# DaehwanKimLab/centrifuge

Hardware: AMD Instinct MI355X
Metric: classified reads/sec (whole node) on 100bp synthetic reads vs p_compressed; HBM GB/s achieved (higher is better)
Workload: dtype u64

## Files before the change

centrifuge_amd/csrc/cf_device.hip:

```cpp
#include <hip/hip_runtime.h>
#include <sched.h>
#include <dlfcn.h>

#include <algorithm>
#include <cmath>
#include <chrono>
#include <cstdio>
#include <cstdlib>
#include <cstring>
#include <memory>
#include <mutex>
#include <stdexcept>
#include <string>
#include <vector>

#include "../../include/centrifuge_amd.h"
#include "cf_index.hpp"
#include "cf_kernels.hpp"
#include "cf_scan.hpp"
#include "cf_textio.hpp"
#include "cf_inflate.hpp"
#include "cf_restore.hpp"
#include "cf_plan.hpp"
#include "cf_knobs.hpp"
// ... 47 lines not shown
__global__ void __launch_bounds__(256) k_search(DIndex ix, DParams pr, DBatch b) { search_body<G>(ix, pr, b); }

__global__ void __launch_bounds__(256) k_rlen(const uint64_t *off, uint32_t *rlen, uint32_t nReads) { rlen_body(off, rlen, nReads, cf_global_thread()); }
__global__ void __launch_bounds__(256) k_convert(DConvert c) { convert_body(c, cf_global_thread()); }
__global__ void __launch_bounds__(256) k_dense_unpack(DUnpack u) { dense_unpack_body(u, (uint64_t)blockIdx.x * blockDim.x + threadIdx.x); }
__global__ void __launch_bounds__(256) k_pack(DBatch b, uint8_t *recs, uint32_t W) { pack_body(b, recs, W, cf_global_thread()); }

template <int G, int W, bool COUNT>
__global__ void __launch_bounds__(256) __attribute__((amdgpu_waves_per_eu(COUNT ? 1 : W == 4 ? 6 : W == 6 ? 5 : 4, 8))) k_search2(DIndex ix, DParams pr, DBatch b) {
    __shared__ __attribute__((aligned(16))) uint8_t lds[(256 / G) * rec_lds_stride(W) + 256 * 4 * RankTab<G>::WORDS + (256 / G) * 16 * kLazyHits];
    search2_body<G, W, COUNT>(ix, pr, b, lds);
}

template <int W, bool COUNT, int LZ = 0, bool MULTI = false>
__global__ void __launch_bounds__(256) __attribute__((amdgpu_waves_per_eu((W == 4 && LZ == 1) ? 7 : (W == 4 && MULTI) ? 6 : (W == 6 && MULTI) ? 5 : 1, 8))) k_search2_l1(DIndex ix, DParams pr, DBatch b) {
    __shared__ __attribute__((aligned(16))) uint8_t lds[256 * rec_lds_stride(W) + 256 * 16 * (LZ ? LZ : (int)lazy_hits(1, W))];
    search2_body<1, W, COUNT, true, LZ, MULTI>(ix, pr, b, lds);
}
__global__ void __launch_bounds__(256) k_pair_planes(DIndex ix, uint8_t *planes2, uint64_t nGroups) {
    pair_planes_body(ix, planes2, (uint64_t)blockIdx.x * blockDim.x + threadIdx.x, nGroups);
}
__global__ void __launch_bounds__(256) k_occ_planes(DIndex ix, uint8_t *planes, uint64_t nSides) {
    occ_planes_body(ix, planes, (uint64_t)blockIdx.x * blockDim.x + threadIdx.x, nSides);
}
__global__ void __launch_bounds__(256) k_repeat_probe(DIndex ix, uint32_t nSamples, uint32_t depth, uint32_t *hits) {
    const uint32_t i = cf_global_thread();
    bool yes = false;
    if (i < nSamples && ix.len > 2) {
        uint64_t x = 0x9e3779b97f4a7c15ull * (i + 1);
        x ^= x >> 29; x *= 0xbf58476d1ce4e5b9ull; x ^= x >> 32;
        yes = repeat_probe_body(ix, x % (ix.len - 1), depth);
    }
    const uint64_t m = cf_ballot(yes);
    if (m && cf_lane() == (uint32_t)cf_ctz64(m)) (void)cf_atomic_add(hits, (uint32_t)cf_popc64(m));
}

__global__ void __launch_bounds__(256) k_post_fast(DIndex ix, DParams pr, DBatch b) {
    const uint32_t q = cf_global_thread();
    const bool d = q < b.nQueries ? post_fast_body(ix, pr, b, q) : false;
    if (q < b.nQueries && b.postDeferred) b.postDeferred[q] = d ? 1 : 0;
    defer_push(b.slowPost, &b.st->nSlowPost, d, q);
}
template <bool EARLY>
__global__ void __launch_bounds__(256) k_score_fast(DIndex ix, DParams pr, DBatch b) {
    const uint32_t q = cf_global_thread();
    const bool d = q < b.nQueries ? score_fast_body<EARLY>(ix, pr, b, q) : false;
    defer_push(b.slowScore, &b.st->nSlowScore, d, q);
}
__global__ void __launch_bounds__(256) k_list_all(uint32_t *list, uint32_t *counter, uint32_t n) {
    const uint32_t q = cf_global_thread();
    if (q < n) list[q] = q;
    if (q == 0) *counter = n;
}
__global__ void __launch_bounds__(64) __attribute__((amdgpu_waves_per_eu(3, 8))) k_post(DIndex ix, DParams pr, DBatch b, uint32_t capHits) {
    extern __shared__ __attribute__((aligned(16))) uint8_t ldsPost[];
    HitP *scratch = capHits ? reinterpret_cast<HitP *>(ldsPost) + (size_t)cf_local_thread() * capHits : nullptr;
    const uint32_t n = b.st->nSlowPost;
    for (uint32_t i = cf_global_thread(); i < n; i += cf_global_threads()) post_body(ix, pr, b, b.slowPost[i], scratch, capHits);
}
__global__ void __launch_bounds__(64) k_postfix_only(DIndex ix, DParams pr, DBatch b) {
    const uint32_t i = cf_global_thread();
    if (i < b.st->nItems / 2) post_fix(ix, pr, b, b.items[i]);
}
__global__ void k_window(DBatch b, uint32_t qLo, bool keepSlow) { if (cf_global_thread() == 0) row_window_body(b, qLo, keepSlow); }
__global__ void __launch_bounds__(256) k_emit(DParams pr, DBatch b) {
    const uint32_t q = cf_global_thread();
    if (q < b.nQueries) emit_body(pr, b, q);
}
template <int G, bool COUNT>
__global__ void __launch_bounds__(256) k_walk2(DIndex ix, DBatch b) { walk2_body<G, COUNT>(ix, b); }
template <int MODE>
__global__ void __launch_bounds__(256) k_walk_table(DIndex ix, DBatch b) { walk2_body<2, false, MODE>(ix, b); }
template <typename T>
__global__ void __launch_bounds__(256) k_stop_samples(DIndex ix, T *stopVal, uint64_t *stopBits, uint64_t nSamples) {
    for (uint64_t i = (uint64_t)blockIdx.x * blockDim.x + threadIdx.x; i < nSamples; i += (uint64_t)gridDim.x * blockDim.x) {
        const uint64_t pos = trio_at(ix.saPos, i << ix.offRate);
        stopVal[pos] = static_cast<const T *>(ix.offs)[i];
        cf_atomic_or64(&stopBits[pos >> 6], 1ull << (pos & 63));
    }
}
template <typename T>
__global__ void __launch_bounds__(256) k_stop_bounds(DIndex ix, T *stopVal, uint64_t *stopBits) {
    for (uint64_t j = (uint64_t)blockIdx.x * blockDim.x + threadIdx.x; j < ix.nBound; j += (uint64_t)gridDim.x * blockDim.x) {
        const uint64_t pos = trio_at(ix.saPos, ix.boundRow[j]);
        stopVal[pos] = (T)ix.boundRef[j];
        cf_atomic_or64(&stopBits[pos >> 6], 1ull << (pos & 63));
    }
}
template <typename T>
__global__ void k_stop_end(DIndex ix, T *stopVal, uint64_t *stopBits) {
    const uint64_t pos = trio_at(ix.saPos, ix.zOff);
    stopVal[pos] = 0;
    cf_atomic_or64(&stopBits[pos >> 6], 1ull << (pos & 63));
}
template <typename T>
__global__ void __launch_bounds__(256) k_table_by_position(DIndex ix, const T *stopVal, const uint64_t *stopBits, T *table, uint64_t nRows, uint32_t *walkMax) {
    uint32_t gap = 0;
    for (uint64_t row = (uint64_t)blockIdx.x * blockDim.x + threadIdx.x; row < nRows; row += (uint64_t)gridDim.x * blockDim.x) {
        const uint64_t pos = trio_at(ix.saPos, row);
        uint64_t w = pos >> 6;
        uint64_t m = stopBits[w] & (~0ull >> (63 - (pos & 63)));
        while (m == 0 && w > 0) m = stopBits[--w];
        const uint64_t pred = m ? (w << 6) + 63 - (uint64_t)__builtin_clzll(m) : 0;
        table[row] = stopVal[pred];
        const uint32_t g = (uint32_t)(pos - pred);
        gap = g > gap ? g : gap;
    }
    for (int d = 32; d > 0; d >>= 1) { const uint32_t o = __shfl_xor(gap, d, 64); gap = o > gap ? o : gap; }
    if ((threadIdx.x & 63) == 0 && gap) atomicMax(walkMax, gap);
}
template <typename T>
__global__ void __launch_bounds__(256) k_table_spot_check(DIndex ix, const T *table, uint64_t nRows, uint32_t nCheck, uint32_t *bad) {
    const uint32_t i = blockIdx.x * blockDim.x + threadIdx.x;
    if (i >= nCheck) return;
    const uint64_t row = i < 64 ? (i < 32 ? (uint64_t)i : nRows - 1 - (i - 32)) % nRows : (0x9e3779b97f4a7c15ull * (i + 1)) % nRows;
    uint32_t steps = 0;
    const uint32_t want = resolve_plain_row(ix, row, steps);
    if ((uint32_t)table[row] != (sizeof(T) == 2 ? (want & 0xffffu) : want)) atomicAdd(bad, 1u);
}

template <bool COUNT>
__global__ void __launch_bounds__(256) k_walk3(DIndex ix, DBatch b) {
    for (uint64_t i = (uint64_t)blockIdx.x * blockDim.x + threadIdx.x; i < b.st->rowHi - b.st->rowLo; i += (uint64_t)gridDim.x * blockDim.x)
        walk3_body<COUNT>(ix, b, i);
}
template <bool PLANES>
__global__ void __launch_bounds__(256) k_wide_ftab(DIndex ix, uint32_t wideChars, uint64_t *table) {
    __builtin_assume(PLANES ? ix.planes != nullptr : ix.planes == nullptr);
    for (uint64_t t = (uint64_t)blockIdx.x * blockDim.x + threadIdx.x; t < (1ull << (2 * wideChars)); t += (uint64_t)gridDim.x * blockDim.x)
        wide_ftab_body(ix, wideChars, table, t);
}

__global__ void __launch_bounds__(64) k_resolve_slow(DIndex ix, DParams pr, DBatch b) {
    const uint32_t n = b.st->nSlowScore;
    for (uint32_t i = cf_global_thread(); i < n; i += cf_global_threads()) resolve_query_body(ix, pr, b, b.slowScore[i]);
}
__global__ void __launch_bounds__(64) k_score(DIndex ix, DParams pr, DBatch b, uint32_t capRows, uint32_t sparse, uint32_t rowsMin, uint32_t rowsMax) {
    extern __shared__ __attribute__((aligned(16))) uint8_t ldsScore[];
    const uint32_t n = b.st->nSlowScore;
    if (cf_local_thread() % sparse) return;
    const uint32_t me = cf_global_thread() / sparse, all = cf_global_threads() / sparse;
    uint8_t *scratch = capRows ? ldsScore + (size_t)(cf_local_thread() / sparse) * score_scratch_bytes(capRows) : nullptr;
    for (uint32_t i = me; i < n; i += all) score_body(ix, pr, b, b.slowScore[i], scratch, capRows, rowsMin, rowsMax);
}

__global__ void __launch_bounds__(256) k_scatter_nmask(const uint64_t *idx, const uint32_t *mask, uint64_t n, uint64_t nWords, uint32_t *nmask) {
    const uint64_t i = (uint64_t)blockIdx.x * blockDim.x + threadIdx.x;
    if (i < n && idx[i] < nWords) nmask[idx[i]] = mask ? mask[i] : 0u;
}
__global__ void __launch_bounds__(1024) k_count(DBatch b, uint32_t slotBits, bool direct) {
    __shared__ uint32_t slots[3 * kCountSlots];
    count_body(b, slots, blockIdx.x, slotBits, direct);
}
__global__ void __launch_bounds__(256) k_plan(DPlan p) { plan_body(p, cf_global_thread()); }
__global__ void __launch_bounds__(256) k_plan_fill(DPlan p) { plan_fill_body(p, cf_global_thread()); }
__global__ void __launch_bounds__(256) k_rev_words(DPlan p, uint32_t wordsPerRead) { rev_words_body(p, wordsPerRead, (uint64_t)blockIdx.x * blockDim.x + threadIdx.x); }
__global__ void __launch_bounds__(256) k_plan_maxscore(const uint32_t *rlen, const uint8_t *pass, uint32_t nQueries, int paired, uint32_t *maxScore) {
    plan_maxscore_body(rlen, pass, nQueries, paired, maxScore, cf_global_thread());
}
__global__ void __launch_bounds__(256) k_compact(DCompact c) {
    compact_body(c, cf_global_thread());
}
__global__ void __launch_bounds__(256) k_text_count(DTextMark m) { text_count_body(m, (uint64_t)blockIdx.x * blockDim.x + threadIdx.x); }
__global__ void __launch_bounds__(256) k_text_mark(DTextMark m) { text_mark_body(m, (uint64_t)blockIdx.x * blockDim.x + threadIdx.x); }
__global__ void __launch_bounds__(256) k_text_records(DTextRec d) { text_record_body(d, cf_global_thread()); }
__global__ void __launch_bounds__(256) k_inflate(DInflate d) {
    __shared__ InfTables tables[256 / CF_WAVE];
    inflate_body<CF_WAVE>(d, cf_global_thread() / CF_WAVE, cf_lane(), &tables[threadIdx.x / CF_WAVE]);
}
__global__ void __launch_bounds__(64) k_inflate_lane(DInflate d) {
    InfTables tables;
    inflate_body<1>(d, cf_global_thread(), 0, &tables);
}
__global__ void k_text_cut(DTextCut c) { if (cf_global_thread() == 0) text_cut_body(c); }
__global__ void k_text_cut_pair(DTextCutPair c) { if (cf_global_thread() == 0) text_cut_pair_body(c); }
static_assert(kCutBadStart == kTxBadStart, "the pair cut's flag is the record pass's");
__global__ void __launch_bounds__(256) k_text_pack(DTextPack d) { text_pack_body(d, cf_global_thread()); }
__global__ void __launch_bounds__(256) k_fmt_size(DTextFmt f) { fmt_size_body(f, cf_global_thread()); }
__global__ void __launch_bounds__(256) k_fmt_write(DTextFmt f) { fmt_write_body(f, cf_global_thread()); }
__global__ void __launch_bounds__(256) k_fmt_cols_size(DTextFmt f, TextCols pc) { fmt_cols_size_body(f, pc, cf_global_thread()); }
__global__ void __launch_bounds__(256) k_fmt_cols_write(DTextFmt f, TextCols pc) { fmt_cols_write_body(f, pc, cf_global_thread()); }
template <int G, bool WRITE>
__global__ void __launch_bounds__(256) k_restore(DIndex ix, DRestore r) { restore_body<G, WRITE>(ix, r); }
__global__ void __launch_bounds__(256) k_restore_rank(const uint64_t *sumIn, const uint32_t *nextIn, uint64_t *sumOut, uint32_t *nextOut, uint32_t nElem) {
    restore_rank_body(sumIn, nextIn, sumOut, nextOut, nElem, cf_global_thread());
}
__global__ void __launch_bounds__(256) k_restore_link(uint64_t *sum, uint32_t *next, uint32_t nSeg, uint32_t *maxLen) {
    const uint32_t s = cf_global_thread();
    if (s < nSeg) {
        if (next[s] == kRestoreTerm) next[s] = nSeg;
        const uint64_t len = sum[s];
        uint32_t l32 = len > 0xffffffffull ? 0xffffffffu : (uint32_t)len;
        for (int m = 32; m > 0; m >>= 1) { const uint32_t o = cf_shfl_xor(l32, m); if (o > l32) l32 = o; }
        if (cf_lane() == 0 && l32) cf_atomic_max(maxLen, l32);
    }
    else if (s == nSeg) { sum[s] = 0; next[s] = nSeg; }
}

template <int G>
__global__ void k_debug_rank(DIndex ix, const uint8_t *chars, const uint64_t *rows, uint64_t n, uint64_t *out) {
    const uint64_t i = (uint64_t)cf_global_thread() / G;
    const uint64_t ii = i < n ? i : n - 1;
    uint64_t t, bb; bool two;
    if (ix.sides) rank_pair<G>(ix, chars[ii] & 3, rows[ii], rows[ii], t, bb, two);
    else rank_any<G>(ix, chars[ii] & 3, rows[ii], rows[ii], t, bb, two);
    if (i < n && Grp<G>::sub() == 0) out[i] = t;
}

__global__ void __launch_bounds__(256) k_random_sides(const uint8_t *sides, uint64_t numSides, uint32_t steps,
                                                        uint64_t seed, unsigned long long *sink) {
    const uint32_t grp = cf_global_thread() >> 3, sub = cf_lane() & 7;
    uint64_t x = seed + 0x9e3779b97f4a7c15ull * (grp + 1);
    unsigned long long acc = 0;
    for (uint32_t s = 0; s < steps; s++) {
        x ^= x >> 12; x ^= x << 25; x ^= x >> 27;
        const uint64_t side = (x * 0x2545f4914f6cdd1dull) % numSides;
        const u64x2 v = cf_load16(sides + side * 128 + 16 * sub);
        uint32_t f = (uint32_t)(v.x ^ v.y);
        f += __shfl_xor(f, 1, 64); f += __shfl_xor(f, 2, 64); f += __shfl_xor(f, 4, 64);
        x += f & 1u;
        acc += f;
    }
    if (acc == 0x1234567u) sink[0] = acc;
}

}

struct TablePlanRecord { int K = 0, textRate = -1, planes = 0, resolveRate = -1, pair = 0, dropSides = 0; bool valid = false; };
struct cf_index {
    HostIndex h;
    int device = -1;
    DIndex d{};
    DevBuf<uint8_t> planes;
    float planesMs = 0;
    DevBuf<uint8_t> planes2;
    float planes2Ms = 0;
    DevBuf<uint64_t> wide;
    float wideMs = 0;
    DevBuf<uint32_t> text;
    DevBuf<uint64_t> saPos, isa;
    float textMs = 0;
    DevBuf<uint8_t> sides, offs, dense;
    int denseRate = -1;
    uint32_t walkMaxSeen = 0;
    bool denseByPos = false;
    uint32_t restoreShift = 0, restoreMaxSeg = 0;
    DevBuf<uint32_t> posBucket;
    DevBuf<u64x2> posFrag, posSeq;
    float denseMs = 0;
    DevBuf<uint64_t> ftab, eftab, boundRow, paths;
    DevBuf<RefInfo> refInfo;
    DevBuf<uint32_t> boundRef, boundBits, pathTidx;
    uint64_t deviceBytes = 0, fileBytes = 0, budgetSeen = 0;
    cf_index_options opt{};
    bool planned = false;
    bool planDropSides = false, sidesDropped = false;
    uint64_t droppedBytes = 0;
    bool wantTextRate0 = false;
    double repeatFrac = -1.0;
    uint32_t multiRowsPlan = 0;
    TablePlanRecord plan{};
    int plannedTextRate = -2;
    int numCUs = 256;
    int occSides[3] = {0, 0, 0}, occPlanes[3] = {0, 0, 0};
    int occMulti[3] = {0, 0, 0};
    int occLazy[3] = {0, 0, 0};
};

struct cf_classifier {
    cf_index *ix = nullptr;
    cf_params p{};
    std::vector<uint64_t> hostList, exclList;
    DParams d{};
    DevBuf<uint8_t> refExcluded;
    DevBuf<uint64_t> hostSet;
    DevBuf<unsigned long long> counts;
    DevBuf<uint8_t> fmtStrs, fmtLeaf;
    DevBuf<uint32_t> fmtUidOff, fmtRankOff, fmtTaxOff;
    uint32_t fmtIdxZero = 0;
    bool fmtMade = false;
    DevBuf<uint8_t> fmtTaxStrs;
    DevBuf<uint32_t> fmtTrankOff, fmtTnameOff;
    bool fmtTaxMade = false;
    std::mutex fmtMu;
};

template <typename T>
struct PinBuf {
    T *p = nullptr;
    size_t n = 0;
    PinBuf() = default;
    PinBuf(const PinBuf &) = delete;
    PinBuf &operator=(const PinBuf &) = delete;
    ~PinBuf() { if (p) (void)hipHostFree(p); }
    void ensure(size_t count) {
        if (count <= n) return;
        if (p) (void)hipHostFree(p);
        p = nullptr; n = 0;
        count += count / 8;
        if (g_dryBytes) { n = count; return; }
        HIP_OK(hipHostMalloc(reinterpret_cast<void **>(&p), count * sizeof(T), hipHostMallocDefault));
        n = count;
    }
};

struct cf_batch {
    cf_classifier *cl = nullptr;
    uint64_t nReads = 0, nQueries = 0, nWords = 0;
    int paired = 0;
    uint32_t maxLenHost = 0;
    uint32_t recWords = 0;
    bool selfRecords = false;
    bool revMade = false;
    uint32_t revDelta = 0;
    bool loaded = false, planned = false, running = false, finished = false, downloaded = false;
    bool fromBytes = false;
    DevBuf<uint8_t> seq, pass, recs;
    DevBuf<uint64_t> bases, woff, off8, hitBase, qBase, rowVal, rowFirst, tileA;
    DevBuf<uint32_t> nmask, rlen, seeds, items, slotOf, hitCap, nhml, rowRef, nOut, score2, maxScore, qRows, tileC, slowPost, slowScore, qflag, itemMeta;
    DevBuf<HitP> hits;
    DevBuf<PlanHit> qplan;
    DevBuf<QHead> qhead;
    DevBuf<uint64_t> o1tax, o1a, o1b;
    DevBuf<uint8_t> dense;
    uint32_t densePending = 0;
    DevBuf<uint8_t> qinfo;
    DevBuf<uint8_t> postDeferred;
    hipEvent_t evPostFast = nullptr, evPost = nullptr;
    int resultFormat = CF_RESULTS_ROWS;
    DevBuf<uint8_t> text, textOut;
    DevBuf<uint32_t> txCnt, txPos, txSeqOff, txIdOff, txIdLen, txQualOff, txSize, txTuples, txTileC;
    TextCols textCols{};
    bool textFastq = false;
    DevBuf<uint64_t> txBase, txOutOff, txTileA;
    DevBuf<TextStatus> txSt;
    PinBuf<TextStatus> hTxSt;
    PinBuf<uint64_t> hTxTotal;
    PinBuf<uint8_t> hTextOut;
    PinBuf<uint32_t> hTuples;
    DevBuf<uint8_t> zIn;
    DevBuf<InfMember> zMembers;
    DevBuf<uint32_t> zErr;
    DevBuf<InfStatus> zSt;
    DevBuf<uint64_t> zCut;
    PinBuf<InfMember> hZMembers;
    PinBuf<uint64_t> hZCut;
    PinBuf<uint8_t> hTail;
    PinBuf<uint8_t> hTail2;
    bool fromText = false;
    bool rowsStay = false;
    bool textDone = false;
    uint64_t textBytes = 0, tupleWords = 0;
    DevBuf<uint64_t> nIdx; DevBuf<uint32_t> nMsk;
    const uint32_t *nmaskZeroOf = nullptr;
    uint64_t nSparsePrev = 0, nmaskZeroN = 0;
    DevBuf<HmEntry> hm;
    DevBuf<TcEntry> tc;
    DevBuf<OutRow> out, outCompact;
    DevBuf<OpCounts> ops;
    DevBuf<unsigned long long> cursor;
    DevBuf<BatchStatus> st;
    uint64_t hitsCapLimit = 0, rowsCapLimit = 0;
    DPlan pl{};
    DBatch d{};
    PinBuf<BatchStatus> hSt;
    PinBuf<OpCounts> hOps;
    PinBuf<OutRow> hRows;
    PinBuf<uint32_t> hNOut, hScore2, hMaxScore;
    PinBuf<uint8_t> hQInfo;
    uint64_t rowsSpec = 0;
    uint64_t rowsOut = 0, rowsTotal = 0;
    double rowsPerQuery = 0;
    double plannedPerQuery = 0;
    uint32_t passes = 0;
    float planMs = 0;
    float ms[5] = {0, 0, 0, 0, 0};
    OpCounts lastOps{};
    bool opsValid = false;
    hipStream_t stream = nullptr;
    hipStream_t tail = nullptr;
    hipEvent_t ev[10] = {};
    hipEvent_t evLate = nullptr;
    bool evInit = false;
    ~cf_batch() { if (evInit) { for (auto &e : ev) (void)hipEventDestroy(e); (void)hipEventDestroy(evLate); (void)hipEventDestroy(evPostFast); (void)hipEventDestroy(evPost); } if (tail) (void)hipStreamDestroy(tail); }
};

namespace {

void streamSection(std::FILE *f, uint64_t bytes, uint8_t *dst) {
    constexpr size_t kChunk = 32u << 20;
    uint8_t *stage[2] = {nullptr, nullptr};
    hipStream_t st;
    HIP_OK(hipStreamCreate(&st));
    hipEvent_t done[2];
    for (int i = 0; i < 2; i++) {
        HIP_OK(hipHostMalloc(reinterpret_cast<void **>(&stage[i]), kChunk, hipHostMallocDefault));
        HIP_OK(hipEventCreate(&done[i]));
    }
    uint64_t pos = 0;
    int cur = 0;
    bool used[2] = {false, false};
    try {
        while (pos < bytes) {
            const size_t n = static_cast<size_t>(std::min<uint64_t>(kChunk, bytes - pos));
            if (used[cur]) HIP_OK(hipEventSynchronize(done[cur]));
            if (std::fread(stage[cur], 1, n, f) != n) throw std::runtime_error("short read while streaming an index section");
            HIP_OK(hipMemcpyAsync(dst + pos, stage[cur], n, hipMemcpyHostToDevice, st));
            HIP_OK(hipEventRecord(done[cur], st));
            used[cur] = true;
            pos += n;
            cur ^= 1;
        }
        HIP_OK(hipStreamSynchronize(st));
    } catch (...) {
        for (int i = 0; i < 2; i++) { (void)hipHostFree(stage[i]); (void)hipEventDestroy(done[i]); }
        (void)hipStreamDestroy(st);
        throw;
    }
    for (int i = 0; i < 2; i++) { (void)hipHostFree(stage[i]); (void)hipEventDestroy(done[i]); }
    (void)hipStreamDestroy(st);
}

void uploadIndex(cf_index &ix, const std::string &base) {
    HostIndex &h = ix.h;
    h.load(base, [&](Section s, std::FILE *f, uint64_t bytes) {
        switch (s) {
            case Section::Sides:
                ix.sides.alloc(bytes + 128);
                streamSection(f, bytes, ix.sides.p);
                break;
            case Section::Ftab:
                ix.ftab.alloc(bytes / 8);
                streamSection(f, bytes, reinterpret_cast<uint8_t *>(ix.ftab.p));
                break;
            case Section::Eftab:
                ix.eftab.alloc(bytes / 8);
                streamSection(f, bytes, reinterpret_cast<uint8_t *>(ix.eftab.p));
                break;
            case Section::SaSample:
                ix.offs.alloc(bytes + 8);
                streamSection(f, bytes, ix.offs.p);
                break;
        }
    });
    const IndexTables t = makeIndexTables(h);
    ix.boundRow.upload(h.boundRow);
    ix.boundRef.upload(h.boundRef);
    ix.boundBits.upload(t.boundBits);
    {
        std::vector<RefInfo> ri(h.uidTid.size() + 1, RefInfo{0, 0, kNone32});
        for (size_t i = 0; i < h.uidTid.size(); i++) ri[i] = RefInfo{h.uidTid[i], t.refTidx[i], t.refPath[i]};
        ix.refInfo.upload(ri);
    }
    ix.paths.upload(t.paths);
    ix.pathTidx.upload(t.pathTidx);

    DIndex &d = ix.d;
    fillIndexScalars(h, t, d);
    d.sides = ix.sides.p; d.ftab = ix.ftab.p; d.eftab = ix.eftab.p;
    d.offs = ix.offs.p; d.walkOffs = ix.offs.p;
    d.boundRow = ix.boundRow.p; d.boundRef = ix.boundRef.p; d.boundBits = ix.boundBits.p;
    d.refInfo = ix.refInfo.p;
    d.paths = ix.paths.p; d.pathTidx = ix.pathTidx.p;
    ix.deviceBytes = ix.sides.bytes() + ix.ftab.bytes() + ix.eftab.bytes() + ix.offs.bytes() + ix.boundRow.bytes() +
                     ix.boundRef.bytes() + ix.boundBits.bytes() + ix.refInfo.bytes() + ix.paths.bytes() + ix.pathTidx.bytes();
}

int envInt(const char *name, int dflt);
int persistentBlocks(const cf_index &ix, uint64_t groups, int blocksPerCU, int lanes);

size_t freeFor(const cf_index &ix) {
    size_t freeB = 0, totalB = 0;
    HIP_OK(hipMemGetInfo(&freeB, &totalB));
    if (ix.opt.hbm_budget_bytes) {
        const uint64_t left = ix.opt.hbm_budget_bytes > ix.deviceBytes ? ix.opt.hbm_budget_bytes - ix.deviceBytes : 0;
        freeB = (size_t)std::min<uint64_t>(freeB, left);
    }
// ... 665 lines not shown
    c->pair_planes_bytes = ix->planes2.bytes(); c->pair_planes = ix->d.planes2 ? 1 : 0;
    c->resolve_bytes = ix->dense.bytes(); c->resolve_rate = ix->denseRate >= 0 ? ix->denseRate : ix->h.g.offRate;
    c->sides_dropped = ix->sidesDropped ? 1 : 0;
    c->file_bytes_dropped = ix->droppedBytes;
    c->small_range_rows = ix->device >= 0 ? (int32_t)ix->d.multiRows : 0;
    c->repeat_fraction = ix->repeatFrac;
    c->plan_realised = !ix->plan.valid ? -1 :
        (ix->d.wideChars == ix->plan.K && (ix->device >= 0 ? ix->d.posRate : -1) == ix->plan.textRate && (ix->d.planes != nullptr) == (ix->plan.planes != 0) &&
         (ix->denseRate >= 0 ? ix->denseRate : ix->h.g.offRate) == ix->plan.resolveRate && (ix->d.planes2 != nullptr) == (ix->plan.pair != 0) &&
         ix->sidesDropped == (ix->plan.dropSides != 0)) ? 1 : 0;
    c->total_bytes = ix->deviceBytes;
    c->build_ms = ix->planesMs + ix->planes2Ms + ix->wideMs + ix->textMs + ix->denseMs;
    const double log4n = n > 1 ? std::log((double)n) / std::log(4.0) : 0.0;
    const int K = c->wide_ftab_chars ? c->wide_ftab_chars : ix->h.g.ftabChars;
    const double calls = 6.5, rows = 1.42;
    const double twoRow = calls * (std::max(0.0, log4n - K) + 1.4);
    const double r = c->text_verify_rate;
    const double single = r < 0 ? 67.6 : 1.5 * (1.0 + ((double)(1u << (int)r) - 1.0)) + 4.0, verify = r < 0 ? 0.0 : 5.0;
    const double walk = rows * (double)(1u << c->resolve_rate);
    c->est_requests_per_100bp_read = twoRow + single + verify + calls + 2.0 + walk;
    return CF_OK;
}

uint64_t cf_index_text_len(const cf_index *ix) { return ix->h.g.len; }
uint64_t cf_index_num_refs(const cf_index *ix) { return ix->h.uid.size(); }
uint64_t cf_index_num_taxa(const cf_index *ix) { return ix->h.taxa.size(); }
uint64_t cf_index_device_bytes(const cf_index *ix) { return ix->deviceBytes; }
int cf_index_compressed(const cf_index *ix) { return ix->h.compressed ? 1 : 0; }
int cf_index_sa_width(const cf_index *ix) { return ix->h.offw ? 4 : 2; }
int cf_index_wide_ftab_chars(const cf_index *ix) { return ix->d.wideChars; }
int cf_index_occ_planes(const cf_index *ix) { return ix->d.planes ? 1 : 0; }
double cf_index_occ_planes_build_ms(const cf_index *ix) { return ix->planesMs; }
int cf_index_text_verify_rate(const cf_index *ix) { return ix->device >= 0 ? ix->d.posRate : -1; }
double cf_index_text_verify_build_ms(const cf_index *ix) { return ix->textMs; }
int cf_index_resolve_rate(const cf_index *ix) { return ix->denseRate >= 0 ? ix->denseRate : ix->h.g.offRate; }
double cf_index_resolve_build_ms(const cf_index *ix) { return ix->denseMs; }
uint32_t cf_index_walk_bound(const cf_index *ix) { return ix->d.posFrag ? ix->d.walkMax : 0u; }
int cf_index_resolve_by_position(const cf_index *ix) { return ix->denseByPos ? 1 : 0; }
const char *cf_index_uid(const cf_index *ix, uint64_t r) { return r < ix->h.uid.size() ? ix->h.uid[r].c_str() : ""; }
uint64_t cf_index_ref_taxid(const cf_index *ix, uint64_t r) { return r < ix->h.uidTid.size() ? ix->h.uidTid[r] : 0; }
uint64_t cf_index_taxon_id(const cf_index *ix, uint64_t i) { return i < ix->h.taxa.size() ? ix->h.taxa[i] : 0; }
const char *cf_format_seqid(const cf_index *ix, uint32_t u, uint64_t t) { return ix->h.formatSeqId(u, t); }
int cf_tax_rank(const cf_index *ix, uint64_t t) { const TaxNode *n = ix->h.findNode(t); return n ? n->rank : 0; }
const char *cf_tax_rank_string(int rank) { return rankString(rank); }
const char *cf_tax_name(const cf_index *ix, uint64_t t) { return ix->h.name(t); }
uint64_t cf_tax_size(const cf_index *ix, uint64_t t) { return ix->h.size(t); }

cf_status cf_params_default(cf_params *p) {
    if (!p) return CF_ERR_ARG;
    std::memset(p, 0, sizeof *p);
    p->khits = 5; p->min_hitlen = 22; p->rank_slot = 0; p->tree_traverse = 1;
    return CF_OK;
}

cf_status cf_classifier_create(cf_index *ix, const cf_params *p, cf_classifier **out) {
    if (!ix || !p || !out || p->khits < 1 || p->min_hitlen < 15 || p->rank_slot < 0 || p->rank_slot > 9) return CF_ERR_ARG;
    *out = nullptr;
    if (ix->device < 0) { g_err = "index was opened host-only"; return CF_ERR_NO_DEVICE; }
    auto cl = std::make_unique<cf_classifier>();
    cf_status st = guard([&] {
        HIP_OK(hipSetDevice(ix->device));
        cl->ix = ix; cl->p = *p;
        cl->hostList.assign(p->host_taxids, p->host_taxids + std::max(0, p->n_host));
        cl->exclList.assign(p->exclude_taxids, p->exclude_taxids + std::max(0, p->n_exclude));
        cl->p.host_taxids = cl->hostList.data(); cl->p.exclude_taxids = cl->exclList.data();
        const ClassifierTables t = makeClassifier(ix->h, cl->p, cl->d);
        if (cl->d.ihits >= 0x7fffffffu) throw ArgError("-k too large");
        if (ix->h.g.len >= (1ull << 40)) throw ArgError("index too large: hit records hold 40-bit rows");
        if (!t.refExcluded.empty()) { cl->refExcluded.upload(t.refExcluded); cl->d.refExcluded = cl->refExcluded.p; }
        if (!t.hostSet.empty()) { cl->hostSet.upload(t.hostSet); cl->d.hostSet = cl->hostSet.p; cl->d.nHostSet = (uint32_t)t.hostSet.size(); }
        cl->counts.alloc(3 * ix->h.taxa.size());
        HIP_OK(hipMemset(cl->counts.p, 0, cl->counts.bytes()));
    });
    if (st == CF_OK) *out = cl.release();
    return st;
}
void cf_classifier_destroy(cf_classifier *c) { delete c; }

uint32_t cf_gen_rand_seed(const uint8_t *seq, const uint8_t *qual, uint64_t len, const char *name, uint64_t nlen,
                          uint32_t seed) {
    uint32_t r = (seed + 101u) * 59u * 61u * 67u * 71u * 73u * 79u * 83u;
    for (uint64_t i = 0; i < len; i++) r ^= (uint32_t)seq[i] << ((i & 15) << 1);
    for (uint64_t i = 0; i < len; i++) r ^= (uint32_t)(qual ? qual[i] : (uint8_t)'I') << ((i & 3) << 3);
    for (uint64_t i = 0; i < nlen; i++) {
        const int p = (int)(signed char)name[i];
        if (p == '/') break;
        r ^= (uint32_t)p << ((i & 3) << 3);
    }
    return r;
}


static void sizeBatch(cf_batch *bt, uint64_t nReads, uint64_t nWords, uint64_t nBases, uint32_t maxLen, int paired) {
    cf_classifier *cl = bt->cl;
    if (paired && (nReads & 1)) throw ArgError("a paired batch needs an even number of reads");
    if (nReads >= 0x7fffffffull) throw ArgError("a batch holds fewer than 2^31 reads");
    if (maxLen > kMaxReadLen) throw ArgError("reads of more than 16,777,213 bases are not supported (24-bit offsets in the hit records)");
    const uint32_t ftc = (uint32_t)std::max(1, cl->ix->h.g.ftabChars);
    bt->nReads = nReads; bt->paired = paired ? 1 : 0; bt->nQueries = paired ? nReads / 2 : nReads; bt->nWords = nWords;
    bt->maxLenHost = maxLen;
    const uint64_t nq = bt->nQueries;
    bt->bases.ensure(nWords + 16); bt->nmask.ensure(nWords + 16);
    bt->rlen.ensure(nReads + 16); bt->seeds.ensure(nReads + 1); bt->woff.ensure(nReads + 1);
    bt->pass.ensure(nReads + 1); bt->hitCap.ensure(nReads + 16);
    bt->slotOf.ensure(nReads + 1); bt->hitBase.ensure(nReads + 1); bt->items.ensure(nReads + 1);
    bt->nhml.ensure(2 * nReads + 1);
    bt->maxScore.ensure(nq + 1); bt->qflag.ensure(nq + 1); bt->qhead.ensure(nq + 1); bt->qRows.ensure(nq + 16); bt->qBase.ensure(nq + 1);
    bt->qplan.ensure((nq + 1) * kInlinePlan); bt->o1tax.ensure((nq + 1) * kFieldRows); bt->o1a.ensure((nq + 1) * kFieldRows); bt->o1b.ensure((nq + 1) * kFieldRows);
    bt->slowPost.ensure(nq + 1); bt->slowScore.ensure(nq + 1);
    if (envInt("CF_EARLY_SCORE", 0)) bt->postDeferred.ensure(nq + 16);
    bt->out.ensure(nq * (uint64_t)cl->d.k + 1); bt->nOut.ensure(nq + 16); bt->score2.ensure(nq + 1); bt->rowFirst.ensure(nq + 1);
    bt->cursor.ensure(4); bt->ops.ensure(1); bt->st.ensure(1);
    bt->tileA.ensure(scan_tiles_for(std::max(nReads, nq)) + 1); bt->tileC.ensure(scan_tiles_for(std::max(nReads, nq)) + 1);
    bt->recWords = searchVersion() != 2 ? 0u : maxLen <= 128 ? 4u : maxLen <= 192 ? 6u : maxLen <= 256 ? 8u : 0u;
    if ((uint64_t)(0.15 * maxLen) + maxLen / (uint64_t)ftc + 3 >= 255) bt->recWords = 0;
    bt->selfRecords = bt->recWords && cl->ix->d.planes && nWords < 0xffffffffull && envInt("CF_SELF_RECORDS", 1);
    if (bt->selfRecords) bt->itemMeta.ensure(8 * nReads + 8);
    bt->revDelta = bt->selfRecords && 2 * nWords + 64 < 0xffffffffull && envInt("CF_REV_WORDS", 1) ? (uint32_t)nWords + 16u : 0u;
    if (bt->revDelta) bt->bases.ensure(2 * (nWords + 16));
    else if (bt->recWords) bt->recs.ensure(2 * nReads * (uint64_t)rec_bytes((int)bt->recWords) + 64);
    uint64_t hitsWant = 2 * ((nBases ? nBases : 32 * nWords) / ftc + 2 * nReads);
    hitsWant += hitsWant / 50 + 4096;
    if (bt->hitsCapLimit) hitsWant = std::min(hitsWant, bt->hitsCapLimit);
    if (bt->hits.n < hitsWant) bt->hits.ensure(hitsWant);
    if (bt->recWords && bt->hits.n > 0xffffffffull) throw ArgError("batch too large: its hit lists need 32-bit offsets, split it");
    uint64_t rowsWant = std::max<uint64_t>(4 * nq, 1u << 16);
    if (bt->plannedPerQuery > 0) rowsWant = std::max<uint64_t>(rowsWant, (uint64_t)((double)nq * bt->plannedPerQuery * 1.15));
    if (const int per = envInt("CF_ROWS_PER_QUERY", 0)) rowsWant = std::max<uint64_t>((uint64_t)per * nq, 1024);
    if (bt->rowsCapLimit) rowsWant = bt->rowsCapLimit;
    if (bt->rowVal.n < rowsWant || bt->rowsCapLimit) { bt->rowVal.ensure(rowsWant); bt->rowRef.ensure(rowsWant); bt->hm.ensure(rowsWant); bt->tc.ensure(rowsWant); }
    bt->outCompact.ensure(nq * (uint64_t)cl->d.k + 1);
    bt->hSt.ensure(1); bt->hOps.ensure(1);
    bt->hNOut.ensure(nq + 1); bt->hScore2.ensure(nq + 1); bt->hMaxScore.ensure(nq + 1);
    if (bt->resultFormat == CF_RESULTS_NARROW) { bt->qinfo.ensure(nq + 16); bt->hQInfo.ensure(nq + 16); }
    bt->rowsSpec = bt->rowsPerQuery > 0 ? (uint64_t)((double)nq * bt->rowsPerQuery * 1.04) + 4096 : nq + nq / 4 + 1024;
    bt->rowsSpec = std::min<uint64_t>(bt->rowsSpec, nq * (uint64_t)cl->d.k);
    bt->hRows.ensure(std::max<uint64_t>(bt->rowsSpec, nq + nq / 4 + 1024));
    if (g_dryBytes) return;
    if (!bt->evInit) { for (auto &e : bt->ev) HIP_OK(hipEventCreate(&e)); HIP_OK(hipEventCreate(&bt->evLate)); HIP_OK(hipEventCreate(&bt->evPostFast)); HIP_OK(hipEventCreate(&bt->evPost)); bt->evInit = true; }
    if (!bt->tail && (envInt("CF_TAIL_STREAM", 0) || envInt("CF_EARLY_SCORE", 0))) HIP_OK(hipStreamCreateWithFlags(&bt->tail, hipStreamNonBlocking));
}

static void bindBatch(cf_batch *bt) {
    cf_classifier *cl = bt->cl;
    DPlan &pl = bt->pl;
    pl.nmask = bt->nmask.p; pl.rlen = bt->rlen.p; pl.woff = bt->woff.p; pl.nReads = (uint32_t)bt->nReads; pl.ftabChars = cl->ix->h.g.ftabChars;
    pl.maxLenAllowed = bt->maxLenHost;
    pl.nWords = bt->nWords;
    pl.pass = bt->pass.p; pl.hitCap = bt->hitCap.p; pl.slotOf = bt->slotOf.p;
    pl.hitBase = bt->hitBase.p; pl.items = bt->items.p; pl.st = bt->st.p;
    pl.itemMeta = bt->selfRecords ? bt->itemMeta.p : nullptr;
    pl.bases = bt->bases.p; pl.revDelta = bt->revDelta;
    pl.hitsCap = bt->hitsCapLimit ? std::min<uint64_t>(bt->hitsCapLimit, bt->hits.n) : bt->hits.n;
    DBatch &d = bt->d;
    d.bases = bt->bases.p; d.nmask = bt->nmask.p; d.rlen = bt->rlen.p; d.woff = bt->woff.p; d.seeds = bt->seeds.p;
    d.pass = bt->pass.p; d.items = bt->items.p; d.slotOf = bt->slotOf.p; d.hitBase = bt->hitBase.p; d.hitCap = bt->hitCap.p;
    d.lazyHits = (uint32_t)(envInt("CF_LAZY_HITS", 1) != 0) | (cl->ix->d.posFrag ? 4u : 0u);
    d.directRefs = (uint32_t)(cl->ix->dense.p && cl->ix->d.walkRate == 0 && envInt("CF_SCORE_FAST", 1) != 0 && envInt("CF_DIRECT_REFS", 1) != 0);
    d.hits = bt->hits.p; d.nhml = bt->nhml.p; d.qflag = bt->qflag.p; d.qhead = bt->qhead.p; d.qplan = bt->qplan.p; d.qplanStride = bt->qplan.n / kInlinePlan; d.qRows = bt->qRows.p; d.qBase = bt->qBase.p;
    d.rowVal = bt->rowVal.p; d.rowRef = bt->rowRef.p; d.hm = bt->hm.p; d.tc = bt->tc.p;
    d.out = bt->out.p; d.nOut = bt->nOut.p; d.score2 = bt->score2.p;
    d.counts = cl->counts.p; d.nTaxa = (uint32_t)cl->ix->h.taxa.size();
    d.nReads = (uint32_t)bt->nReads; d.nQueries = (uint32_t)bt->nQueries; d.paired = bt->paired;
    d.cursor = bt->cursor.p; d.st = bt->st.p; d.ops = bt->ops.p;
    d.slowPost = bt->slowPost.p; d.slowScore = bt->slowScore.p; d.postDeferred = envInt("CF_EARLY_SCORE", 0) ? bt->postDeferred.p : nullptr;
    d.o1tax = bt->o1tax.p; d.o1a = bt->o1a.p; d.o1b = bt->o1b.p; d.oStride = bt->o1tax.n / kFieldRows;
    d.hitsCap = pl.hitsCap;
    d.rowsCap = bt->rowsCapLimit ? std::min<uint64_t>(bt->rowsCapLimit, bt->rowVal.n) : bt->rowVal.n;
    d.recs = bt->recWords && !bt->selfRecords ? bt->recs.p : nullptr; d.recWords = bt->recWords;
    d.itemMeta = bt->selfRecords ? bt->itemMeta.p : nullptr;
}

static void enqueuePlan(cf_batch *bt, hipStream_t st) {
    const uint64_t nReads = bt->nReads;
    const DPlan &pl = bt->pl;
    HIP_OK(hipStreamWaitEvent(st, bt->ev[8], 0));
    if (bt->densePending) {
        const uint32_t L = bt->densePending - 1;
        const DUnpack u{bt->dense.p, bt->bases.p, bt->rlen.p, (uint32_t)nReads, L, bt->revDelta ? bt->bases.p + bt->revDelta : nullptr};
        bt->revMade = bt->revDelta != 0;
        const uint64_t threads = nReads * std::max<uint64_t>(((uint64_t)L + 31) >> 5, 1);
        hipLaunchKernelGGL(k_dense_unpack, dim3((unsigned)((threads + 255) / 256)), dim3(256), 0, st, u);
        bt->densePending = 0;
    }
    HIP_OK(hipEventRecord(bt->ev[5], st));
    HIP_OK(hipMemsetAsync(bt->st.p, 0, sizeof(BatchStatus), st));
    const dim3 gp((unsigned)((nReads + 1 + 255) / 256)), bl(256);
    if (bt->fromBytes && nReads) hipLaunchKernelGGL(k_rlen, gp, bl, 0, st, bt->off8.p, bt->rlen.p, (uint32_t)nReads);
    scan_enqueue<SCAN_WORDS>(bt->rlen.p, nReads, bt->woff.p, nullptr, bt->tileA.p, bt->tileC.p, st);
    if (bt->fromBytes && nReads) {
        DConvert c{bt->seq.p, bt->off8.p, bt->woff.p, bt->bases.p, bt->nmask.p, (uint32_t)nReads};
        hipLaunchKernelGGL(k_convert, dim3((unsigned)((nReads + 255) / 256)), dim3(256), 0, st, c);
    }
    if (bt->fromText && nReads) {
        const DTextPack c{bt->text.p, bt->txSeqOff.p, bt->rlen.p, bt->woff.p, bt->bases.p, bt->nmask.p, (uint32_t)nReads};
        hipLaunchKernelGGL(k_text_pack, dim3((unsigned)((nReads + 255) / 256)), dim3(256), 0, st, c);
    }
    hipLaunchKernelGGL(k_plan, gp, bl, 0, st, pl);
    scan_enqueue<SCAN_HITS>(bt->hitCap.p, nReads, bt->hitBase.p, bt->slotOf.p, bt->tileA.p, bt->tileC.p, st);
    hipLaunchKernelGGL(k_plan_fill, gp, bl, 0, st, pl);
    if (pl.revDelta && nReads && !bt->revMade) {
        const uint64_t threads = nReads * (uint64_t)bt->recWords;
        hipLaunchKernelGGL(k_rev_words, dim3((unsigned)((threads + 255) / 256)), bl, 0, st, pl, bt->recWords);
    }
    if (bt->nQueries) hipLaunchKernelGGL(k_plan_maxscore, dim3((unsigned)((bt->nQueries + 255) / 256)), bl, 0, st, bt->rlen.p, bt->pass.p,
                                         (uint32_t)bt->nQueries, bt->paired, bt->maxScore.p);
    if (bt->recWords && !bt->selfRecords && nReads) {
        const uint64_t threads = 2 * nReads * (uint64_t)bt->recWords;
        hipLaunchKernelGGL(k_pack, dim3((unsigned)((threads + 255) / 256)), bl, 0, st, bt->d, bt->recs.p, bt->recWords);
    }
    HIP_OK(hipEventRecord(bt->ev[6], st));
    bt->planned = true;
}

static dim3 listGrid(const cf_index &ix, uint64_t nq) { return dim3((unsigned)std::max<uint64_t>(1, std::min<uint64_t>((nq + 63) / 64, (uint64_t)ix.numCUs * 32))); }

static bool earlyScoreMode(const cf_batch *bt) {
    static const bool on = envInt("CF_EARLY_SCORE", 0) != 0 && envInt("CF_POST_FAST", 1) != 0 && envInt("CF_SCORE_FAST", 1) != 0 && envInt("CF_TAIL_STREAM", 0) == 0;
    return on && bt->d.directRefs != 0 && bt->tail != nullptr && bt->nQueries != 0;
}

static void enqueuePost(cf_batch *bt, hipStream_t st) {
    cf_classifier *cl = bt->cl;
    cf_index &ix = *cl->ix;
    const DBatch &d = bt->d;
    const uint32_t nq = (uint32_t)bt->nQueries;
    if (!nq) return;
    static const bool fast = envInt("CF_POST_FAST", 1) != 0;
    if (fast) hipLaunchKernelGGL(k_post_fast, dim3((nq + 255) / 256), dim3(256), 0, st, ix.d, cl->d, d);
    else hipLaunchKernelGGL(k_list_all, dim3((nq + 255) / 256), dim3(256), 0, st, bt->slowPost.p, &bt->st.p->nSlowPost, nq);
    if (earlyScoreMode(bt)) {
        HIP_OK(hipEventRecord(bt->evPostFast, st));
        HIP_OK(hipStreamWaitEvent(bt->tail, bt->evPostFast, 0));
        hipLaunchKernelGGL(k_post, listGrid(ix, nq), dim3(64), 0, bt->tail, ix.d, cl->d, d, 0u);
        HIP_OK(hipEventRecord(bt->evPost, bt->tail));
        hipLaunchKernelGGL(k_score_fast<true>, dim3((nq + 255) / 256), dim3(256), 0, st, ix.d, cl->d, d);
        HIP_OK(hipStreamWaitEvent(st, bt->evPost, 0));
        return;
    }
    static const bool postLds = envInt("CF_POST_LDS", 0) != 0;
    const uint32_t capHits = postLds ? (uint32_t)std::min<uint64_t>(60, 2 * ((uint64_t)bt->maxLenHost / (uint64_t)std::max(1, ix.h.g.ftabChars) + 2)) : 0u;
    hipLaunchKernelGGL(k_post, listGrid(ix, nq), dim3(64), (size_t)64 * capHits * sizeof(HitP), st, ix.d, cl->d, d, capHits);
}

static bool enqueueRowPass(cf_batch *bt, uint32_t qLo, hipStream_t st, bool marks, hipStream_t late = nullptr, bool early = false) {
    cf_classifier *cl = bt->cl;
    cf_index &ix = *cl->ix;
    const DBatch &d = bt->d;
    const uint32_t nq = (uint32_t)bt->nQueries;
    static const bool fast = envInt("CF_SCORE_FAST", 1) != 0;
    HIP_OK(hipMemsetAsync(bt->cursor.p + 1, 0, 8, st));
    hipLaunchKernelGGL(k_window, dim3(1), dim3(64), 0, st, d, qLo, early);
    const bool direct = d.directRefs != 0;
    if (nq && !direct) hipLaunchKernelGGL(k_emit, dim3((nq + 255) / 256), dim3(256), 0, st, cl->d, d);
    if (marks) HIP_OK(hipEventRecord(bt->ev[2], st));
    const bool counted = nq && !direct ? launchWalk(cl, bt, st) : true;
    if (marks) HIP_OK(hipEventRecord(bt->ev[3], st));
    if (nq) {
        if (early) {}
        else if (fast) hipLaunchKernelGGL(k_score_fast<false>, dim3((nq + 255) / 256), dim3(256), 0, st, ix.d, cl->d, d);
        else hipLaunchKernelGGL(k_list_all, dim3((nq + 255) / 256), dim3(256), 0, st, bt->slowScore.p, &bt->st.p->nSlowScore, nq);
        if (late && late != st) {
            HIP_OK(hipEventRecord(bt->evLate, st));
            HIP_OK(hipStreamWaitEvent(late, bt->evLate, 0));
            st = late;
        }
        if (direct) hipLaunchKernelGGL(k_resolve_slow, listGrid(ix, nq), dim3(64), 0, st, ix.d, cl->d, d);
        static const uint32_t capRows = (uint32_t)std::clamp(envInt("CF_SCORE_LDS_ROWS", 0), 0, 64), sparse = (uint32_t)std::clamp(envInt("CF_SCORE_LDS_SPARSE", 2), 1, 64);
        hipLaunchKernelGGL(k_score, listGrid(ix, nq), dim3(64), (size_t)(64 / sparse) * score_scratch_bytes(capRows), st, ix.d, cl->d, d, capRows, capRows ? sparse : 1u, 0u, 0xffffffffu);
        static const uint32_t slotBits = (uint32_t)std::clamp(envInt("CF_COUNT_SLOT_BITS", (int)kCountSlotBits), 1, (int)kCountSlotBits);
        hipLaunchKernelGGL(k_count, dim3((nq + kCountChunk - 1) / kCountChunk), dim3(1024), 0, st, d, slotBits, d.nTaxa <= (1u << slotBits));
    }
    if (marks) HIP_OK(hipEventRecord(bt->ev[4], st));
    return counted;
}

static void enqueueCompact(cf_batch *bt, hipStream_t st) {
    const uint32_t nq = (uint32_t)bt->nQueries;
    const dim3 g((nq + 1 + 255) / 256), bl(256);
    scan_enqueue<SCAN_PLAIN>(bt->nOut.p, nq, bt->rowFirst.p, nullptr, bt->tileA.p, bt->tileC.p, st);
    const bool narrow = bt->resultFormat == CF_RESULTS_NARROW;
    const DCompact c{bt->out.p, bt->o1tax.p, bt->o1a.p, bt->o1b.p, bt->d.oStride, bt->nOut.p, bt->rowFirst.p, (uint32_t)bt->cl->d.k, nq, bt->outCompact.p, bt->st.p,
                     narrow ? reinterpret_cast<NarrowRow *>(bt->outCompact.p) : nullptr, bt->qinfo.p, bt->pass.p, bt->paired};
    hipLaunchKernelGGL(k_compact, g, bl, 0, st, c);
}

static void enqueueClassify(cf_batch *bt, hipStream_t st) {
    cf_classifier *cl = bt->cl;
    HIP_OK(hipMemsetAsync(bt->cursor.p, 0, 32, st));
    HIP_OK(hipMemsetAsync(bt->ops.p, 0, sizeof(OpCounts), st));
    static const bool allFast = envInt("CF_POST_FAST", 1) != 0 && envInt("CF_SCORE_FAST", 1) != 0;
    if (!allFast) {
        HIP_OK(hipMemsetAsync(bt->qRows.p, 0, 4 * (bt->nQueries + 1), st));
        HIP_OK(hipMemsetAsync(bt->nOut.p, 0, 4 * (bt->nQueries + 1), st));
    }
    HIP_OK(hipMemsetAsync(&bt->st.p->nSlowPost, 0, 8, st));
    HIP_OK(hipEventRecord(bt->ev[0], st));
    bool counted = true;
    if (bt->nReads) counted = launchSearch(cl, bt, st) && counted;
    HIP_OK(hipEventRecord(bt->ev[1], st));
    static const int tailMode = envInt("CF_TAIL_STREAM", 0);
    hipStream_t ts = bt->tail && tailMode == 1 ? bt->tail : st;
    hipStream_t late = bt->tail && tailMode == 2 ? bt->tail : ts;
    if (ts != st) HIP_OK(hipStreamWaitEvent(ts, bt->ev[1], 0));
    const bool early = earlyScoreMode(bt);
    enqueuePost(bt, ts);
    scan_enqueue<SCAN_PLAIN>(bt->qRows.p, bt->nQueries, bt->qBase.p, nullptr, bt->tileA.p, bt->tileC.p, ts);
    counted = enqueueRowPass(bt, 0, ts, true, late, early) && counted;
    enqueueCompact(bt, late);
    HIP_OK(hipEventRecord(bt->ev[9], late));
    bt->opsValid = counted;
    bt->passes = 1;
    bt->running = true; bt->finished = false; bt->downloaded = false;
    bt->stream = st;
}

static void enqueueDownload(cf_batch *bt, hipStream_t st) {
    const uint64_t nq = bt->nQueries;
    HIP_OK(hipStreamWaitEvent(st, bt->ev[9], 0));
    HIP_OK(hipMemcpyAsync(bt->hSt.p, bt->st.p, sizeof(BatchStatus), hipMemcpyDeviceToHost, st));
    HIP_OK(hipMemcpyAsync(bt->hOps.p, bt->ops.p, sizeof(OpCounts), hipMemcpyDeviceToHost, st));
    if (nq && !bt->rowsStay) {
        const uint64_t spec = std::min<uint64_t>(bt->rowsSpec, nq * (uint64_t)bt->cl->d.k);
        if (bt->resultFormat == CF_RESULTS_NARROW) {
            HIP_OK(hipMemcpyAsync(bt->hQInfo.p, bt->qinfo.p, nq, hipMemcpyDeviceToHost, st));
            HIP_OK(hipMemcpyAsync(bt->hScore2.p, bt->score2.p, nq * 4, hipMemcpyDeviceToHost, st));
            HIP_OK(hipMemcpyAsync(bt->hRows.p, bt->outCompact.p, spec * sizeof(NarrowRow), hipMemcpyDeviceToHost, st));
        } else {
            HIP_OK(hipMemcpyAsync(bt->hNOut.p, bt->nOut.p, nq * 4, hipMemcpyDeviceToHost, st));
            HIP_OK(hipMemcpyAsync(bt->hScore2.p, bt->score2.p, nq * 4, hipMemcpyDeviceToHost, st));
            HIP_OK(hipMemcpyAsync(bt->hMaxScore.p, bt->maxScore.p, nq * 4, hipMemcpyDeviceToHost, st));
            HIP_OK(hipMemcpyAsync(bt->hRows.p, bt->outCompact.p, spec * sizeof(OutRow), hipMemcpyDeviceToHost, st));
        }
    }
    HIP_OK(hipEventRecord(bt->ev[7], st));
    bt->downloaded = true;
}

static void waitBatch(cf_batch *bt) {
    if (!bt->running) throw ArgError("no batch in flight on this slot");
    if (bt->finished) return;
    hipStream_t st = bt->stream;
    if (!bt->downloaded) enqueueDownload(bt, st);
    HIP_OK(hipEventSynchronize(bt->ev[7]));
    HIP_OK(hipGetLastError());
    bool redo = false;
    auto fetchStatus = [&] {
        HIP_OK(hipEventSynchronize(bt->ev[9]));
        HIP_OK(hipMemcpyAsync(bt->hSt.p, bt->st.p, sizeof(BatchStatus), hipMemcpyDeviceToHost, st));
        HIP_OK(hipStreamSynchronize(st));
        HIP_OK(hipGetLastError());
    };
    HIP_OK(hipEventSynchronize(bt->ev[9]));
    auto lapse = [&](float &ms, int a, int b) { if (hipEventElapsedTime(&ms, bt->ev[a], bt->ev[b]) != hipSuccess) { ms = 0; (void)hipGetLastError(); } };
    lapse(bt->planMs, 5, 6);
    lapse(bt->ms[0], 0, 1); lapse(bt->ms[1], 1, 2); lapse(bt->ms[2], 2, 3); lapse(bt->ms[3], 3, 4); lapse(bt->ms[4], 0, 4);
    if (bt->hSt.p->flags & kStLenOverflow) throw ArgError("a read is longer than the max_len the batch was submitted with");
    if (bt->hSt.p->flags & kStWordsOverflow) throw ArgError("the read lengths need more packed words than n_words says were uploaded");
    if (bt->hSt.p->flags & kStHitsOverflow) {
        const uint64_t need = bt->hSt.p->hitsNeed;
        if (bt->recWords && need > 0xffffffffull) throw ArgError("batch too large: its hit lists need 32-bit offsets, split it");
        bt->hitsCapLimit = 0;
        bt->hits.ensure(need + 1);
        bindBatch(bt);
        enqueuePlan(bt, st);
        enqueueClassify(bt, st);
        fetchStatus();
        if (bt->hSt.p->flags & kStHitsOverflow) throw std::logic_error("hit pool still too small after growing it");
        redo = true;
    }
    while (bt->hSt.p->qHi < bt->nQueries) {
        if (bt->hSt.p->qHi == bt->hSt.p->qLo) {
            const uint64_t need = bt->hSt.p->needRows;
            bt->rowsCapLimit = 0;
            bt->rowVal.ensure(need); bt->rowRef.ensure(need); bt->hm.ensure(need); bt->tc.ensure(need);
            bindBatch(bt);
        }
        enqueueRowPass(bt, bt->hSt.p->qHi, st, false);
        bt->passes++;
        bt->opsValid = false;
        fetchStatus();
        redo = true;
    }
    if (redo) {
        enqueueCompact(bt, st);
        HIP_OK(hipEventRecord(bt->ev[9], st));
        enqueueDownload(bt, st);
        HIP_OK(hipEventSynchronize(bt->ev[7]));
        HIP_OK(hipGetLastError());
    }
    bt->rowsOut = bt->hSt.p->rowsOut;
    bt->rowsTotal = bt->hSt.p->rowsTotal;
    if (bt->nQueries) { bt->rowsPerQuery = (double)bt->rowsOut / (double)bt->nQueries; bt->plannedPerQuery = (double)bt->rowsTotal / (double)bt->nQueries; }
    if (bt->rowsOut > bt->rowsSpec && !bt->rowsStay) {
        const uint64_t have = bt->rowsSpec;
        const size_t rb = bt->resultFormat == CF_RESULTS_NARROW ? sizeof(NarrowRow) : sizeof(OutRow);
        if (bt->rowsOut > bt->hRows.n) {
            PinBuf<OutRow> bigger;
            bigger.ensure(bt->rowsOut + bt->rowsOut / 8);
            std::memcpy(bigger.p, bt->hRows.p, have * rb);
            std::swap(bt->hRows.p, bigger.p); std::swap(bt->hRows.n, bigger.n);
        }
        HIP_OK(hipMemcpy(reinterpret_cast<uint8_t *>(bt->hRows.p) + have * rb, reinterpret_cast<const uint8_t *>(bt->outCompact.p) + have * rb, (bt->rowsOut - have) * rb, hipMemcpyDeviceToHost));
    }
    bt->lastOps = *bt->hOps.p;
    bt->lastOps.nRows = bt->rowsTotal;
    bt->finished = true;
}

static void uploadBytes(cf_batch *bt, const uint8_t *seq, const uint64_t *off, const uint32_t *seeds, uint64_t nReads, int paired, hipStream_t st) {
    uint64_t nWords = 0, maxLen = 0;
    for (uint64_t r = 0; r < nReads; r++) {
        if (off[r + 1] < off[r]) throw ArgError("read offsets must be non-decreasing");
        const uint64_t L = off[r + 1] - off[r];
        nWords += (L + 31) >> 5;
        maxLen = std::max(maxLen, L);
    }
    if (maxLen > 0xffffffffull) throw ArgError("a read is longer than 2^32 bases");
    const uint64_t nbases = off[nReads] - off[0];
    if (nbases && !seq) throw ArgError("null sequence buffer");
    sizeBatch(bt, nReads, nWords, nbases, (uint32_t)maxLen, paired);
    bt->seq.ensure(nbases + 16); bt->off8.ensure(nReads + 1);
    bindBatch(bt);
    HIP_OK(hipMemsetAsync(bt->seq.p + nbases, 0, 16, st));
    if (nbases) HIP_OK(hipMemcpyAsync(bt->seq.p, seq + off[0], nbases, hipMemcpyHostToDevice, st));
    if (off[0] == 0) HIP_OK(hipMemcpyAsync(bt->off8.p, off, (nReads + 1) * 8, hipMemcpyHostToDevice, st));
    else {
        std::vector<uint64_t> rel(nReads + 1);
        for (uint64_t r = 0; r <= nReads; r++) rel[r] = off[r] - off[0];
        HIP_OK(hipMemcpy(bt->off8.p, rel.data(), (nReads + 1) * 8, hipMemcpyHostToDevice));
    }
    if (nReads) HIP_OK(hipMemcpyAsync(bt->seeds.p, seeds, nReads * 4, hipMemcpyHostToDevice, st));
    HIP_OK(hipEventRecord(bt->ev[8], st));
    bt->fromBytes = true; bt->fromText = false; bt->densePending = 0; bt->revMade = false; bt->nmaskZeroOf = nullptr;
    bt->loaded = true; bt->planned = false; bt->running = false; bt->finished = false;
}

static void uploadSparseMask(cf_batch *bt, const uint64_t *idx, const uint32_t *mask, uint64_t nNWords, uint64_t nWords, hipStream_t st) {
    if (bt->nmaskZeroOf != bt->nmask.p || bt->nmaskZeroN != bt->nmask.n) {
        HIP_OK(hipMemsetAsync(bt->nmask.p, 0, bt->nmask.bytes(), st));
        bt->nmaskZeroOf = bt->nmask.p; bt->nmaskZeroN = bt->nmask.n; bt->nSparsePrev = 0;
    } else if (bt->nSparsePrev) {
        hipLaunchKernelGGL(k_scatter_nmask, dim3((unsigned)((bt->nSparsePrev + 255) / 256)), dim3(256), 0, st, bt->nIdx.p, nullptr,
                           bt->nSparsePrev, (uint64_t)bt->nmask.n, bt->nmask.p);
        bt->nSparsePrev = 0;
    }
    if (nNWords) {
        bt->nSparsePrev = nNWords;
        bt->nIdx.ensure(nNWords); bt->nMsk.ensure(nNWords);
        HIP_OK(hipMemcpyAsync(bt->nIdx.p, idx, nNWords * 8, hipMemcpyHostToDevice, st));
        HIP_OK(hipMemcpyAsync(bt->nMsk.p, mask, nNWords * 4, hipMemcpyHostToDevice, st));
        hipLaunchKernelGGL(k_scatter_nmask, dim3((unsigned)((nNWords + 255) / 256)), dim3(256), 0, st, bt->nIdx.p, bt->nMsk.p,
                           nNWords, nWords, bt->nmask.p);
    }
}

static void uploadPacked(cf_batch *bt, const cf_packed_reads *in, hipStream_t st) {
    if (in->n_reads && (!in->len || !in->seeds)) throw ArgError("null length / seed array");
    if (in->n_words && !in->bases) throw ArgError("null packed-base array");
    if (!in->nmask && in->n_nwords && (!in->nword_idx || !in->nword_mask)) throw ArgError("null sparse N-mask arrays");
    sizeBatch(bt, in->n_reads, in->n_words, in->n_bases, in->max_len, in->paired);
    bindBatch(bt);
    if (in->n_words) {
        HIP_OK(hipMemcpyAsync(bt->bases.p, in->bases, in->n_words * 8, hipMemcpyHostToDevice, st));
        if (in->nmask) { HIP_OK(hipMemcpyAsync(bt->nmask.p, in->nmask, in->n_words * 4, hipMemcpyHostToDevice, st)); bt->nmaskZeroOf = nullptr; }
        else uploadSparseMask(bt, in->nword_idx, in->nword_mask, in->n_nwords, in->n_words, st);
    }
    if (in->n_reads) {
        HIP_OK(hipMemcpyAsync(bt->rlen.p, in->len, in->n_reads * 4, hipMemcpyHostToDevice, st));
        HIP_OK(hipMemcpyAsync(bt->seeds.p, in->seeds, in->n_reads * 4, hipMemcpyHostToDevice, st));
    }
    HIP_OK(hipEventRecord(bt->ev[8], st));
    bt->fromBytes = false; bt->fromText = false; bt->densePending = 0; bt->revMade = false;
    bt->loaded = true; bt->planned = false; bt->running = false; bt->finished = false;
}

static void uploadDense(cf_batch *bt, const cf_dense_reads *in, hipStream_t st) {
    if (in->n_reads && (!in->bases4 || !in->seeds)) throw ArgError("null dense-base / seed array");
    if (in->n_nwords && (!in->nword_idx || !in->nword_mask)) throw ArgError("null sparse N-mask arrays");
    if (in->read_len > kMaxReadLen) throw ArgError("reads of more than 16,777,213 bases are not supported (24-bit offsets in the hit records)");
    const uint64_t W = ((uint64_t)in->read_len + 31) >> 5, bpr = ((uint64_t)in->read_len + 3) >> 2;
    const uint64_t nWords = in->n_reads * W, nBytes = in->n_reads * bpr;
    sizeBatch(bt, in->n_reads, nWords, in->n_reads * (uint64_t)in->read_len, in->read_len, in->paired);
    bt->dense.ensure(nBytes + 32);
    bindBatch(bt);
    if (in->n_reads) {
        HIP_OK(hipMemcpyAsync(bt->dense.p, in->bases4, nBytes, hipMemcpyHostToDevice, st));
        HIP_OK(hipMemsetAsync(bt->dense.p + nBytes, 0, 32, st));
        HIP_OK(hipMemcpyAsync(bt->seeds.p, in->seeds, in->n_reads * 4, hipMemcpyHostToDevice, st));
        if (nWords) uploadSparseMask(bt, in->nword_idx, in->nword_mask, in->n_nwords, nWords, st);
    }
    bt->densePending = in->n_reads ? in->read_len + 1 : 0; bt->revMade = false;
    HIP_OK(hipEventRecord(bt->ev[8], st));
    bt->fromBytes = false; bt->fromText = false;
    bt->loaded = true; bt->planned = false; bt->running = false; bt->finished = false;
}


static void uploadText(cf_batch *bt, const cf_text_reads *in, hipStream_t st, cf_text_info *info) {
    if (in->format != CF_TEXT_FASTA && in->format != CF_TEXT_FASTQ) throw ArgError("cf_text_reads::format is CF_TEXT_FASTA or CF_TEXT_FASTQ");
    const int nBlocks = in->text2 ? 2 : 1;
    const char *src[2] = {in->text, in->text2};
    const uint64_t nBs[2] = {in->n_bytes, in->text2 ? in->n_bytes2 : 0};
    if ((nBs[0] && !src[0]) || (nBs[1] && !src[1])) throw ArgError("null text block");
    if (nBs[0] + nBs[1] >= 0xffff0000ull) throw ArgError("the text blocks of a batch hold fewer than 2^32 bytes (32-bit places in them)");
    const bool fasta = in->format == CF_TEXT_FASTA;
    uint64_t at[2], pieces[2], pieceAt[2], recCap[2], posCap[2], posAt[2], textBytes = 0, nPieces = 0, posTotal = 0, recMax = 0;
    for (int k = 0; k < nBlocks; k++) {
        at[k] = textBytes; pieces[k] = (nBs[k] + kTextPiece - 1) / kTextPiece; pieceAt[k] = nPieces;
        recCap[k] = nBs[k] / 32 + 1024; posCap[k] = fasta ? recCap[k] : 4 * recCap[k]; posAt[k] = posTotal;
        textBytes += pieces[k] * kTextPiece + kTextPad; nPieces += pieces[k] + 16; posTotal += posCap[k] + 16;
        recMax = std::max(recMax, recCap[k]);
    }
    const uint64_t readCap = recMax * (uint64_t)nBlocks;
    bt->text.ensure(textBytes);
    bt->txCnt.ensure(nPieces + 16); bt->txBase.ensure(nPieces + 16); bt->txPos.ensure(posTotal + 16);
    bt->txTileA.ensure(scan_tiles_for(std::max(pieces[0], pieces[nBlocks - 1])) + 1); bt->txTileC.ensure(scan_tiles_for(std::max(pieces[0], pieces[nBlocks - 1])) + 1);
    bt->rlen.ensure(readCap + 16); bt->seeds.ensure(readCap + 16);
    bt->txSeqOff.ensure(readCap + 16); bt->txIdOff.ensure(readCap + 16); bt->txIdLen.ensure(readCap + 16);
    if (!fasta) bt->txQualOff.ensure(readCap + 16);
    bt->txSt.ensure(1); bt->hTxSt.ensure(1); bt->hTxTotal.ensure(2);
    *info = cf_text_info{};
    bt->loaded = false; bt->planned = false; bt->running = false; bt->finished = false;
    HIP_OK(hipMemsetAsync(bt->txSt.p, 0, sizeof(TextStatus), st));
    const uint32_t seed0 = (in->global_seed + 101u) * 59u * 61u * 67u * 71u * 73u * 79u * 83u;
    const dim3 bl(256);
    for (int k = 0; k < nBlocks; k++) {
        uint8_t *text = bt->text.p + at[k];
        HIP_OK(hipMemsetAsync(text + nBs[k], 0, pieces[k] * kTextPiece + kTextPad - nBs[k], st));
        if (nBs[k]) HIP_OK(hipMemcpyAsync(text, src[k], nBs[k], hipMemcpyHostToDevice, st));
        uint32_t *cnt = bt->txCnt.p + pieceAt[k], *pos = bt->txPos.p + posAt[k];
        uint64_t *base = bt->txBase.p + pieceAt[k];
        const DTextMark m{text, nBs[k], fasta ? (uint32_t)'>' : (uint32_t)'\n', cnt, base, pos, posCap[k]};
        const dim3 gp((unsigned)std::max<uint64_t>(1, (pieces[k] + 255) / 256));
        if (pieces[k]) hipLaunchKernelGGL(k_text_count, gp, bl, 0, st, m);
        scan_enqueue<SCAN_PLAIN>(cnt, pieces[k], base, nullptr, bt->txTileA.p, bt->txTileC.p, st);
        if (pieces[k]) hipLaunchKernelGGL(k_text_mark, gp, bl, 0, st, m);
        DTextRec d{text, nBs[k], pos, base + pieces[k], posCap[k], (uint32_t)recCap[k], (uint32_t)in->format, seed0,
                   bt->rlen.p, bt->seeds.p, bt->txSeqOff.p, bt->txIdOff.p, bt->txIdLen.p, bt->txSt.p, (uint32_t)at[k], (uint32_t)nBlocks, (uint32_t)k,
                   fasta ? nullptr : bt->txQualOff.p};
        hipLaunchKernelGGL(k_text_records, dim3((unsigned)((recCap[k] + 255) / 256)), bl, 0, st, d);
        HIP_OK(hipMemcpyAsync(bt->hTxTotal.p + k, base + pieces[k], 8, hipMemcpyDeviceToHost, st));
    }
    HIP_OK(hipMemcpyAsync(bt->hTxSt.p, bt->txSt.p, sizeof(TextStatus), hipMemcpyDeviceToHost, st));
    HIP_OK(hipStreamSynchronize(st));
    HIP_OK(hipGetLastError());
    const TextStatus ts = *bt->hTxSt.p;
    uint64_t nRec[2] = {0, 0};
    for (int k = 0; k < nBlocks; k++) nRec[k] = fasta ? bt->hTxTotal.p[k] : bt->hTxTotal.p[k] >> 2;
    if (ts.flags) { info->irregular = ts.flags; return; }
    if (nBlocks == 2 && nRec[0] != nRec[1]) { info->irregular = kTxMateCount; return; }
    uint64_t nq = nRec[0];
    if (in->max_reads && nq > in->max_reads) nq = in->max_reads;
    const uint64_t nReads = nq * (uint64_t)nBlocks;
    sizeBatch(bt, nReads, ts.words(), ts.bases(), ts.maxLen, nBlocks == 2);
    bindBatch(bt);
    HIP_OK(hipEventRecord(bt->ev[8], st));
    bt->fromText = true; bt->fromBytes = false; bt->densePending = 0; bt->revMade = false; bt->nmaskZeroOf = nullptr;
    bt->textFastq = !fasta;
    bt->loaded = true;
    info->n_reads = nReads; info->n_bases = ts.bases(); info->max_len = ts.maxLen;
}

constexpr uint64_t kBgzfTailRoom = 1u << 20;
static void uploadBgzf(cf_batch *bt, const cf_bgzf_reads *in, hipStream_t st, cf_text_info *info, cf_bgzf_info *zi) {
    if (in->format != CF_TEXT_FASTA && in->format != CF_TEXT_FASTQ) throw ArgError("cf_bgzf_reads::format is CF_TEXT_FASTA or CF_TEXT_FASTQ");
    if ((in->n_bytes && !in->members) || (in->head_bytes && !in->head)) throw ArgError("null member / head bytes");
    if (in->n_bytes >= 0xffff0000ull || in->head_bytes >= 0xffff0000ull) throw ArgError("the text of a batch holds fewer than 2^32 - 65536 bytes (32-bit places in it)");
    *info = cf_text_info{}; *zi = cf_bgzf_info{};
    bt->loaded = false; bt->planned = false; bt->running = false; bt->finished = false;
    const uint8_t *z = static_cast<const uint8_t *>(in->members);
    uint64_t nMembers = 0;
    for (uint64_t at = 0; at < in->n_bytes; nMembers++) {
        if (in->n_bytes - at < 18) break;
        at += (uint64_t)(z[at + 16] | (z[at + 17] << 8)) + 1;
    }
    bt->hZMembers.ensure(nMembers + 1);
    uint64_t total = in->head_bytes, at = 0;
    uint32_t m = 0;
    for (; at < in->n_bytes; m++) {
        const uint8_t *h = z + at;
        bool ok = in->n_bytes - at >= 18 && h[0] == 0x1f && h[1] == 0x8b && h[2] == 8 && (h[3] & 4);
        const uint64_t xlen = ok ? (uint64_t)(h[10] | (h[11] << 8)) : 0, bsize = ok ? (uint64_t)(h[16] | (h[17] << 8)) + 1 : 0;
        ok = ok && xlen >= 6 && h[12] == 'B' && h[13] == 'C' && h[14] == 2 && h[15] == 0 && bsize >= 12 + xlen + 8 && bsize <= in->n_bytes - at;
        uint32_t crc = 0, isize = 0;
        if (ok) { std::memcpy(&crc, h + bsize - 8, 4); std::memcpy(&isize, h + bsize - 4, 4); ok = isize <= kInfMaxOut; }
        if (!ok) { zi->corrupt = kInfHeader; zi->bad_member = m; return; }
        bt->hZMembers.p[m] = InfMember{(uint32_t)(at + 12 + xlen), (uint32_t)(bsize - 12 - xlen - 8), (uint32_t)total, isize, crc};
        total += isize; at += bsize;
        if (total >= 0xffff0000ull) throw ArgError("the text of a batch holds fewer than 2^32 - 65536 bytes (32-bit places in it)");
    }
    nMembers = m;
    zi->inflated_bytes = total - in->head_bytes;
    const bool fasta = in->format == CF_TEXT_FASTA;
    const uint64_t pieces = (total + kTextPiece - 1) / kTextPiece, recCap = total / 32 + 1024, posCap = fasta ? recCap : 4 * recCap;
    bt->text.ensure(pieces * kTextPiece + kTextPad);
    bt->zIn.ensure(in->n_bytes + kInfPad + 8); bt->zMembers.ensure(nMembers + 1); bt->zErr.ensure(nMembers + 1); bt->zSt.ensure(1); bt->zCut.ensure(2);
    bt->hZCut.ensure(4); bt->hTail.ensure(kBgzfTailRoom + 16);
    bt->txCnt.ensure(pieces + 32); bt->txBase.ensure(pieces + 32); bt->txPos.ensure(posCap + 32);
    bt->txTileA.ensure(scan_tiles_for(pieces) + 1); bt->txTileC.ensure(scan_tiles_for(pieces) + 1);
    bt->rlen.ensure(recCap + 16); bt->seeds.ensure(recCap + 16);
    bt->txSeqOff.ensure(recCap + 16); bt->txIdOff.ensure(recCap + 16); bt->txIdLen.ensure(recCap + 16);
    if (!fasta) bt->txQualOff.ensure(recCap + 16);
    bt->txSt.ensure(1); bt->hTxSt.ensure(1); bt->hTxTotal.ensure(2);
    HIP_OK(hipMemsetAsync(bt->txSt.p, 0, sizeof(TextStatus), st));
    HIP_OK(hipMemsetAsync(bt->zSt.p, 0, sizeof(InfStatus), st));
    uint8_t *text = bt->text.p;
    HIP_OK(hipMemsetAsync(text + total, 0, pieces * kTextPiece + kTextPad - total, st));
    if (in->head_bytes) HIP_OK(hipMemcpyAsync(text, in->head, in->head_bytes, hipMemcpyHostToDevice, st));
    if (nMembers) {
        HIP_OK(hipMemcpyAsync(bt->zIn.p, in->members, in->n_bytes, hipMemcpyHostToDevice, st));
        HIP_OK(hipMemcpyAsync(bt->zMembers.p, bt->hZMembers.p, nMembers * sizeof(InfMember), hipMemcpyHostToDevice, st));
        const DInflate d{bt->zIn.p, bt->zMembers.p, (uint32_t)nMembers, text, bt->zErr.p, bt->zSt.p, nullptr};
        static const bool byLane = cfamd::cf_knob("CF_INFLATE_LANES") && std::atoi(cfamd::cf_knob("CF_INFLATE_LANES")) == 1;
        if (byLane) hipLaunchKernelGGL(k_inflate_lane, dim3((unsigned)((nMembers + 63) / 64)), dim3(64), 0, st, d);
        else hipLaunchKernelGGL(k_inflate, dim3((unsigned)((nMembers + 256 / CF_WAVE - 1) / (256 / CF_WAVE))), dim3(256), 0, st, d);
    }
    const dim3 bl(256);
    const DTextMark mk{text, total, fasta ? (uint32_t)'>' : (uint32_t)'\n', bt->txCnt.p, bt->txBase.p, bt->txPos.p, posCap};
    const dim3 gp((unsigned)std::max<uint64_t>(1, (pieces + 255) / 256));
    if (pieces) hipLaunchKernelGGL(k_text_count, gp, bl, 0, st, mk);
    scan_enqueue<SCAN_PLAIN>(bt->txCnt.p, pieces, bt->txBase.p, nullptr, bt->txTileA.p, bt->txTileC.p, st);
    if (pieces) hipLaunchKernelGGL(k_text_mark, gp, bl, 0, st, mk);
    const DTextCut ct{text, total, bt->txPos.p, bt->txBase.p + pieces, posCap, fasta ? 0u : 1u, in->last ? 1u : 0u, bt->zCut.p};
    hipLaunchKernelGGL(k_text_cut, dim3(1), dim3(64), 0, st, ct);
    HIP_OK(hipMemcpyAsync(bt->hZCut.p, bt->zCut.p, 16, hipMemcpyDeviceToHost, st));
    HIP_OK(hipMemcpyAsync(bt->hZCut.p + 2, bt->zSt.p, sizeof(InfStatus), hipMemcpyDeviceToHost, st));
    HIP_OK(hipStreamSynchronize(st));
    HIP_OK(hipGetLastError());
    InfStatus zs; std::memcpy(&zs, bt->hZCut.p + 2, sizeof zs);
    if (zs.bad) {
        zi->bad_member = 0xffffffffu - zs.bad;
        HIP_OK(hipMemcpy(&zi->corrupt, bt->zErr.p + zi->bad_member, 4, hipMemcpyDeviceToHost));
        if (!zi->corrupt) zi->corrupt = kInfBadCode;
        return;
    }
    const uint64_t cut = bt->hZCut.p[0];
    if (cut > total) throw std::runtime_error("cf_batch_upload_bgzf: the cut lies behind the text");
    if (total - cut > kBgzfTailRoom) { info->irregular = kTxTailRoom; return; }
    if (total > cut) HIP_OK(hipMemcpyAsync(bt->hTail.p, text + cut, total - cut, hipMemcpyDeviceToHost, st));
    const uint32_t seed0 = (in->global_seed + 101u) * 59u * 61u * 67u * 71u * 73u * 79u * 83u;
    const DTextRec d{text, cut, bt->txPos.p, bt->zCut.p + 1, posCap, (uint32_t)recCap, (uint32_t)in->format, seed0,
                     bt->rlen.p, bt->seeds.p, bt->txSeqOff.p, bt->txIdOff.p, bt->txIdLen.p, bt->txSt.p, 0u, 1u, 0u, fasta ? nullptr : bt->txQualOff.p};
    hipLaunchKernelGGL(k_text_records, dim3((unsigned)((recCap + 255) / 256)), bl, 0, st, d);
    HIP_OK(hipMemcpyAsync(bt->hTxSt.p, bt->txSt.p, sizeof(TextStatus), hipMemcpyDeviceToHost, st));
    HIP_OK(hipStreamSynchronize(st));
    HIP_OK(hipGetLastError());
    const TextStatus ts = *bt->hTxSt.p;
    if (ts.flags) { info->irregular = ts.flags; return; }
    uint64_t nq = fasta ? bt->hZCut.p[1] : bt->hZCut.p[1] >> 2;
    if (in->max_reads && nq > in->max_reads) nq = in->max_reads;
    sizeBatch(bt, nq, ts.words(), ts.bases(), ts.maxLen, false);
    bindBatch(bt);
    HIP_OK(hipEventRecord(bt->ev[8], st));
    bt->fromText = true; bt->fromBytes = false; bt->densePending = 0; bt->revMade = false; bt->nmaskZeroOf = nullptr;
    bt->textFastq = !fasta;
    bt->loaded = true;
    info->n_reads = nq; info->n_bases = ts.bases(); info->max_len = ts.maxLen;
    zi->tail = reinterpret_cast<const char *>(bt->hTail.p); zi->tail_bytes = total - cut;
}

static bool bgzfMemberTable(const cf_bgzf_reads *in, uint64_t inAt, uint64_t textAt, InfMember *out, uint64_t &nMembers, uint64_t &total, cf_bgzf_info *zi) {
    const uint8_t *z = static_cast<const uint8_t *>(in->members);
    uint64_t at = 0;
    uint32_t m = 0;
    total = in->head_bytes;
    for (; at < in->n_bytes; m++) {
        const uint8_t *h = z + at;
        bool ok = in->n_bytes - at >= 18 && h[0] == 0x1f && h[1] == 0x8b && h[2] == 8 && (h[3] & 4);
        const uint64_t xlen = ok ? (uint64_t)(h[10] | (h[11] << 8)) : 0, bsize = ok ? (uint64_t)(h[16] | (h[17] << 8)) + 1 : 0;
        ok = ok && xlen >= 6 && h[12] == 'B' && h[13] == 'C' && h[14] == 2 && h[15] == 0 && bsize >= 12 + xlen + 8 && bsize <= in->n_bytes - at;
        uint32_t crc = 0, isize = 0;
        if (ok) { std::memcpy(&crc, h + bsize - 8, 4); std::memcpy(&isize, h + bsize - 4, 4); ok = isize <= kInfMaxOut; }
        if (!ok) { zi->corrupt = kInfHeader; zi->bad_member = m; return false; }
        if (out) out[m] = InfMember{(uint32_t)(inAt + at + 12 + xlen), (uint32_t)(bsize - 12 - xlen - 8), (uint32_t)(textAt + total), isize, crc};
        total += isize; at += bsize;
        if (total >= 0xffff0000ull) throw ArgError("the texts of a batch hold fewer than 2^32 - 65536 bytes (32-bit places in them)");
    }
    nMembers = m;
    return true;
}
static void uploadBgzfPair(cf_batch *bt, const cf_bgzf_reads *in1, const cf_bgzf_reads *in2, hipStream_t st, cf_text_info *info, cf_bgzf_info *z1, cf_bgzf_info *z2) {
    const cf_bgzf_reads *in[2] = {in1, in2};
    cf_bgzf_info *zi[2] = {z1, z2};
    if (in1->format != CF_TEXT_FASTA && in1->format != CF_TEXT_FASTQ) throw ArgError("cf_bgzf_reads::format is CF_TEXT_FASTA or CF_TEXT_FASTQ");
    if (in2->format != in1->format || in2->global_seed != in1->global_seed || in2->max_reads != in1->max_reads)
        throw ArgError("cf_batch_upload_bgzf_pair: format, global_seed and max_reads are the first mate's; the second mate's differ");
    for (int k = 0; k < 2; k++) {
        if ((in[k]->n_bytes && !in[k]->members) || (in[k]->head_bytes && !in[k]->head)) throw ArgError("null member / head bytes");
        if (in[k]->n_bytes >= 0xffff0000ull || in[k]->head_bytes >= 0xffff0000ull) throw ArgError("the texts of a batch hold fewer than 2^32 - 65536 bytes (32-bit places in them)");
    }
    const uint64_t inAt[2] = {0, (in1->n_bytes + 7) & ~7ull}, inBytes = inAt[1] + in2->n_bytes;
    if (inBytes >= 0xffff0000ull) throw ArgError("the members of a batch hold fewer than 2^32 - 65536 bytes (32-bit places in them)");
    *info = cf_text_info{}; *z1 = cf_bgzf_info{}; *z2 = cf_bgzf_info{};
    bt->loaded = false; bt->planned = false; bt->running = false; bt->finished = false;
    uint64_t nM[2] = {0, 0}, total[2] = {0, 0};
    for (int k = 0; k < 2; k++) if (!bgzfMemberTable(in[k], 0, 0, nullptr, nM[k], total[k], zi[k])) return;
    if (total[0] + total[1] >= 0xffff0000ull) throw ArgError("the texts of a batch hold fewer than 2^32 - 65536 bytes (32-bit places in them)");
    const bool fasta = in1->format == CF_TEXT_FASTA;
    uint64_t at[2], pieces[2], pieceAt[2], recCap[2], posCap[2], posAt[2], textBytes = 0, nPieces = 0, posTotal = 0, recMax = 0;
    for (int k = 0; k < 2; k++) {
        at[k] = textBytes; pieces[k] = (total[k] + kTextPiece - 1) / kTextPiece; pieceAt[k] = nPieces;
        recCap[k] = total[k] / 32 + 1024; posCap[k] = fasta ? recCap[k] : 4 * recCap[k]; posAt[k] = posTotal;
        textBytes += pieces[k] * kTextPiece + kTextPad; nPieces += pieces[k] + 16; posTotal += posCap[k] + 16;
        recMax = std::max(recMax, recCap[k]);
    }
    if (textBytes >= 0xffffffffull) throw ArgError("the texts of a batch hold fewer than 2^32 - 65536 bytes (32-bit places in them)");
    const uint64_t nMembers = nM[0] + nM[1];
    bt->hZMembers.ensure(nMembers + 1);
    for (int k = 0; k < 2; k++) (void)bgzfMemberTable(in[k], inAt[k], at[k], bt->hZMembers.p + (k ? nM[0] : 0), nM[k], total[k], zi[k]);
    for (int k = 0; k < 2; k++) zi[k]->inflated_bytes = total[k] - in[k]->head_bytes;
    const uint64_t readCap = 2 * recMax;
    bt->text.ensure(textBytes);
    bt->zIn.ensure(inBytes + kInfPad + 8); bt->zMembers.ensure(nMembers + 1); bt->zErr.ensure(nMembers + 1); bt->zSt.ensure(1); bt->zCut.ensure(4);
    bt->hZCut.ensure(6); bt->hTail.ensure(kBgzfTailRoom + 16); bt->hTail2.ensure(kBgzfTailRoom + 16);
    bt->txCnt.ensure(nPieces + 16); bt->txBase.ensure(nPieces + 16); bt->txPos.ensure(posTotal + 16);
    bt->txTileA.ensure(scan_tiles_for(std::max(pieces[0], pieces[1])) + 1); bt->txTileC.ensure(scan_tiles_for(std::max(pieces[0], pieces[1])) + 1);
    bt->rlen.ensure(readCap + 16); bt->seeds.ensure(readCap + 16);
    bt->txSeqOff.ensure(readCap + 16); bt->txIdOff.ensure(readCap + 16); bt->txIdLen.ensure(readCap + 16);
    if (!fasta) bt->txQualOff.ensure(readCap + 16);
    bt->txSt.ensure(1); bt->hTxSt.ensure(1); bt->hTxTotal.ensure(2);
    HIP_OK(hipMemsetAsync(bt->txSt.p, 0, sizeof(TextStatus), st));
    HIP_OK(hipMemsetAsync(bt->zSt.p, 0, sizeof(InfStatus), st));
    for (int k = 0; k < 2; k++) {
        uint8_t *text = bt->text.p + at[k];
        HIP_OK(hipMemsetAsync(text + total[k], 0, pieces[k] * kTextPiece + kTextPad - total[k], st));
        if (in[k]->head_bytes) HIP_OK(hipMemcpyAsync(text, in[k]->head, in[k]->head_bytes, hipMemcpyHostToDevice, st));
        if (nM[k]) HIP_OK(hipMemcpyAsync(bt->zIn.p + inAt[k], in[k]->members, in[k]->n_bytes, hipMemcpyHostToDevice, st));
    }
    if (nMembers) {
        HIP_OK(hipMemcpyAsync(bt->zMembers.p, bt->hZMembers.p, nMembers * sizeof(InfMember), hipMemcpyHostToDevice, st));
        const DInflate d{bt->zIn.p, bt->zMembers.p, (uint32_t)nMembers, bt->text.p, bt->zErr.p, bt->zSt.p, nullptr};
        hipLaunchKernelGGL(k_inflate, dim3((unsigned)((nMembers + 256 / CF_WAVE - 1) / (256 / CF_WAVE))), dim3(256), 0, st, d);
    }
    const dim3 bl(256);
    DTextCutPair cp{};
    for (int k = 0; k < 2; k++) {
        uint8_t *text = bt->text.p + at[k];
        uint32_t *cnt = bt->txCnt.p + pieceAt[k], *pos = bt->txPos.p + posAt[k];
        uint64_t *base = bt->txBase.p + pieceAt[k];
        const DTextMark mk{text, total[k], fasta ? (uint32_t)'>' : (uint32_t)'\n', cnt, base, pos, posCap[k]};
        const dim3 gp((unsigned)std::max<uint64_t>(1, (pieces[k] + 255) / 256));
        if (pieces[k]) hipLaunchKernelGGL(k_text_count, gp, bl, 0, st, mk);
        scan_enqueue<SCAN_PLAIN>(cnt, pieces[k], base, nullptr, bt->txTileA.p, bt->txTileC.p, st);
        if (pieces[k]) hipLaunchKernelGGL(k_text_mark, gp, bl, 0, st, mk);
        cp.blk[k] = DTextCut{text, total[k], pos, base + pieces[k], posCap[k], fasta ? 0u : 1u, in[k]->last ? 1u : 0u, bt->zCut.p + 2 * k};
    }
    cp.flags = &bt->txSt.p->flags;
    hipLaunchKernelGGL(k_text_cut_pair, dim3(1), dim3(64), 0, st, cp);
    HIP_OK(hipMemcpyAsync(bt->hZCut.p, bt->zCut.p, 32, hipMemcpyDeviceToHost, st));
    HIP_OK(hipMemcpyAsync(bt->hZCut.p + 4, bt->zSt.p, sizeof(InfStatus), hipMemcpyDeviceToHost, st));
    HIP_OK(hipStreamSynchronize(st));
    HIP_OK(hipGetLastError());
    InfStatus zs; std::memcpy(&zs, bt->hZCut.p + 4, sizeof zs);
    if (zs.bad) {
        const uint64_t g = 0xffffffffu - zs.bad;
        cf_bgzf_info *z = g < nM[0] ? z1 : z2;
        z->bad_member = (uint32_t)(g < nM[0] ? g : g - nM[0]);
        HIP_OK(hipMemcpy(&z->corrupt, bt->zErr.p + g, 4, hipMemcpyDeviceToHost));
        if (!z->corrupt) z->corrupt = kInfBadCode;
        return;
    }
    const uint64_t cut[2] = {bt->hZCut.p[0], bt->hZCut.p[2]}, nMark[2] = {bt->hZCut.p[1], bt->hZCut.p[3]};
    if (cut[0] > total[0] || cut[1] > total[1]) throw std::runtime_error("cf_batch_upload_bgzf_pair: a cut lies behind its text");
    if (in1->last && in2->last && (cut[0] < total[0] || cut[1] < total[1])) { info->irregular = kTxMateCount; return; }
    if (total[0] - cut[0] > kBgzfTailRoom || total[1] - cut[1] > kBgzfTailRoom) { info->irregular = kTxTailRoom; return; }
    uint8_t *hTail[2] = {bt->hTail.p, bt->hTail2.p};
    for (int k = 0; k < 2; k++) if (total[k] > cut[k]) HIP_OK(hipMemcpyAsync(hTail[k], bt->text.p + at[k] + cut[k], total[k] - cut[k], hipMemcpyDeviceToHost, st));
    const uint32_t seed0 = (in1->global_seed + 101u) * 59u * 61u * 67u * 71u * 73u * 79u * 83u;
    for (int k = 0; k < 2; k++) {
        const DTextRec d{bt->text.p + at[k], cut[k], bt->txPos.p + posAt[k], bt->zCut.p + 2 * k + 1, posCap[k], (uint32_t)recCap[k], (uint32_t)in1->format, seed0,
                         bt->rlen.p, bt->seeds.p, bt->txSeqOff.p, bt->txIdOff.p, bt->txIdLen.p, bt->txSt.p, (uint32_t)at[k], 2u, (uint32_t)k,
                         fasta ? nullptr : bt->txQualOff.p};
        hipLaunchKernelGGL(k_text_records, dim3((unsigned)((recCap[k] + 255) / 256)), bl, 0, st, d);
    }
    HIP_OK(hipMemcpyAsync(bt->hTxSt.p, bt->txSt.p, sizeof(TextStatus), hipMemcpyDeviceToHost, st));
    HIP_OK(hipStreamSynchronize(st));
    HIP_OK(hipGetLastError());
    const TextStatus ts = *bt->hTxSt.p;
    if (ts.flags) { info->irregular = ts.flags; return; }
    uint64_t nq = fasta ? nMark[0] : nMark[0] >> 2;
    if (nq != (fasta ? nMark[1] : nMark[1] >> 2)) throw std::runtime_error("cf_batch_upload_bgzf_pair: the two cuts hold different numbers of records");
    if (in1->max_reads && nq > in1->max_reads) nq = in1->max_reads;
    sizeBatch(bt, 2 * nq, ts.words(), ts.bases(), ts.maxLen, true);
    bindBatch(bt);
    HIP_OK(hipEventRecord(bt->ev[8], st));
    bt->fromText = true; bt->fromBytes = false; bt->densePending = 0; bt->revMade = false; bt->nmaskZeroOf = nullptr;
    bt->textFastq = !fasta;
    bt->loaded = true;
    info->n_reads = 2 * nq; info->n_bases = ts.bases(); info->max_len = ts.maxLen;
    for (int k = 0; k < 2; k++) { zi[k]->tail = reinterpret_cast<const char *>(hTail[k]); zi[k]->tail_bytes = total[k] - cut[k]; }
}

cf_status cf_host_alloc(void **p, size_t bytes) {
    if (!p) return CF_ERR_ARG;
    *p = nullptr;
    if (!haveDevice()) { g_err = "no HIP device visible"; return CF_ERR_NO_DEVICE; }
    return guard([&] { HIP_OK(hipHostMalloc(p, bytes ? bytes : 1, hipHostMallocDefault)); });
}
void cf_host_free(void *p) { if (p) (void)hipHostFree(p); }

cf_status cf_batch_alloc(cf_classifier *cl, uint64_t maxReads, uint64_t maxWords, cf_batch **out) {
    if (!cl || !out) return CF_ERR_ARG;
    *out = nullptr;
    auto bt = std::make_unique<cf_batch>();
    cf_status st = guard([&] {
        HIP_OK(hipSetDevice(cl->ix->device));
        bt->cl = cl;
        const uint64_t per = maxReads ? (32 * maxWords + maxReads - 1) / maxReads : 0;
        sizeBatch(bt.get(), maxReads & ~1ull, maxWords, 0, (uint32_t)std::min<uint64_t>(per, 128), 0);
        bt->nReads = bt->nQueries = bt->nWords = 0;
    });
    if (st == CF_OK) *out = bt.release();
    return st;
}

cf_status cf_slot_estimate_bytes(uint64_t maxReads, uint64_t maxWords, int khits, int ftabChars, int occPlanes, uint64_t *bytes) {
    if (!bytes || khits < 1 || ftabChars < 1) return CF_ERR_ARG;
    *bytes = 0;
    return guard([&] {
        cf_index ix;
        ix.h.g.ftabChars = ftabChars;
        if (occPlanes) ix.d.planes = reinterpret_cast<const uint8_t *>(&ix);
        cf_classifier cl;
        cl.ix = &ix; cl.d.k = (uint32_t)khits;
        uint64_t total = 0;
        g_dryBytes = &total;
        try {
            cf_batch bt;
            bt.cl = &cl;
            const uint64_t per = maxReads ? (32 * maxWords + maxReads - 1) / maxReads : 0;
            sizeBatch(&bt, maxReads & ~1ull, maxWords, 0, (uint32_t)std::min<uint64_t>(per, 128), 0);
            bt.evInit = false;
        } catch (...) { g_dryBytes = nullptr; throw; }
        g_dryBytes = nullptr;
        *bytes = total;
    });
}

cf_status cf_batch_upload_packed_async(cf_batch *bt, const cf_packed_reads *in, void *streamv) {
    if (!bt || !in) return CF_ERR_ARG;
    return guard([&] {
        HIP_OK(hipSetDevice(bt->cl->ix->device));
        if (bt->running && !bt->finished) throw ArgError("the slot still has a batch in flight: cf_batch_wait first");
        uploadPacked(bt, in, static_cast<hipStream_t>(streamv));
    });
}

cf_status cf_batch_upload_dense_async(cf_batch *bt, const cf_dense_reads *in, void *streamv) {
    if (!bt || !in) return CF_ERR_ARG;
    return guard([&] {
        HIP_OK(hipSetDevice(bt->cl->ix->device));
        if (bt->running && !bt->finished) throw ArgError("the slot still has a batch in flight: cf_batch_wait first");
        uploadDense(bt, in, static_cast<hipStream_t>(streamv));
    });
}

cf_status cf_batch_set_result_format(cf_batch *bt, int format) {
    if (!bt || (format != CF_RESULTS_ROWS && format != CF_RESULTS_NARROW)) return CF_ERR_ARG;
    if (format == CF_RESULTS_NARROW && bt->cl->d.k > 63) { g_err = "the narrow result format holds a query's row count in six bits: -k <= 63"; return CF_ERR_ARG; }
    if (bt->running && !bt->finished) { g_err = "the slot still has a batch in flight: cf_batch_wait first"; return CF_ERR_ARG; }
    return guard([&] {
        HIP_OK(hipSetDevice(bt->cl->ix->device));
        if (format != bt->resultFormat) { bt->finished = false; bt->running = false; bt->downloaded = false; }
        bt->resultFormat = format;
        if (format == CF_RESULTS_NARROW) { bt->qinfo.ensure(bt->nOut.n + 16); bt->hQInfo.ensure(bt->nOut.n + 16); }
    });
}

cf_status cf_classify_async(cf_classifier *cl, cf_batch *bt, void *streamv) {
    if (!cl || !bt || bt->cl != cl) return CF_ERR_ARG;
    return guard([&] {
        HIP_OK(hipSetDevice(cl->ix->device));
        if (!bt->loaded) throw ArgError("no reads were uploaded into this slot");
        hipStream_t st = static_cast<hipStream_t>(streamv);
        bt->rowsStay = false; bt->textDone = false;
        if (!bt->planned) enqueuePlan(bt, st);
        enqueueClassify(bt, st);
    });
}

cf_status cf_batch_reclassify_async(cf_classifier *cl, cf_batch *bt, void *streamv) {
    if (!cl || !bt || bt->cl != cl) return CF_ERR_ARG;
    return guard([&] {
        HIP_OK(hipSetDevice(cl->ix->device));
        if (!bt->loaded) throw ArgError("no reads were uploaded into this slot");
        if (bt->running && !bt->finished) throw ArgError("the slot still has a batch in flight: cf_batch_wait first");
        hipStream_t st = static_cast<hipStream_t>(streamv);
        bt->rowsStay = false; bt->textDone = false;
        enqueuePlan(bt, st);
        enqueueClassify(bt, st);
    });
}

cf_status cf_batch_download_async(cf_batch *bt, void *streamv) {
    if (!bt) return CF_ERR_ARG;
    return guard([&] {
        HIP_OK(hipSetDevice(bt->cl->ix->device));
        if (!bt->running) throw ArgError("cf_classify_async first");
        enqueueDownload(bt, static_cast<hipStream_t>(streamv));
    });
}

cf_status cf_batch_submit(cf_batch *bt, const cf_packed_reads *in, void *streamv) {
    cf_status s = cf_batch_upload_packed_async(bt, in, streamv);
    if (s == CF_OK) s = cf_classify_async(bt->cl, bt, streamv);
    if (s == CF_OK) s = cf_batch_download_async(bt, streamv);
    return s;
}

cf_status cf_batch_wait_narrow(cf_batch *bt, cf_results_narrow *res) {
    if (!bt) return CF_ERR_ARG;
    if (bt->resultFormat != CF_RESULTS_NARROW) { g_err = "cf_batch_wait_narrow on a slot whose result format is not CF_RESULTS_NARROW"; return CF_ERR_ARG; }
    const cf_status rc = guard([&] {
        HIP_OK(hipSetDevice(bt->cl->ix->device));
        if (bt->rowsStay && bt->finished) throw ArgError("the batch was finished by cf_batch_wait_text: its rows were not downloaded");
        waitBatch(bt);
        if (res) {
            static_assert(sizeof(cf_row16) == sizeof(NarrowRow), "cf_row16 layout");
            res->rows = reinterpret_cast<const cf_row16 *>(bt->hRows.p);
            res->qinfo = bt->hQInfo.p; res->score2 = bt->hScore2.p;
            res->n_queries = bt->nQueries; res->total_rows = bt->rowsOut;
            res->planned_sa_rows = bt->rowsTotal; res->row_passes = bt->passes;
            res->slow_post = bt->hSt.p->nSlowPost; res->slow_score = bt->hSt.p->nSlowScore;
        }
    });
    if (rc != CF_OK) {
        (void)hipStreamSynchronize(bt->stream);
        bt->running = false; bt->finished = false;
    }
    return rc;
}

uint32_t cf_narrow_max_score(uint8_t qinfo, uint32_t len1, uint32_t len2, int paired) {
    const uint64_t s0 = len1 > 15 ? (uint64_t)(len1 - 15) * (len1 - 15) : 0u, s1 = len2 > 15 ? (uint64_t)(len2 - 15) * (len2 - 15) : 0u;
    const bool p0 = (qinfo & 0x40u) != 0, p1 = paired && (qinfo & 0x80u) != 0;
    const uint64_t v = (p0 && p1) ? s0 + s1 : p0 ? s0 : p1 ? s1 : 0u;
    return v >= 0xffffffffull ? kMaxScoreNever : (uint32_t)v;
}

// ... 658 lines not shown
```

centrifuge_amd/csrc/cf_kernels.hpp:

```cpp
#pragma once
#include "cf_platform.hpp"

namespace cfamd {

constexpr uint32_t kNone32 = 0xffffffffu;
constexpr uint64_t kNone64 = ~0ull;
constexpr uint32_t kSideChars = 384;
constexpr int kSearchChunk = CF_WAVE;

struct RefInfo { uint64_t tax; uint32_t tidx, pid; };
static_assert(sizeof(RefInfo) == 16, "RefInfo layout");
struct DIndex {
    const uint8_t *sides;
    const uint64_t *ftab, *eftab;
    uint64_t fchr0, fchr1, fchr2, fchr3;
    uint64_t len, zOff, zSide;
    uint32_t zIn;
    int32_t ftabChars, offRate, offw;
    const void *offs;
    const uint8_t *planes;
    const uint8_t *planes2;
    const uint64_t *wide;
    int32_t wideChars;
    const uint64_t *text;
    const uint64_t *saPos;
    const uint64_t *isa;
    int32_t posRate;
    int32_t isaRate;
    uint32_t multiRows, multiMinRun;
    uint32_t verifyMinRun;
    const void *walkOffs;
    int32_t walkRate;
    const uint64_t *boundRow;
    const uint32_t *boundRef;
    const uint32_t *boundBits;
    uint64_t lastBoundary;
    uint32_t nBound;
    int32_t boundShift;
    const uint32_t *posBucket;
    const u64x2 *posFrag, *posSeq;
    uint32_t posShift, nPosFrag, walkMax;
    const RefInfo *refInfo;
    const uint64_t *paths;
    const uint32_t *pathTidx;
    uint32_t nRef, tidxOne;
    int32_t small;
};

struct DParams {
    uint32_t k, m, inc, ihits, rankSlot;
    int32_t traverse;
    const uint8_t *refExcluded;
    const uint64_t *hostSet;
    uint32_t nHostSet;
};

struct Hit {
    uint64_t top, bot;
    uint32_t bwoff, len;
    uint32_t nelt;
};

struct HitP { uint64_t w0, w1; };
constexpr uint64_t kHitPosForm = 1ull << 39, kRowIsPos = 1ull << 63;
CF_DEV uint32_t nhml_make(uint32_t nHits, bool hasLong) { return (nHits & 0x7fffffffu) | (hasLong ? 0x80000000u : 0u); }
CF_DEV uint32_t nhml_n(uint32_t v) { return v & 0x7fffffffu; }
CF_DEV bool nhml_long(uint32_t v) { return (v >> 31) != 0; }
static_assert(sizeof(HitP) == 16, "HitP layout");
constexpr uint64_t kHit40 = (1ull << 40) - 1;
constexpr uint32_t kHit24 = (1u << 24) - 1;
constexpr uint32_t kMaxReadLen = kHit24 - 2;

CF_DEV HitP hit_pack(const Hit &h) {
    const bool dummy = h.top == kNone64;
    const bool pos = !dummy && (h.top & kRowIsPos) != 0;
    const uint64_t size = dummy ? 0 : pos ? (1ull | kHitPosForm) : h.bot - h.top;
    const uint64_t bw = h.bwoff == kNone32 ? (uint64_t)kHit24 : (uint64_t)(h.bwoff & kHit24);
    HitP p;
    p.w0 = (dummy ? kHit40 : (h.top & kHit40)) | ((uint64_t)(h.len & kHit24) << 40);
    p.w1 = (size & kHit40) | (bw << 40);
    return p;
}
CF_DEV uint32_t hp_len(const HitP &p) { return (uint32_t)(p.w0 >> 40); }
CF_DEV uint64_t hp_size(const HitP &p) { return p.w1 & (kHit40 & ~kHitPosForm); }
CF_DEV bool hp_posform(const HitP &p) { return (p.w1 & kHitPosForm) != 0; }
CF_DEV uint32_t hp_bwoff(const HitP &p) { const uint32_t b = (uint32_t)(p.w1 >> 40); return b == kHit24 ? kNone32 : b; }
CF_DEV uint64_t hp_top(const HitP &p) { return p.w0 & kHit40; }
CF_DEV uint64_t hp_row(const HitP &p) { return (p.w0 & kHit40) | (hp_posform(p) ? kRowIsPos : 0ull); }
CF_DEV bool hp_dummy(const HitP &p) { return (p.w0 & kHit40) == kHit40 && (p.w1 & kHit40) == 0; }
CF_DEV void hp_set_len(HitP &p, uint32_t len) { p.w0 = (p.w0 & kHit40) | ((uint64_t)(len & kHit24) << 40); }
CF_DEV void hp_set_bwoff(HitP &p, uint32_t bw) { p.w1 = (p.w1 & kHit40) | ((uint64_t)(bw == kNone32 ? kHit24 : (bw & kHit24)) << 40); }
CF_DEV Hit hit_unpack(const HitP &p) {
    Hit h;
    const bool dummy = hp_dummy(p);
    h.top = dummy ? kNone64 : hp_row(p);
    h.bot = dummy ? kNone64 : hp_row(p) + hp_size(p);
    h.len = hp_len(p); h.bwoff = hp_bwoff(p); h.nelt = 0;
    return h;
}
CF_DEV uint32_t plan_nelt(uint64_t len, uint64_t size, uint64_t maxG, uint64_t m, uint64_t ihits) {
    if (len <= m || size == 0) return 0;
    const uint64_t nelt = size < maxG ? size : maxG;
    return nelt > ihits ? 0u : (uint32_t)nelt;
}

struct PlanHit {
    uint64_t top;
    uint32_t nelt;
    uint32_t meta;
};
CF_DEV uint32_t plan_meta(uint32_t len, int rdi, int f, uint32_t ts) { return (len & 0xffffu) | ((uint32_t)rdi << 16) | ((uint32_t)f << 17) | (ts << 18); }
CF_DEV uint32_t pm_len(uint32_t m) { return m & 0xffffu; }
CF_DEV int pm_rdi(uint32_t m) { return (int)((m >> 16) & 1u); }
CF_DEV int pm_f(uint32_t m) { return (int)((m >> 17) & 1u); }
CF_DEV uint32_t pm_ts(uint32_t m) { return m >> 18; }
constexpr uint32_t kPlanTsMax = (1u << 14) - 1;
constexpr uint32_t kInlinePlan = 4;
constexpr uint32_t kPlanNotInline = 7;

CF_DEV uint32_t qf_make(uint32_t nPlan, uint32_t paired, uint32_t firstMate, uint32_t nMates) { return nPlan | (paired << 3) | (firstMate << 4) | (nMates << 5); }
CF_DEV uint32_t qf_nplan(uint32_t f) { return f & 7u; }
CF_DEV bool qf_paired(uint32_t f) { return (f >> 3) & 1u; }
CF_DEV uint32_t qf_first(uint32_t f) { return (f >> 4) & 1u; }
CF_DEV int qf_nmates(uint32_t f) { return (int)((f >> 5) & 3u); }

struct QHead {
    uint32_t nProc[2][2];
    uint8_t lo[2], hi[2];
    uint8_t brk[2];
    uint8_t pad2[2];
    uint32_t maxG[2][2];
};
static_assert(sizeof(QHead) == 40, "QHead layout");

struct HmEntry {
    uint64_t taxID;
    uint32_t uniqueID, pid;
    uint32_t sc[2][2];
    uint32_t hl[2][2];
    uint32_t ts, score, hitLen, tidx;
    uint8_t rank, pad[7];
};

struct TcEntry { uint64_t tid; uint32_t cnt, tidx; };

struct OutRow { uint64_t taxID; uint32_t uniqueID, score, hitLen, tidx; };
struct NarrowRow { uint32_t uniqueID, tidx, score, hitLen; };
static_assert(sizeof(NarrowRow) == 16, "NarrowRow layout");
constexpr uint32_t kFieldRows = 4;

struct OpCounts { unsigned long long nFtab, nPair, nPair2, nSingle, nWalk, nRows, nFtabWide, nVerify, nTextLoads, nPosHits; };

struct BatchStatus {
    uint32_t nItems;
// ... 184 lines not shown

CF_DEV uint32_t popc_below(uint64_t v, uint32_t o) {
    const uint32_t lo = (uint32_t)v, hi = (uint32_t)(v >> 32);
    const uint32_t klo = o >= 32 ? 0xffffffffu : ((1u << o) - 1u);
    const uint32_t khi = o >= 64 ? 0xffffffffu : (o > 32 ? ((1u << (o - 32)) - 1u) : 0u);
    return (uint32_t)cf_popc32(lo & klo) + (uint32_t)cf_popc32(hi & khi);
}

CF_DEV uint64_t trio_get(const u64x2 &v, uint32_t k) {
    const uint64_t m = (1ull << 40) - 1;
    return k == 0 ? (v.x & m) : k == 1 ? (((v.x >> 40) | (v.y << 24)) & m) : ((v.y >> 16) & m);
}
CF_DEV uint64_t trio_at(const uint64_t *tab, uint64_t i) {
    const uint64_t pc = i / 3;
    return trio_get(cf_load16(reinterpret_cast<const uint8_t *>(tab + 2 * pc)), (uint32_t)(i - 3 * pc));
}
CF_DEV void trio_put(uint64_t *tab, uint64_t i, uint64_t val) {
    const uint64_t pc = i / 3;
    const uint32_t k = (uint32_t)(i - 3 * pc);
    val &= (1ull << 40) - 1;
    uint64_t *w = tab + 2 * pc;
    if (k == 0) { if (val) cf_atomic_or64(w, val); }
    else if (k == 1) { if (val << 40) cf_atomic_or64(w, val << 40); if (val >> 24) cf_atomic_or64(w + 1, val >> 24); }
    else if (val) cf_atomic_or64(w + 1, val << 16);
}
constexpr uint64_t trio_words(uint64_t count) { return 2 * ((count + 2) / 3) + 2; }

template <int G>
CF_DEV void rank_any(const DIndex &ix, int c, uint64_t top, uint64_t bot, uint64_t &t, uint64_t &b, bool &twoSides) {
    if (ix.planes) {
        const u64x2 et = cf_load16(ix.planes + (top >> 6) * 64 + 16 * c);
        t = et.y + popc_below(et.x, (uint32_t)top & 63u);
        twoSides = (bot >> 6) != (top >> 6);
        if (!twoSides) b = et.y + popc_below(et.x, (uint32_t)bot & 63u);
        else { const u64x2 eb = cf_load16(ix.planes + (bot >> 6) * 64 + 16 * c); b = eb.y + popc_below(eb.x, (uint32_t)bot & 63u); }
    } else rank_pair<G>(ix, c, top, bot, t, b, twoSides);
}

CF_DEV bool lf_own_any(const DIndex &ix, uint64_t &row, int &c) {
    if (row == ix.zOff) return false;
    if (ix.planes) {
        const uint8_t *p = ix.planes + (row >> 6) * 64;
        const uint32_t o = (uint32_t)row & 63u;
        const u64x2 e0 = cf_load16(p), e1 = cf_load16(p + 16), e2 = cf_load16(p + 32), e3 = cf_load16(p + 48);
        c = ((e0.x >> o) & 1) ? 0 : ((e1.x >> o) & 1) ? 1 : ((e2.x >> o) & 1) ? 2 : 3;
        const u64x2 e = c == 0 ? e0 : c == 1 ? e1 : c == 2 ? e2 : e3;
        row = e.y + popc_below(e.x, o);
    } else {
        const uint64_t s = row / kSideChars;
        const uint32_t o = (uint32_t)(row - s * kSideChars);
        c = (ix.sides[s * 128 + (o >> 2)] >> (2 * (o & 3))) & 3;
        row = lf_own<1>(ix, row);
    }
    return true;
}

CF_DEV uint64_t ftab_hi(const DIndex &ix, uint64_t i) {
    const uint64_t v = ix.ftab[i];
    return v <= ix.len ? v : ix.eftab[(v ^ kNone64) * 2 + 1];
}
CF_DEV uint64_t ftab_lo(const DIndex &ix, uint64_t i) {
    const uint64_t v = ix.ftab[i];
    return v <= ix.len ? v : ix.eftab[(v ^ kNone64) * 2];
}

struct ReadWin {
    uint64_t w, idx;
    uint32_t m;
};

CF_DEV int strand_char(const DBatch &b, uint64_t wbase, uint32_t L, bool fw, uint32_t j, ReadWin &win) {
    const uint32_t pos = fw ? j : L - 1 - j;
    const uint64_t wi = wbase + (pos >> 5);
    if (wi != win.idx) { win.w = b.bases[wi]; win.m = b.nmask[wi]; win.idx = wi; }
    const uint32_t sh = pos & 31;
    if ((win.m >> sh) & 1u) return 4;
    const int c = (int)((win.w >> (2 * sh)) & 3);
    return fw ? c : (c ^ 3);
}

CF_DEV uint64_t load8_any(const uint8_t *base, uint64_t off) {
    const uint64_t a = off & ~7ull;
    const uint32_t sh = (uint32_t)(off & 7) * 8;
    const uint64_t lo = cf_load8(base + a);
    if (sh == 0) return lo;
    const uint64_t hi = cf_load8(base + a + 8);
    return (lo >> sh) | (hi << (64 - sh));
}
CF_DEV uint64_t nonzero_bytes(uint64_t t) { t |= t >> 4; t |= t >> 2; t |= t >> 1; return t & 0x0101010101010101ull; }
CF_DEV uint64_t bswap64(uint64_t v) {
    v = ((v & 0x00ff00ff00ff00ffull) << 8) | ((v >> 8) & 0x00ff00ff00ff00ffull);
    v = ((v & 0x0000ffff0000ffffull) << 16) | ((v >> 16) & 0x0000ffff0000ffffull);
    return (v << 32) | (v >> 32);
}

CF_DEV void squeeze8(uint64_t x, uint32_t &c16, uint32_t &n8) {
    const uint64_t isN = nonzero_bytes(x & 0xfcfcfcfcfcfcfcfcull);
    uint64_t c = x & 0x0303030303030303ull & ~(isN * 3);
    c = (c | (c >> 6)) & 0x000f000f000f000full;
    c = (c | (c >> 12)) & 0x000000ff000000ffull;
    c = (c | (c >> 24)) & 0xffffull;
    c16 = (uint32_t)c;
    n8 = (uint32_t)((isN * 0x0102040810204080ull) >> 56);
}
CF_DEV uint64_t spread_pairs(uint32_t m) {
    uint64_t x = m;
    x = (x | (x << 16)) & 0x0000ffff0000ffffull;
    x = (x | (x << 8)) & 0x00ff00ff00ff00ffull;
    x = (x | (x << 4)) & 0x0f0f0f0f0f0f0f0full;
    x = (x | (x << 2)) & 0x3333333333333333ull;
    x = (x | (x << 1)) & 0x5555555555555555ull;
    return x * 3;
}
CF_DEV uint64_t pair_reverse(uint64_t x) {
    x = cf_brev64(x);
    return ((x >> 1) & 0x5555555555555555ull) | ((x & 0x5555555555555555ull) << 1);
}

struct DConvert {
    const uint8_t *seq;
    const uint64_t *off;
    const uint64_t *woff;
    uint64_t *bases;
    uint32_t *nmask;
    uint32_t nReads;
};
CF_DEV void convert_body(const DConvert &c, uint32_t r) {
    if (r >= c.nReads) return;
    const uint64_t o = c.off[r], L = c.off[r + 1] - o, wo = c.woff[r];
    for (uint64_t k = 0; 32 * k < L; k++) {
        uint64_t w = 0;
        uint32_t m = 0;
#pragma unroll
        for (uint32_t g = 0; g < 4; g++) {
            const uint64_t j0 = 32 * k + 8 * g;
            if (j0 >= L) break;
            uint64_t x = load8_any(c.seq, o + j0);
            if (L - j0 < 8) x &= (1ull << (8 * (L - j0))) - 1;
            uint32_t c16, n8;
            squeeze8(x, c16, n8);
            w |= (uint64_t)c16 << (16 * g);
            m |= n8 << (8 * g);
        }
        c.bases[wo + k] = w;
        c.nmask[wo + k] = m;
    }
}
struct DUnpack {
    const uint8_t *dense;
    uint64_t *bases;
    uint32_t *rlen;
    uint32_t nReads, readLen;
    uint64_t *rev;
};
CF_DEV void dense_unpack_body(const DUnpack &u, uint64_t t) {
    const uint32_t W = (u.readLen + 31) >> 5, bpr = (u.readLen + 3) >> 2;
    if (W == 0) { if (t < u.nReads) u.rlen[t] = 0; return; }
    const uint64_t r = t / W;
    const uint32_t k = (uint32_t)(t - r * W);
    if (r >= u.nReads) return;
    uint64_t w = load8_any(u.dense, r * bpr + 8ull * k);
    const uint32_t have = u.readLen - 32 * k;
    if (have < 32) w &= (1ull << (2 * have)) - 1;
    u.bases[r * W + k] = w;
    if (k == 0) u.rlen[r] = u.readLen;
    if (u.rev) {
        const uint32_t L = u.readLen;
        const int32_t s0 = (int32_t)(L - 1 - 32u * k) - 31;
        uint64_t x;
        if (s0 >= 0) {
            const uint64_t at = r * bpr + ((uint32_t)s0 >> 2);
            const uint32_t sh = 2u * ((uint32_t)s0 & 3u);
            x = load8_any(u.dense, at) >> sh;
            if (sh) x |= (load8_any(u.dense, at + 8) & 0xffull) << (64 - sh);
        } else x = load8_any(u.dense, r * bpr) << (2 * (uint32_t)(-s0));
        uint64_t rv = pair_reverse(x);
        if (have < 32) rv &= (1ull << (2 * have)) - 1;
        u.rev[r * W + k] = rv;
    }
}

CF_DEV void rlen_body(const uint64_t *off, uint32_t *rlen, uint32_t nReads, uint32_t r) {
    if (r >= nReads) return;
    const uint64_t l = off[r + 1] - off[r];
    rlen[r] = l > 0xffffffffull ? 0xffffffffu : (uint32_t)l;
}

struct DPlan {
    const uint32_t *nmask;
    const uint32_t *rlen;
    const uint64_t *woff;
    uint32_t nReads;
    int32_t ftabChars;
    uint32_t maxLenAllowed;
    uint64_t nWords;
    uint8_t *pass;
    uint32_t *hitCap;
    uint32_t *slotOf;
    uint64_t *hitBase;
    uint32_t *items;
    uint32_t *itemMeta;
    uint64_t *bases;
    uint32_t revDelta;
    BatchStatus *st;
    uint64_t hitsCap;
};

CF_DEV void plan_body(const DPlan &p, uint32_t r) {
    if (r < p.nReads) {
        const uint64_t L = p.rlen[r], wo = p.woff[r];
        uint32_t nN = 0;
        const bool inside = wo + ((L + 31) >> 5) <= p.nWords;
        if (!inside) cf_atomic_or(&p.st->flags, kStWordsOverflow);
        for (uint64_t k = 0; inside && 32 * k < L; k++) {
            uint32_t m = p.nmask[wo + k];
            if (L - 32 * k < 32) m &= (1u << (L - 32 * k)) - 1u;
            nN += (uint32_t)cf_popc32(m);
        }
        const uint64_t maxns = (uint64_t)(0.0 + (double)0.15f * (double)L);
        bool ok = inside && L >= 2 && nN <= maxns;
        if (ok && L > p.maxLenAllowed) { cf_atomic_or(&p.st->flags, kStLenOverflow); ok = false; }
        const uint32_t cap = ok ? (uint32_t)(nN + (L - nN) / (uint64_t)p.ftabChars + 2) : 0u;
        p.pass[r] = ok ? 1 : 0;
        p.hitCap[r] = cap;
    }
}

CF_DEV uint64_t rev_word(const uint64_t *rw, uint32_t L, uint32_t k) {
    const uint32_t have = L - 32u * k;
    const int32_t s0 = (int32_t)(L - 1 - 32u * k) - 31;
    uint64_t x;
    if (s0 >= 0) {
        const uint32_t wi = (uint32_t)s0 >> 5, sh = (uint32_t)s0 & 31;
        x = rw[wi] >> (2 * sh);
        if (sh) x |= rw[wi + 1] << (64 - 2 * sh);
    } else x = rw[0] << (2 * (uint32_t)(-s0));
    uint64_t w = pair_reverse(x);
    if (have < 32) w &= (1ull << (2 * have)) - 1;
    return w;
}

constexpr uint32_t kItemHasN = 0x80000000u;
constexpr uint32_t kItemPre = 0x40000000u;
CF_DEV void plan_fill_body(const DPlan &p, uint32_t r) {
    if (r > p.nReads) return;
    if (r == p.nReads) {
        const uint64_t need = p.hitBase[r];
        p.st->hitsNeed = need;
        if (need > p.hitsCap) { cf_atomic_or(&p.st->flags, kStHitsOverflow); p.st->nItems = 0; }
        else p.st->nItems = 2u * p.slotOf[r];
        return;
    }
    const uint32_t slot = p.slotOf[r];
    if (p.pass[r]) {
        p.items[slot] = r;
        if (p.itemMeta) {
            const uint32_t wo = (uint32_t)p.woff[r], L = p.rlen[r], hb = (uint32_t)p.hitBase[r];
            uint32_t any = 0;
            for (uint32_t k = 0; 32 * k < L; k++) {
                uint32_t mk = p.nmask[p.woff[r] + k];
                if (L - 32 * k < 32) mk &= (1u << (L - 32 * k)) - 1u;
                any |= mk;
            }
            const bool pre = p.revDelta && !any;
            const uint32_t Lf = L | (any ? kItemHasN : 0u) | (pre ? kItemPre : 0u);
            uint32_t *m = p.itemMeta + 8 * (size_t)slot;
            m[0] = pre ? wo + p.revDelta : wo; m[1] = Lf; m[2] = hb; m[3] = r;
            m[4] = wo; m[5] = Lf; m[6] = hb + p.hitCap[r]; m[7] = r;
        }
    } else p.slotOf[r] = kNone32;
}

CF_DEV void rev_words_body(const DPlan &p, uint32_t wordsPerRead, uint64_t t) {
    const uint64_t r = t / wordsPerRead;
    const uint32_t k = (uint32_t)(t - r * wordsPerRead);
    if (r >= p.nReads || !p.revDelta || !p.pass[r]) return;
    const uint32_t L = p.rlen[r];
    if (32u * k >= L) return;
    const uint64_t wo = p.woff[r];
    p.bases[wo + p.revDelta + k] = rev_word(p.bases + wo, L, k);
}

constexpr uint32_t kMaxScoreNever = 0xffffffffu;
CF_DEV void plan_maxscore_body(const uint32_t *rlen, const uint8_t *pass, uint32_t nQueries, int paired, uint32_t *maxScore, uint32_t q) {
    if (q >= nQueries) return;
    const uint32_t r0 = paired ? 2 * q : q;
    const uint64_t L0 = rlen[r0];
    const uint64_t s0 = L0 > 15 ? (L0 - 15) * (L0 - 15) : 0u;
    const bool p0 = pass[r0] != 0;
    uint64_t v = p0 ? s0 : 0u;
    if (paired) {
        const uint64_t L1 = rlen[r0 + 1];
        const uint64_t s1 = L1 > 15 ? (L1 - 15) * (L1 - 15) : 0u;
        const bool p1 = pass[r0 + 1] != 0;
        v = (p0 && p1) ? s0 + s1 : p0 ? s0 : p1 ? s1 : 0u;
    }
    maxScore[q] = v >= 0xffffffffull ? kMaxScoreNever : (uint32_t)v;
}

struct DCompact {
    const OutRow *out;
    const uint64_t *o1tax, *o1a, *o1b;
    uint64_t oStride;
    const uint32_t *nOut;
    const uint64_t *rowFirst;
    uint32_t k, nQueries;
    OutRow *dst;
    BatchStatus *st;
    NarrowRow *dstNarrow;
    uint8_t *qinfo;
    const uint8_t *pass;
    int32_t paired;
};
CF_DEV OutRow row_of_one(uint64_t tax, uint64_t a, uint64_t bb) {
    OutRow o; o.taxID = tax; o.uniqueID = (uint32_t)a; o.score = (uint32_t)(a >> 32); o.hitLen = (uint32_t)bb; o.tidx = (uint32_t)(bb >> 32);
    return o;
}
CF_DEV void compact_body(const DCompact &c, uint32_t q) {
    if (q == c.nQueries && c.st) c.st->rowsOut = c.rowFirst[q];
    if (q >= c.nQueries) return;
    const uint32_t n = c.nOut[q] < c.k ? c.nOut[q] : c.k;
    const uint64_t f = c.rowFirst[q];
    if (c.dstNarrow) {
        if (n <= kFieldRows) {
#pragma unroll
            for (uint32_t i = 0; i < kFieldRows; i++) if (i < n) {
                const uint64_t a = c.o1a[i * c.oStride + q], bb = c.o1b[i * c.oStride + q];
                c.dstNarrow[f + i] = NarrowRow{(uint32_t)a, (uint32_t)(bb >> 32), (uint32_t)(a >> 32), (uint32_t)bb};
            }
        } else for (uint32_t i = 0; i < n; i++) { const OutRow o = c.out[(uint64_t)q * c.k + i]; c.dstNarrow[f + i] = NarrowRow{o.uniqueID, o.tidx, o.score, o.hitLen}; }
        const uint32_t r0 = c.paired ? 2 * q : q;
        c.qinfo[q] = (uint8_t)(n | (c.pass[r0] ? 0x40u : 0u) | ((c.paired && c.pass[r0 + 1]) ? 0x80u : 0u));
        return;
    }
    if (n <= kFieldRows) {
#pragma unroll
        for (uint32_t i = 0; i < kFieldRows; i++) if (i < n) c.dst[f + i] = row_of_one(c.o1tax[i * c.oStride + q], c.o1a[i * c.oStride + q], c.o1b[i * c.oStride + q]);
    } else for (uint32_t i = 0; i < n; i++) c.dst[f + i] = c.out[(uint64_t)q * c.k + i];
}

CF_DEV int ps_begin(const DIndex &ix, const DBatch &b, uint64_t wbase, uint32_t L, bool fw, uint32_t cur,
                    ReadWin &win, uint64_t &top, uint64_t &bot, uint32_t &dep, uint32_t &len, uint32_t &newCur,
                    bool &usedFtab) {
    const uint32_t ftc = (uint32_t)ix.ftabChars;
    const uint32_t left = L - cur;
    usedFtab = false;
    if (left < ftc) { len = L - cur; newCur = L; return 0; }
    uint64_t fi = 0;
    for (uint32_t i = 0; i < ftc; i++) {
        const int c = strand_char(b, wbase, L, fw, L - cur - 1 - i, win);
        if (c > 3) { len = i + 1; newCur = cur + i + 1; return 0; }
        fi |= (uint64_t)c << (2 * i);
    }
    usedFtab = true;
    top = ftab_hi(ix, fi);
    bot = ftab_lo(ix, fi + 1);
    dep = cur + ftc;
    if (bot <= top) { len = ftc; newCur = dep; return 0; }
    return 1;
}

enum : int { MODE_IDLE = 0, MODE_CALL = 1, MODE_EXT = 2 };

template <int G>
CF_DEV void search_body(const DIndex &ix, const DParams &pr, const DBatch &b) {
    const int sub = Grp<G>::sub();
    const uint32_t lane = cf_lane();
    const uint32_t leaderLane = lane & ~(uint32_t)(G - 1);
    int mode = MODE_IDLE;
    uint32_t item = 0, L = 0, cur = 0, offset = 0, dep = 0, nh = 0, mxl = 0;
    uint64_t wbase = 0, top = 0, bot = 0;
    bool fw = true;
    HitP *hl = nullptr;
    ReadWin win{0, kNone64, 0};
    const uint32_t nItems = b.st->nItems;
    uint32_t wnext = 0, wend = 0;
    bool exhausted = false;
    unsigned long long cFtab = 0, cPair = 0, cPair2 = 0, cSingle = 0;

    for (;;) {
        const uint64_t idleMask = cf_ballot(mode == MODE_IDLE && sub == 0);
        if (idleMask) {
            if (wnext >= wend && !exhausted) {
                uint32_t base = 0;
                if (lane == 0) base = (uint32_t)cf_atomic_add(&b.cursor[0], (unsigned long long)kSearchChunk);
                base = cf_first_lane_u32(base);
                if (base >= nItems) { exhausted = true; wnext = wend = 0; }
                else { wnext = base; wend = base + kSearchChunk < nItems ? base + kSearchChunk : nItems; }
            }
            const uint32_t avail = wend - wnext;
            const uint32_t nIdle = (uint32_t)cf_popc64(idleMask);
            if (mode == MODE_IDLE) {
                const uint32_t rnk = (uint32_t)cf_popc64(idleMask & ((1ull << leaderLane) - 1));
                if (rnk < avail) {
                    item = wnext + rnk;
                    const uint32_t rd = b.items[item >> 1];
                    fw = (item & 1) == 0;
                    wbase = b.woff[rd];
                    L = b.rlen[rd];
                    hl = b.hits + b.hitBase[rd] + (fw ? 0u : b.hitCap[rd]);
                    cur = 0; nh = 0; mxl = 0; win.idx = kNone64;
                    mode = MODE_CALL;
                }
            }
            wnext += nIdle < avail ? nIdle : avail;
        }
        if (cf_ballot(mode != MODE_IDLE) == 0) {
            if (exhausted) break;
            continue;
        }
        bool push = false;
        uint64_t pTop = kNone64, pBot = kNone64;
        uint32_t pLen = 0;
        if (mode == MODE_CALL) {
            offset = cur;
            uint32_t len = 0, newCur = 0;
            bool usedFtab;
            const int r = ps_begin(ix, b, wbase, L, fw, cur, win, top, bot, dep, len, newCur, usedFtab);
            if (usedFtab) cFtab++;
            if (r == 0) { push = true; pLen = len; cur = newCur; }
            else mode = MODE_EXT;
        }
        if (mode == MODE_EXT) {
            bool stop = dep >= L;
            if (!stop) {
                const int c = strand_char(b, wbase, L, fw, L - dep - 1, win);
                if (c > 3) stop = true;
                else {
                    uint64_t t, bb; bool two;
                    if (bot - top > 1) { cPair++; } else { cSingle++; }
                    rank_any<G>(ix, c, top, bot, t, bb, two);
                    if (two) cPair2++;
                    if (bb <= t) stop = true;
                    else { top = t; bot = bb; dep++; stop = dep >= L; }
                }
            }
            if (stop) { push = true; pTop = top; pBot = bot; pLen = dep - offset; cur = dep; }
        }
        if (push) {
            if (sub == 0) {
                Hit h; h.top = pTop; h.bot = pBot; h.bwoff = offset; h.len = pLen; h.nelt = 0;
                hl[nh] = hit_pack(h);
            }
            nh++;
            mxl = pLen > mxl ? pLen : mxl;
            bool done = cur >= L;
            if (!done) {
                if (pLen > pr.inc) cur += 1;
                done = cur + pr.m >= L;
            }
            if (done) {
                if (sub == 0) b.nhml[item] = nhml_make(nh, mxl >= pr.m);
                mode = MODE_IDLE;
            } else mode = MODE_CALL;
        }
    }
    if (b.ops && sub == 0 && (cFtab | cPair | cSingle)) {
        cf_atomic_add(&b.ops->nFtab, cFtab); cf_atomic_add(&b.ops->nPair, cPair);
        cf_atomic_add(&b.ops->nPair2, cPair2); cf_atomic_add(&b.ops->nSingle, cSingle);
    }
}


constexpr int rec_bytes(int W) { return ((12 * W + 16 + 31) / 32) * 32; }
constexpr int rec_lds_stride(int W) { return rec_bytes(W) + 8; }

CF_DEV bool pack_word(const DBatch &b, uint32_t item, uint32_t k, uint64_t &w, uint32_t &m, uint32_t *meta) {
    if (item >= b.st->nItems) return false;
    const uint32_t rd = b.items[item >> 1];
    const bool fw = (item & 1) == 0;
    const uint64_t wo = b.woff[rd];
    const uint32_t L = b.rlen[rd];
    w = 0; m = 0;
    if (32 * k < L) {
        const uint32_t have = L - 32 * k;
        if (fw) {
            const int32_t s0 = (int32_t)(L - 1 - 32 * k) - 31;
            uint64_t x;
            uint32_t mm;
            if (s0 >= 0) {
                const uint32_t wi = (uint32_t)s0 >> 5, sh = (uint32_t)s0 & 31;
                x = b.bases[wo + wi] >> (2 * sh);
                mm = b.nmask[wo + wi] >> sh;
                if (sh) { x |= b.bases[wo + wi + 1] << (64 - 2 * sh); mm |= b.nmask[wo + wi + 1] << (32 - sh); }
            } else {
                const uint32_t neg = (uint32_t)(-s0);
                x = b.bases[wo] << (2 * neg);
                mm = b.nmask[wo] << neg;
            }
            w = pair_reverse(x);
            m = cf_brev32(mm);
// ... 903 lines not shown
    }
    a[first + hole] = val;
}
CF_DEV void ss_adjust_heap(HitP *a, int first, int hole, int len, const HitP &val) {
    const int top = hole;
    int child = hole;
    while (child < (len - 1) / 2) {
        child = 2 * (child + 1);
        if (hit_less(a[first + child], a[first + (child - 1)])) child--;
        a[first + hole] = a[first + child]; hole = child;
    }
    if ((len & 1) == 0 && child == (len - 2) / 2) {
        child = 2 * (child + 1);
        a[first + hole] = a[first + (child - 1)]; hole = child - 1;
    }
    ss_push_heap(a, first, hole, top, val);
}
CF_DEV void ss_heapsort(HitP *a, int first, int last) {
    const int len = last - first;
    if (len >= 2) {
        int parent = (len - 2) / 2;
        for (;;) { const HitP v = a[first + parent]; ss_adjust_heap(a, first, parent, len, v); if (parent == 0) break; parent--; }
    }
    while (last - first > 1) {
        --last;
        const HitP v = a[last]; a[last] = a[first];
        ss_adjust_heap(a, first, 0, last - first, v);
    }
}
CF_DEV void std_sort_hits(HitP *a, int n) {
    if (n <= 1) return;
    int lg = 0;
    for (int t = n; t > 1; t >>= 1) lg++;
    int stF[48], stL[48], stD[48], sp = 0;
    int first = 0, last = n, depth = 2 * lg;
    for (;;) {
        while (last - first > 16) {
            if (depth == 0) { ss_heapsort(a, first, last); break; }
            --depth;
            const int mid = first + (last - first) / 2;
            {
                const int x = first + 1, y = mid, z = last - 1;
                if (hit_less(a[x], a[y])) {
                    if (hit_less(a[y], a[z])) hit_swap(a[first], a[y]);
                    else if (hit_less(a[x], a[z])) hit_swap(a[first], a[z]);
                    else hit_swap(a[first], a[x]);
                } else if (hit_less(a[x], a[z])) hit_swap(a[first], a[x]);
                else if (hit_less(a[y], a[z])) hit_swap(a[first], a[z]);
                else hit_swap(a[first], a[y]);
            }
            int lo = first + 1, hi = last;
            for (;;) {
                while (hit_less(a[lo], a[first])) ++lo;
                --hi;
                while (hit_less(a[first], a[hi])) --hi;
                if (!(lo < hi)) break;
                hit_swap(a[lo], a[hi]);
                ++lo;
            }
            if (sp < 48) { stF[sp] = lo; stL[sp] = last; stD[sp] = depth; sp++; }
            last = lo;
        }
        if (sp == 0) break;
        --sp; first = stF[sp]; last = stL[sp]; depth = stD[sp];
    }
    if (n > 16) {
        ss_insertion(a, 0, 16);
        for (int i = 16; i != n; ++i) ss_linear_insert(a, i);
    } else ss_insertion(a, 0, n);
}

CF_DEV void hit_reset(HitP &h) { Hit z; z.top = z.bot = 0; z.bwoff = kNone32; z.len = 0; z.nelt = 0; h = hit_pack(z); }

CF_DEV void post_trim(HitP *h, uint32_t n) {
    if (n < 2) return;
    for (uint32_t i = 0; i + 1 < n; i++) {
        for (uint32_t j = i + 1; j < n; j++) {
            const uint32_t bi = hp_bwoff(h[i]), bj = hp_bwoff(h[j]), li = hp_len(h[i]), lj = hp_len(h[j]);
            if (bi >= bj) { hp_set_len(h[i], 0); break; }
            if ((uint64_t)bi + li <= bj) break;
            if (li >= lj) {
                const uint32_t e = bj + lj;
                hp_set_bwoff(h[j], bi + li); hp_set_len(h[j], e - (bi + li));
            } else hp_set_len(h[i], bj - bi);
        }
    }
}

CF_DEV void post_fix(const DIndex &ix, const DParams &pr, const DBatch &b, uint32_t rd, HitP *const hs[2], const uint32_t n[2]) {
    const uint64_t wbase = b.woff[rd], m = pr.m;
    const uint32_t L = b.rlen[rd];
    uint64_t sum[2] = {0, 0};
    for (int f = 0; f < 2; f++) for (uint32_t i = 0; i < n[f]; i++) if (hp_len(hs[f][i]) >= m) sum[f] += hp_len(hs[f][i]);
    if (sum[0] >= m && sum[1] >= m) {
        for (uint32_t i = 0; i < n[0]; i++) {
            HitP &hit = hs[0][i];
            const uint64_t len = hp_len(hit), l = hp_bwoff(hit), r = l + len;
            for (uint32_t j = 0; j < n[1]; j++) {
                HitP &rc = hs[1][j];
                const uint64_t rclen = hp_len(rc);
                if (len < m && rclen < m) continue;
                const uint64_t rc_l = (uint64_t)L - hp_bwoff(rc) - rclen, rc_r = rc_l + rclen;
                if (r <= rc_l) continue;
                if (rc_r <= l) continue;
                if (l == rc_l && r == rc_r) continue;
                if (l < rc_l && r > rc_r) continue;
                if (l > rc_l && r < rc_r) continue;
                if (l > rc_l) {
                    Hit t; ps_whole<1>(ix, b, wbase, L, true, (uint32_t)rc_l, t);
                    if (t.len == len + l - rc_l) hit = hit_pack(t);
                }
                if (r > rc_r) {
                    Hit t; ps_whole<1>(ix, b, wbase, L, false, (uint32_t)(L - r), t);
                    if (t.len == rclen + r - rc_r) rc = hit_pack(t);
                }
            }
        }
        for (uint32_t i = 0; i < n[0]; i++) {
            HitP &hit = hs[0][i];
            const uint64_t len = hp_len(hit), l = hp_bwoff(hit), r = l + len;
            for (uint32_t j = 0; j < n[1]; j++) {
                HitP &rc = hs[1][j];
                const uint64_t rclen = hp_len(rc), rc_l = (uint64_t)L - hp_bwoff(rc) - rclen, rc_r = rc_l + rclen;
                if (rc_l < l) break;
                if (len != rclen) continue;
                if (l == rc_l && r == rc_r && hp_size(hit) + hp_size(rc) > pr.ihits) {
                    hit_reset(hit); hit_reset(rc); break;
                }
            }
        }
    }
    post_trim(hs[0], n[0]);
    post_trim(hs[1], n[1]);
}
CF_DEV void post_fix(const DIndex &ix, const DParams &pr, const DBatch &b, uint32_t rd) {
    const uint32_t slot = b.slotOf[rd];
    HitP *hs[2] = {b.hits + b.hitBase[rd], b.hits + b.hitBase[rd] + b.hitCap[rd]};
    const uint32_t n[2] = {nhml_n(b.nhml[2 * slot]), nhml_n(b.nhml[2 * slot + 1])};
    post_fix(ix, pr, b, rd, hs, n);
}

CF_DEV void hits_copy(HitP *dst, const HitP *src, uint32_t n) {
    uint32_t i = 0;
    for (; i + 4 <= n; i += 4) { const HitP a = src[i], b2 = src[i + 1], c = src[i + 2], d = src[i + 3]; dst[i] = a; dst[i + 1] = b2; dst[i + 2] = c; dst[i + 3] = d; }
    for (; i < n; i++) dst[i] = src[i];
}

CF_DEV void post_body(const DIndex &ix, const DParams &pr, const DBatch &b, uint32_t q, HitP *scratch = nullptr, uint32_t scratchCap = 0) {
    if (b.st->flags & kStHitsOverflow) { b.qRows[q] = 0; return; }
    QHead qi;
    for (int a = 0; a < 2; a++) { qi.lo[a] = qi.hi[a] = 0; qi.nProc[a][0] = qi.nProc[a][1] = 0; qi.brk[a] = 0; qi.pad2[a] = 0; qi.maxG[a][0] = qi.maxG[a][1] = 0; }
    uint32_t nPlanned = 0;
    const uint32_t r0 = b.paired ? 2 * q : q;
    const bool p0 = b.pass[r0] != 0, p1 = b.paired ? b.pass[r0 + 1] != 0 : false;
    uint32_t rds[2] = {r0, r0 + 1};
    int nm;
    uint32_t isPaired = 0, firstMate = 0;
    if (b.paired && p0 && p1) { nm = 2; isPaired = 1; }
    else if (p0) nm = 1;
    else if (p1) { nm = 1; rds[0] = r0 + 1; firstMate = 1; }
    else nm = 0;
    const uint64_t k = pr.k, m = pr.m;
    uint64_t maxG = k;
    uint32_t rowsTotal = 0;
    uint32_t tsBase = 0;
    bool tsWide = false;
    for (int rdi = 0; rdi < nm; rdi++) {
        const uint32_t rd = rds[rdi], slot = b.slotOf[rd];
        HitP *const pool[2] = {b.hits + b.hitBase[rd], b.hits + b.hitBase[rd] + b.hitCap[rd]};
        HitP *hs[2] = {pool[0], pool[1]};
        const uint32_t hm0 = b.nhml[2 * slot], hm1 = b.nhml[2 * slot + 1];
        const uint32_t n[2] = {nhml_n(hm0), nhml_n(hm1)};
        const bool long0 = nhml_long(hm0), long1 = nhml_long(hm1);
        if (!long0 && !long1) continue;
        const uint32_t need = (long0 ? n[0] : 0u) + (long1 ? n[1] : 0u);
        const bool staged = scratch != nullptr && need <= scratchCap;
        if (staged) {
            hs[0] = scratch; hs[1] = scratch + (long0 ? n[0] : 0u);
            if (long0) hits_copy(hs[0], pool[0], n[0]);
            if (long1) hits_copy(hs[1], pool[1], n[1]);
        }
        if (long0 && long1) post_fix(ix, pr, b, rd, hs, n);
        else post_trim(hs[long0 ? 0 : 1], n[long0 ? 0 : 1]);
        uint64_t tot[2] = {0, 0}, mx[2] = {0, 0};
        for (int f = 0; f < 2; f++) if (f == 0 ? long0 : long1) for (uint32_t i = 0; i < n[f]; i++) {
            const uint64_t len = hp_len(hs[f][i]);
            if (len < m) continue;
            tot[f] += (len - 15) * (len - 15);
            if (len > mx[f]) mx[f] = len;
        }
        int lo, hi;
        if (tot[0] != tot[1]) { lo = tot[0] > tot[1] ? 0 : 1; hi = lo + 1; }
        else if (mx[0] != mx[1]) { lo = mx[0] > mx[1] ? 0 : 1; hi = lo + 1; }
        else { lo = 0; hi = 2; }
        qi.lo[rdi] = (uint8_t)lo; qi.hi[rdi] = (uint8_t)hi;
        for (int f = lo; f < hi; f++) {
            HitP *h = hs[f];
            for (uint32_t i = 0; i < n[f]; i++)
                if (hp_len(h[i]) >= m && hp_size(h[i]) > maxG) maxG = hp_size(h[i]);
            if (maxG > k) maxG += k;
            qi.maxG[rdi][f] = maxG > 0xffffffffull ? 0xffffffffu : (uint32_t)maxG;
            std_sort_hits(h, (int)n[f]);
            uint64_t cnt = 0;
            uint32_t i = 0;
            for (; i < n[f]; i++) {
                const uint64_t len = hp_len(h[i]), size = hp_size(h[i]);
                const uint64_t nelt = plan_nelt(len, size, maxG, m, pr.ihits);
                if (nelt == 0) continue;
                if (nPlanned < kInlinePlan) {
                    PlanHit ph;
                    ph.top = hp_row(h[i]); ph.nelt = (uint32_t)nelt; ph.meta = plan_meta((uint32_t)len, rdi, f, tsBase + i);
                    if (tsBase + i > kPlanTsMax || len > 0xffffu) tsWide = true;
                    b.qplan[(uint64_t)nPlanned * b.qplanStride + q] = ph;
                }
                nPlanned++;
                rowsTotal += (uint32_t)nelt;
                cnt += nelt;
                if (cnt >= maxG) { i++; qi.brk[rdi] |= (uint8_t)(1u << f); break; }
            }
            qi.nProc[rdi][f] = i;
            tsBase += i - ((qi.brk[rdi] >> f) & 1u);
            if (staged) hits_copy(pool[f], h, n[f]);
        }
    }
    const uint32_t nPlan = (nPlanned <= kInlinePlan && !tsWide) ? nPlanned : kPlanNotInline;
    b.qflag[q] = qf_make(nPlan, isPaired, firstMate, (uint32_t)nm);
    if (nPlan == kPlanNotInline) b.qhead[q] = qi;
    b.qRows[q] = rowsTotal;
}

CF_DEV void defer_push(uint32_t *list, uint32_t *counter, bool defer, uint32_t q) {
    const uint64_t mask = cf_ballot(defer);
    if (!mask) return;
    const uint32_t lane = cf_lane();
    const int leader = cf_ctz64(mask);
    uint32_t base = 0;
    if ((int)lane == leader) base = cf_atomic_add(counter, (uint32_t)cf_popc64(mask));
    base = cf_shfl(base, leader);
    if (defer) list[base + (uint32_t)cf_popc64(mask & ((1ull << lane) - 1))] = q;
}

constexpr int kPostFastHits = 8;
CF_DEV bool post_fast_body(const DIndex &ix, const DParams &pr, const DBatch &b, uint32_t q) {
    (void)ix;
    if (b.st->flags & kStHitsOverflow) { b.qRows[q] = 0; return false; }
    uint32_t fOf0 = 2, fOf1 = 2, np0 = 0, np1 = 0, brk0 = 0, brk1 = 0;
    uint8_t isPaired = 0, firstMate = 0;
    const uint32_t r0 = b.paired ? 2 * q : q;
    const bool p0 = b.pass[r0] != 0, p1 = b.paired ? b.pass[r0 + 1] != 0 : false;
    uint32_t rd0 = r0;
    int nm;
    if (b.paired && p0 && p1) { nm = 2; isPaired = 1; }
    else if (p0) nm = 1;
    else if (p1) { nm = 1; rd0 = r0 + 1; firstMate = 1; }
    else nm = 0;
    const uint64_t k = pr.k, m = pr.m;
    uint64_t maxG = k;
    uint32_t rowsTotal = 0, tsBase = 0, nPlanned = 0;
    PlanHit pl0{0, 0, 0}, pl1{0, 0, 0}, pl2{0, 0, 0}, pl3{0, 0, 0};
    static_assert(kInlinePlan == 4, "four plan slots below");
    bool defer = false;
    for (int rdi = 0; rdi < nm && !defer; rdi++) {
        const uint32_t rd = rd0 + (uint32_t)rdi, slot = b.slotOf[rd];
        const uint32_t hm0 = b.nhml[2 * slot], hm1 = b.nhml[2 * slot + 1];
        const bool long0 = nhml_long(hm0), long1 = nhml_long(hm1);
        if (!long0 && !long1) continue;
        if (long0 && long1) { defer = true; break; }
        const int f = long0 ? 0 : 1;
        const uint32_t n = nhml_n(f ? hm1 : hm0);
        if (n > (uint32_t)kPostFastHits) { defer = true; break; }
        const uint8_t *hp = reinterpret_cast<const uint8_t *>(b.hits + b.hitBase[rd] + (f ? b.hitCap[rd] : 0u));
        uint64_t w0[kPostFastHits], w1[kPostFastHits];
#pragma unroll
        for (int i = 0; i < kPostFastHits; i++) {
            u64x2 v{0, 0};
            if ((uint32_t)i < n) v = cf_load16(hp + 16 * i);
            w0[i] = v.x; w1[i] = v.y;
        }
        bool apart = true;
        uint64_t mg = maxG;
#pragma unroll
        for (int i = 0; i < kPostFastHits; i++) {
            if ((uint32_t)i >= n) continue;
            const HitP hi{w0[i], w1[i]};
            const uint64_t len = hp_len(hi), size = hp_size(hi);
            if (len >= m && size > mg) mg = size;
            if (i + 1 < kPostFastHits && (uint32_t)(i + 1) < n) {
                const HitP hj{w0[i + 1], w1[i + 1]};
                const uint64_t bi = hp_bwoff(hi), bj = hp_bwoff(hj);
                if (bi >= bj || bi + len > bj) apart = false;
            }
        }
        if (!apart) { defer = true; break; }
        maxG = mg;
        if (maxG > k) maxG += k;
        uint32_t rank[kPostFastHits];
#pragma unroll
        for (int i = 0; i < kPostFastHits; i++) rank[i] = 0;
#pragma unroll
        for (int i = 0; i < kPostFastHits; i++) {
#pragma unroll
            for (int j = i + 1; j < kPostFastHits; j++) {
                if ((uint32_t)j < n) {
                    const bool jFirst = hit_less(HitP{w0[j], w1[j]}, HitP{w0[i], w1[i]});
                    rank[i] += jFirst ? 1u : 0u;
                    rank[j] += jFirst ? 0u : 1u;
                }
            }
        }
        uint64_t cnt = 0;
        uint32_t visited = n;
        bool stopped = false, brk = false;
#pragma unroll
        for (int r = 0; r < kPostFastHits; r++) {
            if ((uint32_t)r >= n || stopped) continue;
            uint64_t c0 = 0, c1 = 0;
#pragma unroll
            for (int i = 0; i < kPostFastHits; i++) if ((uint32_t)i < n && rank[i] == (uint32_t)r) { c0 = w0[i]; c1 = w1[i]; }
            const HitP c{c0, c1};
            const uint64_t len = hp_len(c), size = hp_size(c);
            uint64_t nelt = 0;
            if (!(len <= m || size == 0)) {
                nelt = size < maxG ? size : maxG;
                if (nelt > pr.ihits) nelt = 0;
            }
            if (nelt == 0) continue;
            const PlanHit ph{hp_row(c), (uint32_t)nelt, plan_meta((uint32_t)len, rdi, f, tsBase + (uint32_t)r)};
            if (tsBase + (uint32_t)r > kPlanTsMax || len > 0xffffu) defer = true;
            if (nPlanned == 0) pl0 = ph; else if (nPlanned == 1) pl1 = ph; else if (nPlanned == 2) pl2 = ph; else if (nPlanned == 3) pl3 = ph;
            nPlanned++;
            rowsTotal += (uint32_t)nelt;
            cnt += nelt;
            if (cnt >= maxG) { visited = (uint32_t)r + 1; brk = true; stopped = true; }
        }
        if (rdi == 0) { fOf0 = (uint32_t)f; np0 = visited; brk0 = brk ? 1u : 0u; }
        else { fOf1 = (uint32_t)f; np1 = visited; brk1 = brk ? 1u : 0u; }
        tsBase += visited - (brk ? 1u : 0u);
    }
    if (defer || nPlanned > kInlinePlan) return true;
    (void)np0; (void)np1; (void)brk0; (void)brk1; (void)fOf0; (void)fOf1;
    b.qflag[q] = qf_make(nPlanned, isPaired, firstMate, (uint32_t)nm);
    if (nPlanned > 0) b.qplan[q] = pl0;
    if (nPlanned > 1) b.qplan[b.qplanStride + q] = pl1;
    if (nPlanned > 2) b.qplan[2 * b.qplanStride + q] = pl2;
    if (nPlanned > 3) b.qplan[3 * b.qplanStride + q] = pl3;
    b.qRows[q] = rowsTotal;
    return false;
}

CF_DEV void row_window_body(const DBatch &b, uint32_t qLo, bool keepSlow = false) {
    BatchStatus &st = *b.st;
    const uint32_t nq = b.nQueries;
    st.rowsTotal = b.qBase[nq];
    st.needRows = 0;
    if (!keepSlow) st.nSlowScore = 0;
    if (st.flags & kStHitsOverflow) { st.qLo = st.qHi = 0; st.rowLo = st.rowHi = 0; return; }
    if (qLo > nq) qLo = nq;
    const uint64_t rowLo = b.qBase[qLo];
    uint32_t lo = qLo, hi = nq;
    while (lo < hi) {
        const uint32_t md = lo + (hi - lo + 1) / 2;
        if (b.qBase[md] - rowLo <= b.rowsCap) lo = md; else hi = md - 1;
    }
    if (lo == qLo && qLo < nq) st.needRows = b.qBase[qLo + 1] - rowLo;
    st.qLo = qLo; st.qHi = lo;
    st.rowLo = rowLo; st.rowHi = b.qBase[lo];
}

template <typename Put>
CF_DEV void for_each_planned_row(const DParams &pr, const DBatch &b, uint32_t q, Put put) {
    if (q < b.st->qLo || q >= b.st->qHi) return;
    const uint32_t nRows = b.qRows[q];
    if (nRows == 0) return;
    const uint32_t qf = b.qflag[q], nPlan = qf_nplan(qf);
    const uint64_t base = b.qBase[q] - b.st->rowLo;
    uint32_t rowoff = 0;
    if (nPlan != kPlanNotInline) {
#pragma unroll
        for (uint32_t j = 0; j < kInlinePlan; j++) {
            if (j >= nPlan) continue;
            const PlanHit ph = b.qplan[(uint64_t)j * b.qplanStride + q];
            for (uint32_t e = 0; e < ph.nelt; e++) put(base + rowoff + e, ph.top + e);
            rowoff += ph.nelt;
        }
        return;
    }
    const QHead *qp = &b.qhead[q];
    const uint32_t r0 = (b.paired ? 2 * q : q) + qf_first(qf);
    const int nMates = qf_nmates(qf);
    for (int rdi = 0; rdi < nMates; rdi++) {
        const uint32_t rd = r0 + rdi;
        const int lo = qp->lo[rdi], hi = qp->hi[rdi];
        for (int f = lo; f < hi; f++) {
            const HitP *h = b.hits + b.hitBase[rd] + (f ? b.hitCap[rd] : 0u);
            const uint32_t np = qp->nProc[rdi][f];
            const uint64_t mg = qp->maxG[rdi][f];
            for (uint32_t i = 0; i < np; i++) {
                const HitP hp = h[i];
                const uint32_t ne = plan_nelt(hp_len(hp), hp_size(hp), mg, pr.m, pr.ihits);
                for (uint32_t e = 0; e < ne; e++) put(base + rowoff + e, hp_row(hp) + e);
                rowoff += ne;
            }
// ... 759 lines not shown
```

centrifuge_amd/csrc/cf_scan.hpp:

```cpp
#pragma once
#include <hip/hip_runtime.h>

#include <cstdint>

namespace cfamd {

enum : int { SCAN_WORDS = 0, SCAN_PLAIN = 1, SCAN_HITS = 2 };
constexpr int kScanBlock = 256, kScanPer = 16, kScanTile = kScanBlock * kScanPer;

template <int MODE>
__device__ __forceinline__ uint64_t scan_value(uint32_t x) {
    return MODE == SCAN_WORDS ? (((uint64_t)x + 31) >> 5) : MODE == SCAN_HITS ? 2ull * x : (uint64_t)x;
}

__device__ __forceinline__ void scan_load(const uint32_t *in, uint64_t n, uint64_t first, uint32_t (&x)[kScanPer]) {
    if (first + kScanPer <= n) {
        const uint4 *p = reinterpret_cast<const uint4 *>(in + first);
#pragma unroll
        for (int i = 0; i < kScanPer / 4; i++) { const uint4 v = p[i]; x[4 * i] = v.x; x[4 * i + 1] = v.y; x[4 * i + 2] = v.z; x[4 * i + 3] = v.w; }
    } else {
#pragma unroll
        for (int i = 0; i < kScanPer; i++) x[i] = first + i < n ? in[first + i] : 0u;
    }
}

__device__ __forceinline__ void scan_block_reduce(uint64_t &a, uint32_t &c, uint64_t *ldsA, uint32_t *ldsC) {
#pragma unroll
    for (int m = 32; m > 0; m >>= 1) { a += __shfl_xor(a, m, 64); c += __shfl_xor(c, m, 64); }
    const int w = threadIdx.x >> 6;
    if ((threadIdx.x & 63) == 0) { ldsA[w] = a; ldsC[w] = c; }
    __syncthreads();
    a = 0; c = 0;
#pragma unroll
    for (int i = 0; i < kScanBlock / 64; i++) { a += ldsA[i]; c += ldsC[i]; }
}

template <int MODE>
__global__ void __launch_bounds__(kScanBlock) k_scan_sums(const uint32_t *in, uint64_t n, uint64_t *tileA, uint32_t *tileC) {
    __shared__ uint64_t ldsA[kScanBlock / 64];
    __shared__ uint32_t ldsC[kScanBlock / 64];
    uint32_t x[kScanPer];
    scan_load(in, n, (uint64_t)blockIdx.x * kScanTile + (uint64_t)threadIdx.x * kScanPer, x);
    uint64_t a = 0;
    uint32_t c = 0;
#pragma unroll
    for (int i = 0; i < kScanPer; i++) { a += scan_value<MODE>(x[i]); if (MODE == SCAN_HITS) c += x[i] != 0; }
    scan_block_reduce(a, c, ldsA, ldsC);
    if (threadIdx.x == 0) { tileA[blockIdx.x] = a; if (MODE == SCAN_HITS) tileC[blockIdx.x] = c; }
}

__global__ void __launch_bounds__(kScanBlock) k_scan_tiles(uint64_t *tileA, uint32_t *tileC, uint32_t nTiles, bool withC) {
    __shared__ uint64_t sA[kScanBlock];
    __shared__ uint32_t sC[kScanBlock];
    uint64_t carryA = 0;
    uint32_t carryC = 0;
    for (uint32_t base = 0; base < nTiles; base += kScanBlock) {
        const uint32_t i = base + threadIdx.x;
        const uint64_t a = i < nTiles ? tileA[i] : 0;
        const uint32_t c = (withC && i < nTiles) ? tileC[i] : 0;
        sA[threadIdx.x] = a; sC[threadIdx.x] = c;
        __syncthreads();
        for (int d = 1; d < kScanBlock; d <<= 1) {
            const uint64_t ta = threadIdx.x >= (unsigned)d ? sA[threadIdx.x - d] : 0;
            const uint32_t tc = threadIdx.x >= (unsigned)d ? sC[threadIdx.x - d] : 0;
            __syncthreads();
            sA[threadIdx.x] += ta; sC[threadIdx.x] += tc;
            __syncthreads();
        }
        if (i < nTiles) { tileA[i] = carryA + sA[threadIdx.x] - a; if (withC) tileC[i] = carryC + sC[threadIdx.x] - c; }
        carryA += sA[kScanBlock - 1]; carryC += sC[kScanBlock - 1];
        __syncthreads();
    }
}

template <int MODE>
__global__ void __launch_bounds__(kScanBlock) k_scan_write(const uint32_t *in, uint64_t n, const uint64_t *tileA, const uint32_t *tileC,
                                                            uint64_t *outA, uint32_t *outC) {
    __shared__ uint64_t ldsA[kScanBlock / 64];
    __shared__ uint32_t ldsC[kScanBlock / 64];
    const uint64_t first = (uint64_t)blockIdx.x * kScanTile + (uint64_t)threadIdx.x * kScanPer;
    uint32_t x[kScanPer];
    scan_load(in, n, first, x);
    uint64_t a = 0;
    uint32_t c = 0;
#pragma unroll
    for (int i = 0; i < kScanPer; i++) { a += scan_value<MODE>(x[i]); if (MODE == SCAN_HITS) c += x[i] != 0; }
    uint64_t ia = a;
    uint32_t ic = c;
    const int lane = threadIdx.x & 63, w = threadIdx.x >> 6;
#pragma unroll
    for (int d = 1; d < 64; d <<= 1) {
        const uint64_t ta = __shfl_up(ia, d, 64);
        const uint32_t tc = __shfl_up(ic, d, 64);
        if (lane >= d) { ia += ta; ic += tc; }
    }
    if (lane == 63) { ldsA[w] = ia; ldsC[w] = ic; }
    __syncthreads();
    uint64_t offA = tileA[blockIdx.x] + ia - a;
    uint32_t offC = (MODE == SCAN_HITS ? tileC[blockIdx.x] : 0u) + ic - c;
    for (int i = 0; i < w; i++) { offA += ldsA[i]; offC += ldsC[i]; }
#pragma unroll
    for (int i = 0; i < kScanPer; i++) {
        const uint64_t idx = first + i;
        if (idx <= n) { outA[idx] = offA; if (MODE == SCAN_HITS) outC[idx] = offC; }
        offA += scan_value<MODE>(x[i]);
        if (MODE == SCAN_HITS) offC += x[i] != 0;
    }
}

inline uint32_t scan_tiles_for(uint64_t n) { return (uint32_t)((n + 1 + kScanTile - 1) / kScanTile); }

template <int MODE>
inline void scan_enqueue(const uint32_t *in, uint64_t n, uint64_t *outA, uint32_t *outC, uint64_t *tileA, uint32_t *tileC, hipStream_t st) {
    const uint32_t tiles = scan_tiles_for(n);
    hipLaunchKernelGGL((k_scan_sums<MODE>), dim3(tiles), dim3(kScanBlock), 0, st, in, n, tileA, tileC);
    hipLaunchKernelGGL(k_scan_tiles, dim3(1), dim3(kScanBlock), 0, st, tileA, tileC, tiles, MODE == SCAN_HITS);
    hipLaunchKernelGGL((k_scan_write<MODE>), dim3(tiles), dim3(kScanBlock), 0, st, in, n, (const uint64_t *)tileA, (const uint32_t *)tileC, outA, outC);
}

}
```

Measured before the change: 1.433 billion.

## Fuse plan and compact passes into tiled scan kernels, skip word-offset scan for uniform reads

The per-read plan, hit-cap scan and plan-fill steps become one two-pass tiled scan: sums, tile scan, then a write pass that redoes the per-read plan and stages offsets in LDS. Compaction is likewise fused into the scan write pass, and the max-score kernel is folded into the plan. For dense uniform-length input, word offsets are written during unpack and the rlen/woff scan kernels are skipped. This removes several kernel launches and global round trips for intermediate arrays, at the cost of recomputing the plan in both scan passes and more complex LDS staging.

```diff
diff --git a/centrifuge_amd/csrc/cf_device.hip b/centrifuge_amd/csrc/cf_device.hip
--- a/centrifuge_amd/csrc/cf_device.hip
+++ b/centrifuge_amd/csrc/cf_device.hip
@@ -223,15 +223,26 @@
     __shared__ uint32_t slots[3 * kCountSlots];
     count_body(b, slots, blockIdx.x, slotBits, direct);
 }
-__global__ void __launch_bounds__(256) k_plan(DPlan p) { plan_body(p, cf_global_thread()); }
-__global__ void __launch_bounds__(256) k_plan_fill(DPlan p) { plan_fill_body(p, cf_global_thread()); }
+struct PlanScan {
+    static constexpr bool kWithC = true;
+    DPlan p;
+    __device__ void sums(uint64_t tile0, uint32_t t, uint64_t &a, uint32_t &c) const { plan_sums_thread(p, tile0, t, a, c); }
+    __device__ void load(uint64_t first, uint32_t (&x)[kScanPer], uint64_t &a, uint32_t &c) const { plan_write_load(p, first, x, a, c); }
+    __device__ void stage(const uint32_t (&x)[kScanPer], uint32_t t, uint64_t offA, uint32_t offC, uint64_t *sA, uint32_t *sC) const { plan_write_stage(x, t, offA, offC, sA, sC); }
+    __device__ void write(uint64_t tile0, uint32_t t, const uint64_t *sA, const uint32_t *sC) const { plan_write_thread(p, tile0, t, sA, sC); }
+};
+__global__ void __launch_bounds__(kScanBlock) k_plan_sums(PlanScan f, uint64_t *tileA, uint32_t *tileC) { scan_sums_tile(f, tileA, tileC); }
+__global__ void __launch_bounds__(kScanBlock) k_plan_write(PlanScan f, const uint64_t *tileA, const uint32_t *tileC) { scan_write_tile(f, tileA, tileC); }
 __global__ void __launch_bounds__(256) k_rev_words(DPlan p, uint32_t wordsPerRead) { rev_words_body(p, wordsPerRead, (uint64_t)blockIdx.x * blockDim.x + threadIdx.x); }
-__global__ void __launch_bounds__(256) k_plan_maxscore(const uint32_t *rlen, const uint8_t *pass, uint32_t nQueries, int paired, uint32_t *maxScore) {
-    plan_maxscore_body(rlen, pass, nQueries, paired, maxScore, cf_global_thread());
-}
-__global__ void __launch_bounds__(256) k_compact(DCompact c) {
-    compact_body(c, cf_global_thread());
-}
+struct CompactScan {
+    static constexpr bool kWithC = false;
+    DCompact c;
+    uint64_t *rowFirst;
+    __device__ void load(uint64_t first, uint32_t (&x)[kScanPer], uint64_t &a, uint32_t &cc) const { compact_write_load(c, first, x, a); cc = 0; }
+    __device__ void stage(const uint32_t (&x)[kScanPer], uint32_t t, uint64_t offA, uint32_t, uint64_t *sA, uint32_t *) const { compact_write_stage(x, t, offA, sA); }
+    __device__ void write(uint64_t tile0, uint32_t t, const uint64_t *sA, const uint32_t *) const { compact_write_thread(c, rowFirst, tile0, t, sA); }
+};
+__global__ void __launch_bounds__(kScanBlock) k_compact_write(CompactScan f, const uint64_t *tileA) { scan_write_tile(f, tileA, nullptr); }
 __global__ void __launch_bounds__(256) k_text_count(DTextMark m) { text_count_body(m, (uint64_t)blockIdx.x * blockDim.x + threadIdx.x); }
 __global__ void __launch_bounds__(256) k_text_mark(DTextMark m) { text_mark_body(m, (uint64_t)blockIdx.x * blockDim.x + threadIdx.x); }
 __global__ void __launch_bounds__(256) k_text_records(DTextRec d) { text_record_body(d, cf_global_thread()); }
@@ -394,6 +405,7 @@
     DevBuf<QHead> qhead;
     DevBuf<uint64_t> o1tax, o1a, o1b;
     DevBuf<uint8_t> dense;
+    uint32_t uniformLen = 0;
     uint32_t densePending = 0;
     DevBuf<uint8_t> qinfo;
     DevBuf<uint8_t> postDeferred;
@@ -1365,6 +1377,7 @@
     pl.itemMeta = bt->selfRecords ? bt->itemMeta.p : nullptr;
     pl.bases = bt->bases.p; pl.revDelta = bt->revDelta;
     pl.hitsCap = bt->hitsCapLimit ? std::min<uint64_t>(bt->hitsCapLimit, bt->hits.n) : bt->hits.n;
+    pl.maxScore = bt->nQueries ? bt->maxScore.p : nullptr; pl.nQueries = (uint32_t)bt->nQueries; pl.paired = bt->paired;
     DBatch &d = bt->d;
     d.bases = bt->bases.p; d.nmask = bt->nmask.p; d.rlen = bt->rlen.p; d.woff = bt->woff.p; d.seeds = bt->seeds.p;
     d.pass = bt->pass.p; d.items = bt->items.p; d.slotOf = bt->slotOf.p; d.hitBase = bt->hitBase.p; d.hitCap = bt->hitCap.p;
@@ -1386,11 +1399,12 @@
 
 static void enqueuePlan(cf_batch *bt, hipStream_t st) {
     const uint64_t nReads = bt->nReads;
-    const DPlan &pl = bt->pl;
+    DPlan &pl = bt->pl;
+    pl.uniformLen = bt->uniformLen;
     HIP_OK(hipStreamWaitEvent(st, bt->ev[8], 0));
     if (bt->densePending) {
         const uint32_t L = bt->densePending - 1;
-        const DUnpack u{bt->dense.p, bt->bases.p, bt->rlen.p, (uint32_t)nReads, L, bt->revDelta ? bt->bases.p + bt->revDelta : nullptr};
+        const DUnpack u{bt->dense.p, bt->bases.p, bt->rlen.p, (uint32_t)nReads, L, bt->revDelta ? bt->bases.p + bt->revDelta : nullptr, bt->woff.p};
         bt->revMade = bt->revDelta != 0;
         const uint64_t threads = nReads * std::max<uint64_t>(((uint64_t)L + 31) >> 5, 1);
         hipLaunchKernelGGL(k_dense_unpack, dim3((unsigned)((threads + 255) / 256)), dim3(256), 0, st, u);
@@ -1399,25 +1413,29 @@
     HIP_OK(hipEventRecord(bt->ev[5], st));
     HIP_OK(hipMemsetAsync(bt->st.p, 0, sizeof(BatchStatus), st));
     const dim3 gp((unsigned)((nReads + 1 + 255) / 256)), bl(256);
-    if (bt->fromBytes && nReads) hipLaunchKernelGGL(k_rlen, gp, bl, 0, st, bt->off8.p, bt->rlen.p, (uint32_t)nReads);
-    scan_enqueue<SCAN_WORDS>(bt->rlen.p, nReads, bt->woff.p, nullptr, bt->tileA.p, bt->tileC.p, st);
-    if (bt->fromBytes && nReads) {
-        DConvert c{bt->seq.p, bt->off8.p, bt->woff.p, bt->bases.p, bt->nmask.p, (uint32_t)nReads};
-        hipLaunchKernelGGL(k_convert, dim3((unsigned)((nReads + 255) / 256)), dim3(256), 0, st, c);
-    }
-    if (bt->fromText && nReads) {
-        const DTextPack c{bt->text.p, bt->txSeqOff.p, bt->rlen.p, bt->woff.p, bt->bases.p, bt->nmask.p, (uint32_t)nReads};
-        hipLaunchKernelGGL(k_text_pack, dim3((unsigned)((nReads + 255) / 256)), dim3(256), 0, st, c);
-    }
-    hipLaunchKernelGGL(k_plan, gp, bl, 0, st, pl);
-    scan_enqueue<SCAN_HITS>(bt->hitCap.p, nReads, bt->hitBase.p, bt->slotOf.p, bt->tileA.p, bt->tileC.p, st);
-    hipLaunchKernelGGL(k_plan_fill, gp, bl, 0, st, pl);
+    if (!bt->uniformLen) {
+        if (bt->fromBytes && nReads) hipLaunchKernelGGL(k_rlen, gp, bl, 0, st, bt->off8.p, bt->rlen.p, (uint32_t)nReads);
+        scan_enqueue<SCAN_WORDS>(bt->rlen.p, nReads, bt->woff.p, nullptr, bt->tileA.p, bt->tileC.p, st);
+        if (bt->fromBytes && nReads) {
+            DConvert c{bt->seq.p, bt->off8.p, bt->woff.p, bt->bases.p, bt->nmask.p, (uint32_t)nReads};
+            hipLaunchKernelGGL(k_convert, dim3((unsigned)((nReads + 255) / 256)), dim3(256), 0, st, c);
+        }
+        if (bt->fromText && nReads) {
+            const DTextPack c{bt->text.p, bt->txSeqOff.p, bt->rlen.p, bt->woff.p, bt->bases.p, bt->nmask.p, (uint32_t)nReads};
+            hipLaunchKernelGGL(k_text_pack, dim3((unsigned)((nReads + 255) / 256)), dim3(256), 0, st, c);
+        }
+    }
+    {
+        const uint32_t tiles = scan_tiles_for(nReads);
+        const PlanScan f{pl};
+        hipLaunchKernelGGL(k_plan_sums, dim3(tiles), dim3(kScanBlock), 0, st, f, bt->tileA.p, bt->tileC.p);
+        hipLaunchKernelGGL(k_scan_tiles, dim3(1), dim3(kScanBlock), 0, st, bt->tileA.p, bt->tileC.p, tiles, true);
+        hipLaunchKernelGGL(k_plan_write, dim3(tiles), dim3(kScanBlock), 0, st, f, (const uint64_t *)bt->tileA.p, (const uint32_t *)bt->tileC.p);
+    }
     if (pl.revDelta && nReads && !bt->revMade) {
         const uint64_t threads = nReads * (uint64_t)bt->recWords;
         hipLaunchKernelGGL(k_rev_words, dim3((unsigned)((threads + 255) / 256)), bl, 0, st, pl, bt->recWords);
     }
-    if (bt->nQueries) hipLaunchKernelGGL(k_plan_maxscore, dim3((unsigned)((bt->nQueries + 255) / 256)), bl, 0, st, bt->rlen.p, bt->pass.p,
-                                         (uint32_t)bt->nQueries, bt->paired, bt->maxScore.p);
     if (bt->recWords && !bt->selfRecords && nReads) {
         const uint64_t threads = 2 * nReads * (uint64_t)bt->recWords;
         hipLaunchKernelGGL(k_pack, dim3((unsigned)((threads + 255) / 256)), bl, 0, st, bt->d, bt->recs.p, bt->recWords);
@@ -1490,12 +1508,13 @@
 
 static void enqueueCompact(cf_batch *bt, hipStream_t st) {
     const uint32_t nq = (uint32_t)bt->nQueries;
-    const dim3 g((nq + 1 + 255) / 256), bl(256);
-    scan_enqueue<SCAN_PLAIN>(bt->nOut.p, nq, bt->rowFirst.p, nullptr, bt->tileA.p, bt->tileC.p, st);
+    const uint32_t tiles = scan_tiles_for(nq);
     const bool narrow = bt->resultFormat == CF_RESULTS_NARROW;
     const DCompact c{bt->out.p, bt->o1tax.p, bt->o1a.p, bt->o1b.p, bt->d.oStride, bt->nOut.p, bt->rowFirst.p, (uint32_t)bt->cl->d.k, nq, bt->outCompact.p, bt->st.p,
                      narrow ? reinterpret_cast<NarrowRow *>(bt->outCompact.p) : nullptr, bt->qinfo.p, bt->pass.p, bt->paired};
-    hipLaunchKernelGGL(k_compact, g, bl, 0, st, c);
+    hipLaunchKernelGGL((k_scan_sums<SCAN_PLAIN>), dim3(tiles), dim3(kScanBlock), 0, st, (const uint32_t *)bt->nOut.p, (uint64_t)nq, bt->tileA.p, bt->tileC.p);
+    hipLaunchKernelGGL(k_scan_tiles, dim3(1), dim3(kScanBlock), 0, st, bt->tileA.p, bt->tileC.p, tiles, false);
+    hipLaunchKernelGGL(k_compact_write, dim3(tiles), dim3(kScanBlock), 0, st, CompactScan{c, bt->rowFirst.p}, (const uint64_t *)bt->tileA.p);
 }
 
 static void enqueueClassify(cf_batch *bt, hipStream_t st) {
@@ -1645,7 +1664,7 @@
     }
     if (nReads) HIP_OK(hipMemcpyAsync(bt->seeds.p, seeds, nReads * 4, hipMemcpyHostToDevice, st));
     HIP_OK(hipEventRecord(bt->ev[8], st));
-    bt->fromBytes = true; bt->fromText = false; bt->densePending = 0; bt->revMade = false; bt->nmaskZeroOf = nullptr;
+    bt->fromBytes = true; bt->fromText = false; bt->densePending = 0; bt->uniformLen = 0; bt->revMade = false; bt->nmaskZeroOf = nullptr;
     bt->loaded = true; bt->planned = false; bt->running = false; bt->finished = false;
 }
 
@@ -1684,7 +1703,7 @@
         HIP_OK(hipMemcpyAsync(bt->seeds.p, in->seeds, in->n_reads * 4, hipMemcpyHostToDevice, st));
     }
     HIP_OK(hipEventRecord(bt->ev[8], st));
-    bt->fromBytes = false; bt->fromText = false; bt->densePending = 0; bt->revMade = false;
+    bt->fromBytes = false; bt->fromText = false; bt->densePending = 0; bt->uniformLen = 0; bt->revMade = false;
     bt->loaded = true; bt->planned = false; bt->running = false; bt->finished = false;
 }
 
@@ -1704,6 +1723,7 @@
         if (nWords) uploadSparseMask(bt, in->nword_idx, in->nword_mask, in->n_nwords, nWords, st);
     }
     bt->densePending = in->n_reads ? in->read_len + 1 : 0; bt->revMade = false;
+    bt->uniformLen = bt->densePending;
     HIP_OK(hipEventRecord(bt->ev[8], st));
     bt->fromBytes = false; bt->fromText = false;
     bt->loaded = true; bt->planned = false; bt->running = false; bt->finished = false;
@@ -1769,7 +1789,7 @@
     sizeBatch(bt, nReads, ts.words(), ts.bases(), ts.maxLen, nBlocks == 2);
     bindBatch(bt);
     HIP_OK(hipEventRecord(bt->ev[8], st));
-    bt->fromText = true; bt->fromBytes = false; bt->densePending = 0; bt->revMade = false; bt->nmaskZeroOf = nullptr;
+    bt->fromText = true; bt->fromBytes = false; bt->densePending = 0; bt->uniformLen = 0; bt->revMade = false; bt->nmaskZeroOf = nullptr;
     bt->textFastq = !fasta;
     bt->loaded = true;
     info->n_reads = nReads; info->n_bases = ts.bases(); info->max_len = ts.maxLen;
@@ -1866,7 +1886,7 @@
     sizeBatch(bt, nq, ts.words(), ts.bases(), ts.maxLen, false);
     bindBatch(bt);
     HIP_OK(hipEventRecord(bt->ev[8], st));
-    bt->fromText = true; bt->fromBytes = false; bt->densePending = 0; bt->revMade = false; bt->nmaskZeroOf = nullptr;
+    bt->fromText = true; bt->fromBytes = false; bt->densePending = 0; bt->uniformLen = 0; bt->revMade = false; bt->nmaskZeroOf = nullptr;
     bt->textFastq = !fasta;
     bt->loaded = true;
     info->n_reads = nq; info->n_bases = ts.bases(); info->max_len = ts.maxLen;
@@ -1998,7 +2018,7 @@
     sizeBatch(bt, 2 * nq, ts.words(), ts.bases(), ts.maxLen, true);
     bindBatch(bt);
     HIP_OK(hipEventRecord(bt->ev[8], st));
-    bt->fromText = true; bt->fromBytes = false; bt->densePending = 0; bt->revMade = false; bt->nmaskZeroOf = nullptr;
+    bt->fromText = true; bt->fromBytes = false; bt->densePending = 0; bt->uniformLen = 0; bt->revMade = false; bt->nmaskZeroOf = nullptr;
     bt->textFastq = !fasta;
     bt->loaded = true;
     info->n_reads = 2 * nq; info->n_bases = ts.bases(); info->max_len = ts.maxLen;
diff --git a/centrifuge_amd/csrc/cf_kernels.hpp b/centrifuge_amd/csrc/cf_kernels.hpp
--- a/centrifuge_amd/csrc/cf_kernels.hpp
+++ b/centrifuge_amd/csrc/cf_kernels.hpp
@@ -1,5 +1,6 @@
 #pragma once
 #include "cf_platform.hpp"
+#include "cf_tile.hpp"
 
 namespace cfamd {
 
@@ -490,10 +491,11 @@
     uint32_t *rlen;
     uint32_t nReads, readLen;
     uint64_t *rev;
+    uint64_t *woff;
 };
 CF_DEV void dense_unpack_body(const DUnpack &u, uint64_t t) {
     const uint32_t W = (u.readLen + 31) >> 5, bpr = (u.readLen + 3) >> 2;
-    if (W == 0) { if (t < u.nReads) u.rlen[t] = 0; return; }
+    if (W == 0) { if (t < u.nReads) { u.rlen[t] = 0; if (u.woff) { u.woff[t] = 0; if (t + 1 == u.nReads) u.woff[t + 1] = 0; } } return; }
     const uint64_t r = t / W;
     const uint32_t k = (uint32_t)(t - r * W);
     if (r >= u.nReads) return;
@@ -501,7 +503,10 @@
     const uint32_t have = u.readLen - 32 * k;
     if (have < 32) w &= (1ull << (2 * have)) - 1;
     u.bases[r * W + k] = w;
-    if (k == 0) u.rlen[r] = u.readLen;
+    if (k == 0) {
+        u.rlen[r] = u.readLen;
+        if (u.woff) { u.woff[r] = r * W; if (r + 1 == u.nReads) u.woff[r + 1] = (r + 1) * W; }
+    }
     if (u.rev) {
         const uint32_t L = u.readLen;
         const int32_t s0 = (int32_t)(L - 1 - 32u * k) - 31;
@@ -542,25 +547,40 @@
     uint32_t revDelta;
     BatchStatus *st;
     uint64_t hitsCap;
+    uint32_t uniformLen;
+    uint32_t *maxScore;
+    uint32_t nQueries;
+    int32_t paired;
 };
-
+CF_DEV uint64_t plan_len(const DPlan &p, uint64_t r) { return p.uniformLen ? (uint64_t)(p.uniformLen - 1) : (uint64_t)p.rlen[r]; }
+CF_DEV uint64_t plan_woff(const DPlan &p, uint64_t r) { return p.uniformLen ? r * (((uint64_t)p.uniformLen + 30) >> 5) : p.woff[r]; }
+
+constexpr uint8_t kPassOk = 1, kPassHasN = 2;
+
+struct PlanOne { bool ok; uint32_t cap; bool anyN; };
+CF_DEV PlanOne plan_one(const DPlan &p, uint64_t L, uint64_t wo) {
+    uint32_t nN = 0;
+    const bool inside = wo + ((L + 31) >> 5) <= p.nWords;
+    if (!inside) cf_atomic_or(&p.st->flags, kStWordsOverflow);
+    for (uint64_t k = 0; inside && 32 * k < L; k++) {
+        uint32_t m = p.nmask[wo + k];
+        if (L - 32 * k < 32) m &= (1u << (L - 32 * k)) - 1u;
+        nN += (uint32_t)cf_popc32(m);
+    }
+    const uint64_t maxns = (uint64_t)(0.0 + (double)0.15f * (double)L);
+    bool ok = inside && L >= 2 && nN <= maxns;
+    if (ok && L > p.maxLenAllowed) { cf_atomic_or(&p.st->flags, kStLenOverflow); ok = false; }
+    PlanOne o;
+    o.ok = ok;
+    o.cap = ok ? (uint32_t)(nN + (L - nN) / (uint64_t)p.ftabChars + 2) : 0u;
+    o.anyN = ok && nN != 0;
+    return o;
+}
 CF_DEV void plan_body(const DPlan &p, uint32_t r) {
     if (r < p.nReads) {
-        const uint64_t L = p.rlen[r], wo = p.woff[r];
-        uint32_t nN = 0;
-        const bool inside = wo + ((L + 31) >> 5) <= p.nWords;
-        if (!inside) cf_atomic_or(&p.st->flags, kStWordsOverflow);
-        for (uint64_t k = 0; inside && 32 * k < L; k++) {
-            uint32_t m = p.nmask[wo + k];
-            if (L - 32 * k < 32) m &= (1u << (L - 32 * k)) - 1u;
-            nN += (uint32_t)cf_popc32(m);
-        }
-        const uint64_t maxns = (uint64_t)(0.0 + (double)0.15f * (double)L);
-        bool ok = inside && L >= 2 && nN <= maxns;
-        if (ok && L > p.maxLenAllowed) { cf_atomic_or(&p.st->flags, kStLenOverflow); ok = false; }
-        const uint32_t cap = ok ? (uint32_t)(nN + (L - nN) / (uint64_t)p.ftabChars + 2) : 0u;
-        p.pass[r] = ok ? 1 : 0;
-        p.hitCap[r] = cap;
+        const PlanOne o = plan_one(p, p.rlen[r], p.woff[r]);
+        p.pass[r] = o.ok ? kPassOk : 0;
+        p.hitCap[r] = o.cap;
     }
 }
 
@@ -580,39 +600,40 @@
 
 constexpr uint32_t kItemHasN = 0x80000000u;
 constexpr uint32_t kItemPre = 0x40000000u;
+CF_DEV void plan_fill_total(const DPlan &p, uint64_t need, uint32_t nSlots) {
+    p.st->hitsNeed = need;
+    if (need > p.hitsCap) { cf_atomic_or(&p.st->flags, kStHitsOverflow); p.st->nItems = 0; }
+    else p.st->nItems = 2u * nSlots;
+}
+CF_DEV void plan_fill_one(const DPlan &p, uint32_t r, uint32_t L, uint32_t wo, bool any, uint32_t cap, uint32_t slot, uint32_t hb) {
+    p.items[slot] = r;
+    if (p.itemMeta) {
+        const bool pre = p.revDelta && !any;
+        const uint32_t Lf = L | (any ? kItemHasN : 0u) | (pre ? kItemPre : 0u);
+        uint32_t *m = p.itemMeta + 8 * (size_t)slot;
+        m[0] = pre ? wo + p.revDelta : wo; m[1] = Lf; m[2] = hb; m[3] = r;
+        m[4] = wo; m[5] = Lf; m[6] = hb + cap; m[7] = r;
+    }
+}
 CF_DEV void plan_fill_body(const DPlan &p, uint32_t r) {
     if (r > p.nReads) return;
-    if (r == p.nReads) {
-        const uint64_t need = p.hitBase[r];
-        p.st->hitsNeed = need;
-        if (need > p.hitsCap) { cf_atomic_or(&p.st->flags, kStHitsOverflow); p.st->nItems = 0; }
-        else p.st->nItems = 2u * p.slotOf[r];
-        return;
-    }
-    const uint32_t slot = p.slotOf[r];
-    if (p.pass[r]) {
-        p.items[slot] = r;
-        if (p.itemMeta) {
-            const uint32_t wo = (uint32_t)p.woff[r], L = p.rlen[r], hb = (uint32_t)p.hitBase[r];
-            uint32_t any = 0;
-            for (uint32_t k = 0; 32 * k < L; k++) {
-                uint32_t mk = p.nmask[p.woff[r] + k];
-                if (L - 32 * k < 32) mk &= (1u << (L - 32 * k)) - 1u;
-                any |= mk;
-            }
-            const bool pre = p.revDelta && !any;
-            const uint32_t Lf = L | (any ? kItemHasN : 0u) | (pre ? kItemPre : 0u);
-            uint32_t *m = p.itemMeta + 8 * (size_t)slot;
-            m[0] = pre ? wo + p.revDelta : wo; m[1] = Lf; m[2] = hb; m[3] = r;
-            m[4] = wo; m[5] = Lf; m[6] = hb + p.hitCap[r]; m[7] = r;
-        }
+    if (r == p.nReads) { plan_fill_total(p, p.hitBase[r], p.slotOf[r]); return; }
+    if (p.pass[r] & kPassOk) {
+        const uint64_t L = p.rlen[r], wo = p.woff[r];
+        uint32_t any = 0;
+        for (uint32_t k = 0; p.itemMeta && 32 * k < L; k++) {
+            uint32_t mk = p.nmask[wo + k];
+            if (L - 32 * k < 32) mk &= (1u << (L - 32 * k)) - 1u;
+            any |= mk;
+        }
+        plan_fill_one(p, r, (uint32_t)L, (uint32_t)wo, any != 0, p.hitCap[r], p.slotOf[r], (uint32_t)p.hitBase[r]);
     } else p.slotOf[r] = kNone32;
 }
 
 CF_DEV void rev_words_body(const DPlan &p, uint32_t wordsPerRead, uint64_t t) {
     const uint64_t r = t / wordsPerRead;
     const uint32_t k = (uint32_t)(t - r * wordsPerRead);
-    if (r >= p.nReads || !p.revDelta || !p.pass[r]) return;
+    if (r >= p.nReads || !p.revDelta || !(p.pass[r] & kPassOk)) return;
     const uint32_t L = p.rlen[r];
     if (32u * k >= L) return;
     const uint64_t wo = p.woff[r];
@@ -620,20 +641,67 @@
 }
 
 constexpr uint32_t kMaxScoreNever = 0xffffffffu;
+CF_DEV uint32_t plan_maxscore_one(uint64_t L0, bool p0, uint64_t L1, bool p1, bool paired) {
+    const uint64_t s0 = L0 > 15 ? (L0 - 15) * (L0 - 15) : 0u;
+    uint64_t v = p0 ? s0 : 0u;
+    if (paired) {
+        const uint64_t s1 = L1 > 15 ? (L1 - 15) * (L1 - 15) : 0u;
+        v = (p0 && p1) ? s0 + s1 : p0 ? s0 : p1 ? s1 : 0u;
+    }
+    return v >= 0xffffffffull ? kMaxScoreNever : (uint32_t)v;
+}
 CF_DEV void plan_maxscore_body(const uint32_t *rlen, const uint8_t *pass, uint32_t nQueries, int paired, uint32_t *maxScore, uint32_t q) {
     if (q >= nQueries) return;
     const uint32_t r0 = paired ? 2 * q : q;
-    const uint64_t L0 = rlen[r0];
-    const uint64_t s0 = L0 > 15 ? (L0 - 15) * (L0 - 15) : 0u;
-    const bool p0 = pass[r0] != 0;
-    uint64_t v = p0 ? s0 : 0u;
-    if (paired) {
-        const uint64_t L1 = rlen[r0 + 1];
-        const uint64_t s1 = L1 > 15 ? (L1 - 15) * (L1 - 15) : 0u;
-        const bool p1 = pass[r0 + 1] != 0;
-        v = (p0 && p1) ? s0 + s1 : p0 ? s0 : p1 ? s1 : 0u;
-    }
-    maxScore[q] = v >= 0xffffffffull ? kMaxScoreNever : (uint32_t)v;
+    maxScore[q] = plan_maxscore_one(rlen[r0], (pass[r0] & kPassOk) != 0, paired ? rlen[r0 + 1] : 0u, paired && (pass[r0 + 1] & kPassOk) != 0, paired != 0);
+}
+
+CF_DEV void plan_sums_thread(const DPlan &p, uint64_t tile0, uint32_t t, uint64_t &a, uint32_t &c) {
+    a = 0; c = 0;
+    for (int i = 0; i < kScanPer; i++) {
+        const uint64_t r = tile0 + (uint64_t)i * kScanBlock + t;
+        if (r >= p.nReads) break;
+        const PlanOne o = plan_one(p, plan_len(p, r), plan_woff(p, r));
+        p.pass[r] = (uint8_t)(o.ok ? (o.anyN ? kPassOk | kPassHasN : kPassOk) : 0);
+        p.hitCap[r] = o.cap;
+        a += 2ull * o.cap; c += o.cap != 0;
+    }
+}
+CF_DEV void plan_write_load(const DPlan &p, uint64_t first, uint32_t (&cap)[kScanPer], uint64_t &a, uint32_t &c) {
+    scan_load(p.hitCap, p.nReads, first, cap);
+    a = 0; c = 0;
+#pragma unroll
+    for (int i = 0; i < kScanPer; i++) { a += 2ull * cap[i]; c += cap[i] != 0; }
+}
+CF_DEV void plan_write_stage(const uint32_t (&cap)[kScanPer], uint32_t t, uint64_t offA, uint32_t offC, uint64_t *stageA, uint32_t *stageC) {
+#pragma unroll
+    for (int i = 0; i < kScanPer; i++) {
+        const uint32_t at = scan_stage_at(t * kScanPer + i);
+        stageA[at] = offA; stageC[at] = offC;
+        offA += 2ull * cap[i]; offC += cap[i] != 0;
+    }
+}
+CF_DEV void plan_write_one(const DPlan &p, uint64_t r, uint64_t hb, uint32_t slot) {
+    if (r > p.nReads) return;
+    p.hitBase[r] = hb;
+    if (r == p.nReads) { p.slotOf[r] = slot; plan_fill_total(p, hb, slot); return; }
+    const uint8_t pb = p.pass[r];
+    const uint64_t L = plan_len(p, r);
+    p.slotOf[r] = (pb & kPassOk) ? slot : kNone32;
+    if (pb & kPassOk) plan_fill_one(p, (uint32_t)r, (uint32_t)L, (uint32_t)plan_woff(p, r), (pb & kPassHasN) != 0, p.hitCap[r], slot, (uint32_t)hb);
+    if (p.maxScore) {
+        if (!p.paired) { if (r < p.nQueries) p.maxScore[r] = plan_maxscore_one(L, (pb & kPassOk) != 0, 0, false, false); }
+        else if (!(r & 1) && (r >> 1) < p.nQueries)
+            p.maxScore[r >> 1] = plan_maxscore_one(L, (pb & kPassOk) != 0, plan_len(p, r + 1), (p.pass[r + 1] & kPassOk) != 0, true);
+    }
+}
+CF_DEV void plan_write_thread(const DPlan &p, uint64_t tile0, uint32_t t, const uint64_t *stageA, const uint32_t *stageC) {
+#pragma unroll 4
+    for (int i = 0; i < kScanPer; i++) {
+        const uint32_t j = (uint32_t)i * kScanBlock + t;
+        if (tile0 + j > p.nReads) break;
+        plan_write_one(p, tile0 + j, stageA[scan_stage_at(j)], stageC[scan_stage_at(j)]);
+    }
 }
 
 struct DCompact {
@@ -654,27 +722,51 @@
     OutRow o; o.taxID = tax; o.uniqueID = (uint32_t)a; o.score = (uint32_t)(a >> 32); o.hitLen = (uint32_t)bb; o.tidx = (uint32_t)(bb >> 32);
     return o;
 }
+CF_DEV void compact_one(const DCompact &c, uint32_t q, uint64_t f) {
+    const uint32_t n = c.nOut[q] < c.k ? c.nOut[q] : c.k;
+    if (c.dstNarrow) {
+        if (n <= kFieldRows) {
+#pragma unroll
+            for (uint32_t i = 0; i < kFieldRows; i++) if (i < n) {
+                const uint64_t a = c.o1a[i * c.oStride + q], bb = c.o1b[i * c.oStride + q];
+                c.dstNarrow[f + i] = NarrowRow{(uint32_t)a, (uint32_t)(bb >> 32), (uint32_t)(a >> 32), (uint32_t)bb};
+            }
+        } else for (uint32_t i = 0; i < n; i++) { const OutRow o = c.out[(uint64_t)q * c.k + i]; c.dstNarrow[f + i] = NarrowRow{o.uniqueID, o.tidx, o.score, o.hitLen}; }
+        const uint32_t r0 = c.paired ? 2 * q : q;
+        c.qinfo[q] = (uint8_t)(n | ((c.pass[r0] & kPassOk) ? 0x40u : 0u) | ((c.paired && (c.pass[r0 + 1] & kPassOk)) ? 0x80u : 0u));
+        return;
+    }
+    if (n <= kFieldRows) {
+#pragma unroll
+        for (uint32_t i = 0; i < kFieldRows; i++) if (i < n) c.dst[f + i] = row_of_one(c.o1tax[i * c.oStride + q], c.o1a[i * c.oStride + q], c.o1b[i * c.oStride + q]);
+    } else for (uint32_t i = 0; i < n; i++) c.dst[f + i] = c.out[(uint64_t)q * c.k + i];
+}
 CF_DEV void compact_body(const DCompact &c, uint32_t q) {
     if (q == c.nQueries && c.st) c.st->rowsOut = c.rowFirst[q];
     if (q >= c.nQueries) return;
-    const uint32_t n = c.nOut[q] < c.k ? c.nOut[q] : c.k;
-    const uint64_t f = c.rowFirst[q];
-    if (c.dstNarrow) {
-        if (n <= kFieldRows) {
-#pragma unroll
-            for (uint32_t i = 0; i < kFieldRows; i++) if (i < n) {
-                const uint64_t a = c.o1a[i * c.oStride + q], bb = c.o1b[i * c.oStride + q];
-                c.dstNarrow[f + i] = NarrowRow{(uint32_t)a, (uint32_t)(bb >> 32), (uint32_t)(a >> 32), (uint32_t)bb};
-            }
-        } else for (uint32_t i = 0; i < n; i++) { const OutRow o = c.out[(uint64_t)q * c.k + i]; c.dstNarrow[f + i] = NarrowRow{o.uniqueID, o.tidx, o.score, o.hitLen}; }
-        const uint32_t r0 = c.paired ? 2 * q : q;
-        c.qinfo[q] = (uint8_t)(n | (c.pass[r0] ? 0x40u : 0u) | ((c.paired && c.pass[r0 + 1]) ? 0x80u : 0u));
-        return;
-    }
-    if (n <= kFieldRows) {
-#pragma unroll
-        for (uint32_t i = 0; i < kFieldRows; i++) if (i < n) c.dst[f + i] = row_of_one(c.o1tax[i * c.oStride + q], c.o1a[i * c.oStride + q], c.o1b[i * c.oStride + q]);
-    } else for (uint32_t i = 0; i < n; i++) c.dst[f + i] = c.out[(uint64_t)q * c.k + i];
+    compact_one(c, q, c.rowFirst[q]);
+}
+CF_DEV void compact_write_load(const DCompact &c, uint64_t first, uint32_t (&x)[kScanPer], uint64_t &a) {
+    scan_load(c.nOut, c.nQueries, first, x);
+    a = 0;
+#pragma unroll
+    for (int i = 0; i < kScanPer; i++) a += x[i];
+}
+CF_DEV void compact_write_stage(const uint32_t (&x)[kScanPer], uint32_t t, uint64_t offA, uint64_t *stageA) {
+#pragma unroll
+    for (int i = 0; i < kScanPer; i++) { stageA[scan_stage_at(t * kScanPer + i)] = offA; offA += x[i]; }
+}
+CF_DEV void compact_write_thread(const DCompact &c, uint64_t *rowFirst, uint64_t tile0, uint32_t t, const uint64_t *stageA) {
+#pragma unroll 4
+    for (int i = 0; i < kScanPer; i++) {
+        const uint32_t j = (uint32_t)i * kScanBlock + t;
+        const uint64_t q = tile0 + j;
+        if (q > c.nQueries) break;
+        const uint64_t f = stageA[scan_stage_at(j)];
+        rowFirst[q] = f;
+        if (q == c.nQueries) { if (c.st) c.st->rowsOut = f; }
+        else compact_one(c, (uint32_t)q, f);
+    }
 }
 
 CF_DEV int ps_begin(const DIndex &ix, const DBatch &b, uint64_t wbase, uint32_t L, bool fw, uint32_t cur,
@@ -1884,7 +1976,7 @@
     for (int a = 0; a < 2; a++) { qi.lo[a] = qi.hi[a] = 0; qi.nProc[a][0] = qi.nProc[a][1] = 0; qi.brk[a] = 0; qi.pad2[a] = 0; qi.maxG[a][0] = qi.maxG[a][1] = 0; }
     uint32_t nPlanned = 0;
     const uint32_t r0 = b.paired ? 2 * q : q;
-    const bool p0 = b.pass[r0] != 0, p1 = b.paired ? b.pass[r0 + 1] != 0 : false;
+    const bool p0 = (b.pass[r0] & kPassOk) != 0, p1 = b.paired ? (b.pass[r0 + 1] & kPassOk) != 0 : false;
     uint32_t rds[2] = {r0, r0 + 1};
     int nm;
     uint32_t isPaired = 0, firstMate = 0;
@@ -1979,7 +2071,7 @@
     uint32_t fOf0 = 2, fOf1 = 2, np0 = 0, np1 = 0, brk0 = 0, brk1 = 0;
     uint8_t isPaired = 0, firstMate = 0;
     const uint32_t r0 = b.paired ? 2 * q : q;
-    const bool p0 = b.pass[r0] != 0, p1 = b.paired ? b.pass[r0 + 1] != 0 : false;
+    const bool p0 = (b.pass[r0] & kPassOk) != 0, p1 = b.paired ? (b.pass[r0 + 1] & kPassOk) != 0 : false;
     uint32_t rd0 = r0;
     int nm;
     if (b.paired && p0 && p1) { nm = 2; isPaired = 1; }
diff --git a/centrifuge_amd/csrc/cf_scan.hpp b/centrifuge_amd/csrc/cf_scan.hpp
--- a/centrifuge_amd/csrc/cf_scan.hpp
+++ b/centrifuge_amd/csrc/cf_scan.hpp
@@ -3,25 +3,15 @@
 
 #include <cstdint>
 
+#include "cf_tile.hpp"
+
 namespace cfamd {
 
 enum : int { SCAN_WORDS = 0, SCAN_PLAIN = 1, SCAN_HITS = 2 };
-constexpr int kScanBlock = 256, kScanPer = 16, kScanTile = kScanBlock * kScanPer;
 
 template <int MODE>
 __device__ __forceinline__ uint64_t scan_value(uint32_t x) {
     return MODE == SCAN_WORDS ? (((uint64_t)x + 31) >> 5) : MODE == SCAN_HITS ? 2ull * x : (uint64_t)x;
-}
-
-__device__ __forceinline__ void scan_load(const uint32_t *in, uint64_t n, uint64_t first, uint32_t (&x)[kScanPer]) {
-    if (first + kScanPer <= n) {
-        const uint4 *p = reinterpret_cast<const uint4 *>(in + first);
-#pragma unroll
-        for (int i = 0; i < kScanPer / 4; i++) { const uint4 v = p[i]; x[4 * i] = v.x; x[4 * i + 1] = v.y; x[4 * i + 2] = v.z; x[4 * i + 3] = v.w; }
-    } else {
-#pragma unroll
-        for (int i = 0; i < kScanPer; i++) x[i] = first + i < n ? in[first + i] : 0u;
-    }
 }
 
 __device__ __forceinline__ void scan_block_reduce(uint64_t &a, uint32_t &c, uint64_t *ldsA, uint32_t *ldsC) {
@@ -73,6 +63,22 @@
     }
 }
 
+__device__ __forceinline__ void scan_block_exclusive(uint64_t a, uint32_t c, uint64_t *ldsA, uint32_t *ldsC, uint64_t &offA, uint32_t &offC) {
+    uint64_t ia = a;
+    uint32_t ic = c;
+    const int lane = threadIdx.x & 63, w = threadIdx.x >> 6;
+#pragma unroll
+    for (int d = 1; d < 64; d <<= 1) {
+        const uint64_t ta = __shfl_up(ia, d, 64);
+        const uint32_t tc = __shfl_up(ic, d, 64);
+        if (lane >= d) { ia += ta; ic += tc; }
+    }
+    if (lane == 63) { ldsA[w] = ia; ldsC[w] = ic; }
+    __syncthreads();
+    offA = ia - a; offC = ic - c;
+    for (int i = 0; i < w; i++) { offA += ldsA[i]; offC += ldsC[i]; }
+}
+
 template <int MODE>
 __global__ void __launch_bounds__(kScanBlock) k_scan_write(const uint32_t *in, uint64_t n, const uint64_t *tileA, const uint32_t *tileC,
                                                             uint64_t *outA, uint32_t *outC) {
@@ -85,20 +91,11 @@
     uint32_t c = 0;
 #pragma unroll
     for (int i = 0; i < kScanPer; i++) { a += scan_value<MODE>(x[i]); if (MODE == SCAN_HITS) c += x[i] != 0; }
-    uint64_t ia = a;
-    uint32_t ic = c;
-    const int lane = threadIdx.x & 63, w = threadIdx.x >> 6;
-#pragma unroll
-    for (int d = 1; d < 64; d <<= 1) {
-        const uint64_t ta = __shfl_up(ia, d, 64);
-        const uint32_t tc = __shfl_up(ic, d, 64);
-        if (lane >= d) { ia += ta; ic += tc; }
-    }
-    if (lane == 63) { ldsA[w] = ia; ldsC[w] = ic; }
-    __syncthreads();
-    uint64_t offA = tileA[blockIdx.x] + ia - a;
-    uint32_t offC = (MODE == SCAN_HITS ? tileC[blockIdx.x] : 0u) + ic - c;
-    for (int i = 0; i < w; i++) { offA += ldsA[i]; offC += ldsC[i]; }
+    uint64_t offA;
+    uint32_t offC;
+    scan_block_exclusive(a, c, ldsA, ldsC, offA, offC);
+    offA += tileA[blockIdx.x];
+    if (MODE == SCAN_HITS) offC += tileC[blockIdx.x];
 #pragma unroll
     for (int i = 0; i < kScanPer; i++) {
         const uint64_t idx = first + i;
@@ -106,6 +103,34 @@
         offA += scan_value<MODE>(x[i]);
         if (MODE == SCAN_HITS) offC += x[i] != 0;
     }
+}
+
+template <class F>
+__device__ __forceinline__ void scan_sums_tile(const F &f, uint64_t *tileA, uint32_t *tileC) {
+    __shared__ uint64_t ldsA[kScanBlock / 64];
+    __shared__ uint32_t ldsC[kScanBlock / 64];
+    uint64_t a;
+    uint32_t c;
+    f.sums((uint64_t)blockIdx.x * kScanTile, threadIdx.x, a, c);
+    scan_block_reduce(a, c, ldsA, ldsC);
+    if (threadIdx.x == 0) { tileA[blockIdx.x] = a; if (F::kWithC) tileC[blockIdx.x] = c; }
+}
+template <class F>
+__device__ __forceinline__ void scan_write_tile(const F &f, const uint64_t *tileA, const uint32_t *tileC) {
+    __shared__ uint64_t ldsA[kScanBlock / 64];
+    __shared__ uint32_t ldsC[kScanBlock / 64];
+    __shared__ uint64_t stageA[kScanStage];
+    __shared__ uint32_t stageC[F::kWithC ? kScanStage : 1];
+    uint32_t x[kScanPer];
+    uint64_t a, offA;
+    uint32_t c, offC;
+    f.load((uint64_t)blockIdx.x * kScanTile + (uint64_t)threadIdx.x * kScanPer, x, a, c);
+    scan_block_exclusive(a, c, ldsA, ldsC, offA, offC);
+    offA += tileA[blockIdx.x];
+    if (F::kWithC) offC += tileC[blockIdx.x];
+    f.stage(x, threadIdx.x, offA, offC, stageA, stageC);
+    __syncthreads();
+    f.write((uint64_t)blockIdx.x * kScanTile, threadIdx.x, stageA, stageC);
 }
 
 inline uint32_t scan_tiles_for(uint64_t n) { return (uint32_t)((n + 1 + kScanTile - 1) / kScanTile); }
diff --git a/centrifuge_amd/csrc/cf_tile.hpp b/centrifuge_amd/csrc/cf_tile.hpp
--- /dev/null
+++ b/centrifuge_amd/csrc/cf_tile.hpp
@@ -0,0 +1,24 @@
+#pragma once
+#include "cf_platform.hpp"
+
+namespace cfamd {
+
+constexpr int kScanBlock = 256, kScanPer = 16, kScanTile = kScanBlock * kScanPer;
+static_assert(kScanPer % 2 == 0, "a pair of mates never straddles two threads, let alone two tiles");
+constexpr int kScanStage = kScanTile + kScanBlock;
+CF_DEV uint32_t scan_stage_at(uint32_t j) { return j + j / kScanPer; }
+
+CF_DEV void scan_load(const uint32_t *in, uint64_t n, uint64_t first, uint32_t (&x)[kScanPer]) {
+    if (first + kScanPer <= n) {
+#pragma unroll
+        for (int i = 0; i < kScanPer / 4; i++) {
+            const u64x2 v = cf_load16(reinterpret_cast<const uint8_t *>(in + first) + 16 * i);
+            x[4 * i] = (uint32_t)v.x; x[4 * i + 1] = (uint32_t)(v.x >> 32); x[4 * i + 2] = (uint32_t)v.y; x[4 * i + 3] = (uint32_t)(v.y >> 32);
+        }
+    } else {
+#pragma unroll
+        for (int i = 0; i < kScanPer; i++) x[i] = first + i < n ? in[first + i] : 0u;
+    }
+}
+
+}
```

After: 1.488 billion, median of 6. 1.04x the previous value.
